# dexmal/dexbotic

Measured on AMD Instinct MI355X. Metric: episodes/sec DB-CogACT fine-tune, higher is better.
Workload: dtype bf16; 1 GPU; DB-CogACT fine-tune step (CLIP-L/14@224 x1 view, Qwen2.5-7B-class 28L decoder, DiT-B head, AdamW), 16 episodes/GPU, 32-token instruction, S=287; global_batch=16, seq_len=287, parallelism=dp1, optimizer=AdamW serial, grad_accum=1, activations=resident

## Files before the change

dexbotic_amd/_lib.py:

```python
from __future__ import annotations

import ctypes as C
import os

import torch

_HERE = os.path.dirname(os.path.abspath(__file__))
LIB_PATH = os.environ.get("DXA_LIB") or os.path.join(_HERE, "libdexbotic_amd.so")

F32, BF16 = 0, 1
ACT_NONE, ACT_GELU_ERF, ACT_GELU_TANH, ACT_QUICK_GELU, ACT_SILU, ACT_RELU, ACT_SIGMOID = 0, 1, 2, 3, 4, 5, 6
NT, NN, TN = 0, 1, 2
FILTER_BICUBIC = 3
FUSE_NONE, FUSE_SWIGLU = 0, 1

_vp, _i64, _i32, _f32, _sz = C.c_void_p, C.c_int64, C.c_int32, C.c_float, C.c_size_t
_int = C.c_int


class DxaError(RuntimeError):
    pass


class GemmDesc(C.Structure):
    _fields_ = [
        ("layout", _i32), ("in_dtype", _i32), ("out_dtype", _i32), ("act", _i32),
        ("M", _i64), ("N", _i64), ("K", _i64),
        ("A", _vp), ("lda", _i64), ("B", _vp), ("ldb", _i64), ("C", _vp), ("ldc", _i64),
        ("bias", _vp), ("residual", _vp), ("ldr", _i64), ("aux_out", _vp), ("mulgrad", _vp), ("ldg", _i64),
        ("alpha", _f32), ("accumulate", _i32), ("nb", _i32 * 3),
        ("sA", _i64 * 3), ("sB", _i64 * 3), ("sC", _i64 * 3), ("sR", _i64 * 3), ("sG", _i64 * 3),
        ("epi_f32", _i32), ("mirror", _vp), ("sumsq", _vp),
        ("A2", _vp), ("B2", _vp), ("K2", _i64),
        ("fuse", _i32), ("ld_aux", _i64),
    ]


class GemmStepInfo(C.Structure):
    _fields_ = [
        ("kernel", C.c_char_p), ("grid", _i32 * 3), ("block", _i32), ("lds", _i32),
        ("K", _i64), ("K2", _i64), ("a_off", _i64), ("b_off", _i64), ("seg2", _i32),
        ("accumulate", _i32), ("bias", _i32), ("residual", _i32),
        ("tm", _i32), ("tn", _i32), ("full", _i32), ("tail_r", _i32), ("split_s", _i32), ("group_m", _i32),
        ("vecA", _i32), ("vecB", _i32), ("vecC", _i32), ("vecR", _i32), ("vecG", _i32), ("vecBias", _i32),
        ("ksplit", _i32), ("kper", _i32), ("split_ws", _i32), ("mirror", _i32), ("sumsq", _i32),
    ]


class GemmPlanInfo(C.Structure):
    _fields_ = [("nsteps", _i32), ("mirror_pass", _i32), ("sumsq_pass", _i32), ("step", GemmStepInfo * 2)]


class Split3Op(C.Structure):
    _fields_ = [("src", _vp), ("ld", _i64), ("dst", _vp), ("rows", _i64), ("cols", _i64), ("pad", _i64), ("side", _i32), ("transposed", _i32)]


class AttnDesc(C.Structure):
    _fields_ = [
        ("dtype", _i32), ("B", _i32), ("Hq", _i32), ("Hkv", _i32), ("Sq", _i32), ("Sk", _i32), ("D", _i32),
        ("causal", _i32), ("scale", _f32),
        ("q", _vp), ("q_sb", _i64), ("q_sh", _i64), ("q_ss", _i64),
        ("k", _vp), ("k_sb", _i64), ("k_sh", _i64), ("k_ss", _i64),
        ("v", _vp), ("v_sb", _i64), ("v_sh", _i64), ("v_ss", _i64),
        ("o", _vp), ("o_sb", _i64), ("o_sh", _i64), ("o_ss", _i64),
        ("lse", _vp), ("kv_start", _vp), ("kv_end", _vp),
        ("d_o", _vp), ("do_sb", _i64), ("do_sh", _i64), ("do_ss", _i64),
        ("dq", _vp), ("dq_sb", _i64), ("dq_sh", _i64), ("dq_ss", _i64),
        ("dk", _vp), ("dk_sb", _i64), ("dk_sh", _i64), ("dk_ss", _i64),
        ("dv", _vp), ("dv_sb", _i64), ("dv_sh", _i64), ("dv_ss", _i64),
        ("force_generic", _i32),
        ("q_limit", _vp), ("key_valid", _vp), ("drop_mask", _vp),
    ]


class AdamWDesc(C.Structure):
    _fields_ = [
        ("p", _vp), ("g", _vp), ("m", _vp), ("v", _vp), ("shadow", _vp),
        ("chunk_start", _vp), ("chunk_len", _vp), ("chunk_grp", _vp), ("n_chunks", _i32),
        ("lr", _f32 * 8), ("wd", _f32 * 8),
        ("beta1", _f32), ("beta2", _f32), ("eps", _f32), ("bc1", _f32), ("bc2", _f32),
        ("clip_coef", _vp), ("g_dtype", _i32), ("chunk_state", _vp), ("chunk_mv_start", _vp),
    ]


class ImageDesc(C.Structure):
    _fields_ = [
        ("src", _vp), ("n", _i32), ("h", _i32), ("w", _i32), ("pad", _i32), ("bg", C.c_ubyte * 4),
        ("res_h", _i32), ("res_w", _i32), ("crop_top", _i32), ("crop_left", _i32), ("out_h", _i32), ("out_w", _i32),
        ("row0", _i32), ("rows", _i32), ("hb", _vp), ("hk", _vp), ("hks", _i32), ("vb", _vp), ("vk", _vp), ("vks", _i32),
        ("tmp", _vp), ("out", _vp), ("out_dtype", _i32), ("out_u8", _vp), ("rescale", C.c_double),
        ("mean", _f32 * 3), ("std", _f32 * 3),
    ]


class DecodeDesc(C.Structure):
    _fields_ = [
        ("layers", _vp), ("x_in", _vp), ("out", _vp), ("final_norm_w", _vp), ("cos_row", _vp), ("sin_row", _vp),
        ("workspace", _vp), ("workspace_bytes", _sz),
        ("n_layers", _i32), ("d", _i32), ("Hq", _i32), ("Hkv", _i32), ("D", _i32), ("F", _i32), ("slot", _i32), ("kv_lo", _i32),
        ("max_len", _i32), ("eps", _f32),
    ]


SIGNATURES = {
    "dxa_last_error": (C.c_char_p, []),
    "dxa_version": (_int, []),
    "dxa_gemm": (_int, [C.POINTER(GemmDesc), _vp]),
    "dxa_gemm_plan": (_int, [C.POINTER(GemmDesc), C.POINTER(GemmPlanInfo)]),
    "dxa_gemm_kernel_name": (C.c_char_p, [_int]),
    "dxa_split3": (_int, [_vp, _i64, _vp, _i64, _i64, _int, _vp]),
    "dxa_split3_t": (_int, [_vp, _i64, _vp, _i64, _i64, _i64, _int, _vp]),
    "dxa_split3_pair": (_int, [C.POINTER(Split3Op), C.POINTER(Split3Op), _vp]),
    "dxa_rmsnorm_fwd": (_int, [_vp, _vp, _vp, _vp, _i64, _i64, _f32, _int, _int, _vp]),
    "dxa_rmsnorm_bwd": (_int, [_vp, _vp, _vp, _vp, _vp, _vp, _vp, _i64, _i64, _int, _int, _vp]),
    "dxa_layernorm_fwd": (_int, [_vp, _vp, _vp, _vp, _vp, _vp, _i64, _i64, _f32, _int, _int, _vp]),
    "dxa_layernorm_bwd": (_int, [_vp, _vp, _vp, _vp, _vp, _vp, _vp, _vp, _i64, _i64, _int, _int, _vp]),
    "dxa_norm_bwd_blocks": (_int, [_i64]),
    "dxa_downsample_layernorm_fwd": (_int, [_vp, _vp, _vp, _vp, _vp, _vp, _i64, _i64, _i64, _f32, _int, _int, _vp]),
    "dxa_downsample_layernorm_bwd": (_int, [_vp, _vp, _vp, _vp, _vp, _vp, _vp, _i64, _i64, _i64, _int, _int, _vp]),
    "dxa_colsum": (_int, [_vp, _i64, _vp, _i64, _i64, _int, _int, _vp, _sz, _vp]),
    "dxa_rope_split": (_int, [_vp, _vp, _vp, _vp, _vp, _vp, _vp, _int, _int, _int, _int, _int, _int, _vp]),
    "dxa_rope_merge": (_int, [_vp, _vp, _vp, _vp, _vp, _vp, _vp, _int, _int, _int, _int, _int, _int, _vp]),
    "dxa_rope_split_at": (_int, [_vp, _vp, _vp, _vp, _vp, _vp, _vp, _int, _int, _int, _int, _int, _int, _int, _int, _vp]),
    "dxa_rope_merge_at": (_int, [_vp, _vp, _vp, _vp, _vp, _vp, _vp, _int, _int, _int, _int, _int, _int, _int, _int, _vp]),
    "dxa_qknorm_rope_split": (_int, [_vp, _vp, _vp, _vp, _vp, _vp, _f32, _vp, _vp, _vp, _vp, _int, _int, _int, _int, _int, _int, _vp]),
    "dxa_qknorm_rope_merge": (_int, [_vp, _vp, _vp, _vp, _vp, _vp, _vp, _vp, _vp, _vp, _vp, _vp, _int, _int, _int, _int, _int, _int, _vp]),
    "dxa_qknorm_rope_merge_blocks": (_int, [_i64, _int, _int, _int, _int]),
    "dxa_attn_fwd": (_int, [C.POINTER(AttnDesc), _vp]),
    "dxa_attn_fwd_workspace": (_sz, [C.POINTER(AttnDesc)]),
    "dxa_attn_fwd_ws": (_int, [C.POINTER(AttnDesc), _vp, _sz, _vp]),
    "dxa_attn_bwd_workspace": (_sz, [C.POINTER(AttnDesc)]),
    "dxa_attn_bwd": (_int, [C.POINTER(AttnDesc), _vp, _sz, _vp]),
    "dxa_swiglu_fwd": (_int, [_vp, _vp, _i64, _i64, _int, _vp]),
    "dxa_swiglu_bwd": (_int, [_vp, _vp, _vp, _i64, _i64, _int, _vp]),
    "dxa_axpby": (_int, [_vp, _vp, _vp, _i64, _f32, _f32, _int, _vp]),
    "dxa_mul": (_int, [_vp, _vp, _vp, _i64, _int, _vp]),
    "dxa_mul_rows": (_int, [_vp, _vp, _vp, _i64, _i64, _i64, _int, _vp]),
    "dxa_glu_fwd": (_int, [_vp, _vp, _i64, _i64, _int, _int, _vp]),
    "dxa_glu_bwd": (_int, [_vp, _vp, _vp, _i64, _i64, _int, _int, _vp]),
    "dxa_act_fwd": (_int, [_vp, _vp, _i64, _int, _int, _vp]),
    "dxa_act_bwd": (_int, [_vp, _vp, _vp, _i64, _int, _int, _vp]),
    "dxa_add": (_int, [_vp, _vp, _vp, _i64, _int, _vp]),
    "dxa_cast": (_int, [_vp, _vp, _i64, _int, _int, _vp]),
    "dxa_copy2d": (_int, [_vp, _i64, _vp, _i64, _i64, _i64, _i64, _int, _int, _vp]),
    "dxa_transpose": (_int, [_vp, _i64, _vp, _i64, _i64, _i64, _i64, _int, _vp]),
    "dxa_permute_bshd": (_int, [_vp, _vp, _int, _int, _int, _int, _int, _int, _vp]),
    "dxa_splice_fwd": (_int, [_vp, _vp, _vp, _vp, _i64, _i64, _int, _vp]),
    "dxa_splice_bwd": (_int, [_vp, _vp, _vp, _vp, _i64, _i64, _int, _vp]),
    "dxa_zero_rows": (_int, [_vp, _vp, _i64, _i64, _vp]),
    "dxa_gather_rows": (_int, [_vp, _vp, _vp, _i64, _i64, _int, _int, _vp]),
    "dxa_scatter_rows": (_int, [_vp, _vp, _vp, _i64, _i64, _i64, _int, _int, _vp]),
    "dxa_im2col": (_int, [_vp, _vp, _int, _int, _int, _int, _i64, _int, _int, _vp]),
    "dxa_vit_embed_fwd": (_int, [_vp, _vp, _vp, _vp, _int, _int, _int, _int, _int, _vp]),
    "dxa_vit_embed_bwd": (_int, [_vp, _vp, _int, _int, _int, _int, _vp]),
    "dxa_qsample": (_int, [_vp, _vp, _vp, _vp, _vp, _i64, _i64, _vp]),
    "dxa_timestep_embedding": (_int, [_vp, _vp, _vp, _i64, _int, _vp]),
    "dxa_dit_assemble_fwd": (_int, [_vp, _vp, _vp, _vp, _vp, _int, _int, _int, _vp]),
    "dxa_dit_assemble_bwd": (_int, [_vp, _vp, _vp, _int, _int, _int, _vp]),
    "dxa_token_drop": (_int, [_vp, _vp, _vp, _vp, _i64, _i64, _vp]),
    "dxa_token_drop_bwd": (_int, [_vp, _vp, _vp, _vp, _i64, _i64, _int, _vp]),
    "dxa_dropout_mask": (_int, [_vp, _i64, _f32, C.c_uint64, C.c_uint64, _int, _vp]),
    "dxa_bank_consolidate": (_int, [_vp, _vp, _int, _i64, _i64, _int, _int, _vp, _vp]),
    "dxa_add_rows": (_int, [_vp, _vp, _vp, _i64, _i64, _i64, _f32, _int, _vp]),
    "dxa_token_sum": (_int, [_vp, _vp, _i64, _i64, _i64, _f32, _int, _vp]),
    "dxa_mse_loss": (_int, [_vp, _vp, _vp, _vp, _i64, _f32, _vp]),
    "dxa_mse_loss_rows": (_int, [_vp, _vp, _vp, _vp, _vp, _i64, _i64, _f32, _vp]),
    "dxa_ddim_step": (_int, [_vp, _vp, _i64, _i64, _int, _f32, _f32, _f32, _f32, _vp]),
    "dxa_adamw": (_int, [C.POINTER(AdamWDesc), _vp]),
    "dxa_sumsq": (_int, [_vp, _i64, _int, _vp, _vp, _int, _vp]),
    "dxa_sumsq_ranges": (_int, [_vp, _int, _vp, _vp, _int, _vp, _vp, _int, _vp]),
    "dxa_sum_f32": (_int, [_vp, _i64, _vp, _int, _vp]),
    "dxa_gemm_sumsq_slots": (_i64, [_i64, _i64]),
    "dxa_cross_entropy_fwd": (_int, [_vp, _i64, _vp, _vp, _vp, _i64, _i64, _i64, _int, _vp]),
    "dxa_cross_entropy_bwd": (_int, [_vp, _i64, _vp, _vp, _vp, _f32, _vp, _i64, _i64, _i64, _i64, _int, _vp]),
    "dxa_soft_cross_entropy_fwd": (_int, [_vp, _i64, _vp, _vp, _vp, _i64, _i64, _i64, _vp, _vp, _int, _f32, _int, _vp]),
    "dxa_soft_cross_entropy_bwd": (_int, [_vp, _i64, _vp, _vp, _vp, _f32, _vp, _i64, _i64, _i64, _i64, _vp, _vp, _int, _f32,
                                          _int, _vp]),
    "dxa_argmax_rows": (_int, [_vp, _i64, _vp, _i64, _i64, _int, _vp]),
    "dxa_sample_rows": (_int, [_vp, _i64, _i64, _i64, _int, _f32, _i64, _f32, _vp, _vp, _vp, _vp, _vp, _vp]),
    "dxa_resample_ksize":(_int, [_int, _int]),
    "dxa_resample_coeffs": (_int, [_int, _int, _int, _vp, _vp]),
    "dxa_image_preprocess": (_int, [C.POINTER(ImageDesc), _vp]),
    "dxa_dit_blocks_workspace": (_sz, [_int, _int, _int]),
    "dxa_dit_blocks_fwd": (_int, [_vp, _vp, _int, _int, _int, _int, _int, _int, _f32, _vp, _sz, _vp]),
    "dxa_dit_blocks_status": (_int, [_vp, _vp]),
    "dxa_dit_sample_workspace": (_sz, [_int, _int, _int]),
    "dxa_dit_sample_fwd": (_int, [_vp] * 9 + [_int, _int, _int, _int, _f32, _vp, _int, _int, _int, _int, _int, _int, _f32, _vp, _sz, _vp]),
    "dxa_dit_bf16_pack_bytes": (_sz, [_int, _int, _int]),
    "dxa_dit_bf16_pack": (_int, [_vp, _int, _int, _int, _vp, _sz, _vp, _vp]),
    "dxa_dit_bf16_pack_per_bytes": (_sz, [_int, _int, _int]),
    "dxa_dit_bf16_pack_per": (_int, [_vp, _int, _int, _int, _vp, _sz, _vp, _vp]),
    "dxa_dit_sample_bf16_per_fwd": (_int, [_vp] * 9 + [_int, _int, _int, _int, _f32, _vp, _vp, _int, _int, _int, _int, _int, _int, _int, _f32, _vp, _sz, _vp]),
    "dxa_dit_sample_bf16_workspace": (_sz, [_int, _int, _int]),
    "dxa_dit_sample_bf16_fwd": (_int, [_vp] * 9 + [_int, _int, _int, _int, _f32, _vp, _int, _int, _int, _int, _int, _int, _f32, _vp, _sz, _vp]),
    "dxa_decode_step_workspace": (_sz, [_int, _int, _int, _int, _int]),
    "dxa_decode_step": (_int, [C.POINTER(DecodeDesc), _vp]),
    "dxa_decode_status": (_int, [_vp, _vp]),
    "dxa_clip_coef": (_int, [_vp, _f32, _vp, _vp, _vp]),
    "dxa_clip_coef_scaled": (_int, [_vp, _f32, _f32, _vp, _vp, _vp]),
    "dxa_scale": (_int, [_vp, _i64, _f32, _vp]),
    "dxa_scale_dev": (_int, [_vp, _i64, _vp, _vp]),
}


def _load() -> C.CDLL:
    if not os.path.exists(LIB_PATH):
        raise ImportError(
            f"dexbotic_amd: native library {LIB_PATH} not found. Build it with "
            "`python -m dexbotic_amd.build` (hipcc --offload-arch=gfx950); there is no CPU fallback.")
    lib = C.CDLL(LIB_PATH)
    for name, (res, args) in SIGNATURES.items():
        try:
            fn = getattr(lib, name)
        except AttributeError as e:
            raise ImportError(f"dexbotic_amd: symbol {name} missing from {LIB_PATH} (stale build?)") from e
        fn.restype = res
        fn.argtypes = args
    return lib


lib = _load()


def last_error() -> str:
    return (lib.dxa_last_error() or b"").decode()


def check(rc: int, what: str = "") -> None:
    if rc != 0:
        raise DxaError(f"{what}: status {rc}: {last_error()}")
```

dexbotic_amd/csrc/gemm.hip:

```cpp
#include "common.h"
#include "gemm_common.h"

#include <algorithm>
#include <cassert>

namespace {


template <typename T> struct EltTraits;
template <> struct EltTraits<float> { static constexpr int EPC = 4; };
template <> struct EltTraits<bf16_t> { static constexpr int EPC = 8; };

__device__ __forceinline__ int lds_off(int row, int chunk) { return row * ROWB + ((chunk ^ (row & 7)) << 4); }

template <typename T, int NR>
__device__ __forceinline__ void load_kc(uint4 (&r)[4], const T* __restrict__ base, int64_t ld, int64_t row0,
                                        int64_t rows, int64_t k0, int64_t K, int vec, int tid) {
  constexpr int EPC = EltTraits<T>::EPC;
  const int c = tid & 7;
  const int64_t k = k0 + (int64_t)c * EPC;
#pragma unroll
  for (int i = 0; i < NR / 32; ++i) {
    const int64_t row = row0 + (tid >> 3) + 32 * i;
    uint4 v = make_uint4(0, 0, 0, 0);
// ... 515 lines not shown
#pragma unroll
    for (int w = 0; w < 8; ++w) {
      const float4 v = *reinterpret_cast<const float4*>(red[w][wave][lane]);
      a4[0] += v.x; a4[1] += v.y; a4[2] += v.z; a4[3] += v.w;
    }
  }
  if (split_s > 1) {
    constexpr int SC1 = 16;
    constexpr uint32_t SLOT = MB * 64 * 16;
    const __amdgpu_buffer_rsrc_t rW = __builtin_amdgcn_make_buffer_rsrc(p.ws, 0, (int)(256u * 7u * 4u * 64u * 16u), 0x00020000);
    const uint32_t slot0 = (uint32_t)tile * (uint32_t)(split_s - 1) * SLOT + (uint32_t)(wave * 64 + lane) * 16u;
    if (split_j < split_s - 1) {
      if (worker) {
        const f32x4_t v = {a4[0], a4[1], a4[2], a4[3]};
        __builtin_amdgcn_raw_buffer_store_b128(__builtin_bit_cast(u32x4_t, v), rW, slot0 + (uint32_t)split_j * SLOT, 0, SC1);
      }
      asm volatile("s_waitcnt vmcnt(0)" ::: "memory");
      __syncthreads();
      if (tid == 0) __hip_atomic_fetch_add(p.flags + tile, 1, __ATOMIC_RELAXED, __HIP_MEMORY_SCOPE_AGENT);
      return;
    }
    if (tid == 0) {
      while (__hip_atomic_load(p.flags + tile, __ATOMIC_RELAXED, __HIP_MEMORY_SCOPE_AGENT) < split_s - 1)
        __builtin_amdgcn_s_sleep(2);
      __hip_atomic_store(p.flags + tile, 0, __ATOMIC_RELAXED, __HIP_MEMORY_SCOPE_AGENT);
    }
    __syncthreads();
    if (worker) {
      float own[4] = {a4[0], a4[1], a4[2], a4[3]};
      a4[0] = a4[1] = a4[2] = a4[3] = 0.f;
      for (int sj = 0; sj < split_s - 1; ++sj) {
        const f32x4_t v = __builtin_bit_cast(f32x4_t, __builtin_amdgcn_raw_buffer_load_b128(rW, slot0 + (uint32_t)sj * SLOT, 0, SC1));
        a4[0] += v[0]; a4[1] += v[1]; a4[2] += v[2]; a4[3] += v[3];
      }
      a4[0] += own[0]; a4[1] += own[1]; a4[2] += own[2]; a4[3] += own[3];
    }
  }
  if (!worker) return;
  const int64_t m = (int64_t)wave * 16 + l16, n = n0 + 4 * lg;
  if (m >= p.M || n >= p.N) return;
  const int n_ok = (int)min((int64_t)4, p.N - n);
  float bv[4] = {0.f, 0.f, 0.f, 0.f};
  const float* bias = reinterpret_cast<const float*>(p.bias);
  if (bias) load4<float>(bv, bias + n, p.vecBias, n_ok);
  epilogue4<float, float>(p, reinterpret_cast<float*>(p.C), reinterpret_cast<float*>(p.aux),
                          reinterpret_cast<const float*>(p.R), reinterpret_cast<const float*>(p.G), bv, m, n, n_ok, a4);
}

template <int MB, typename TO, int U = 2>
__global__ __launch_bounds__(512) void gemm_skinny_bf16_kernel(const GemmP p) {
  __shared__ float red[8][MB][64][4];
  const int tid = threadIdx.x, lane = tid & 63, wave = tid >> 6;
  const int l16 = lane & 15, lg = lane >> 4;
  const int split_s = p.split_s > 1 ? p.split_s : 1;
  const int ntile = (int)gridDim.x / split_s;
  const int tile = (int)blockIdx.x % ntile, split_j = (int)blockIdx.x / ntile;
  const int64_t n0 = (int64_t)tile * 16;
  const bf16_t* W = reinterpret_cast<const bf16_t*>(p.B) + min(n0 + l16, p.N - 1) * p.ldb + 8 * lg;
  const bf16_t* A[MB];
#pragma unroll
  for (int mb = 0; mb < MB; ++mb)
    A[mb] = reinterpret_cast<const bf16_t*>(p.A) + min((int64_t)mb * 16 + l16, p.M - 1) * p.lda + 8 * lg;
  f32x4_t acc[MB];
#pragma unroll
  for (int mb = 0; mb < MB; ++mb) acc[mb] = (f32x4_t){0.f, 0.f, 0.f, 0.f};
  const int nkb = (int)(p.K / 64);
  const int kb_lo = split_j * nkb / split_s, kb_hi = (split_j + 1) * nkb / split_s;
  for (int kb = kb_lo + wave; kb < kb_hi; kb += 8 * U) {
    u32x4n_t wv[U][2];
    uint4 av[U][MB][2];
#pragma unroll
    for (int u = 0; u < U; ++u) {
      const int k0 = (kb + 8 * u) * 64;
      if (kb + 8 * u < kb_hi) {
#pragma unroll
        for (int j = 0; j < 2; ++j) wv[u][j] = __builtin_nontemporal_load(reinterpret_cast<const u32x4n_t*>(W + k0 + 32 * j));
#pragma unroll
        for (int mb = 0; mb < MB; ++mb)
#pragma unroll
          for (int j = 0; j < 2; ++j) av[u][mb][j] = *reinterpret_cast<const uint4*>(A[mb] + k0 + 32 * j);
      } else {
#pragma unroll
        for (int j = 0; j < 2; ++j) {
          wv[u][j] = (u32x4n_t){0u, 0u, 0u, 0u};
#pragma unroll
          for (int mb = 0; mb < MB; ++mb) av[u][mb][j] = make_uint4(0, 0, 0, 0);
        }
      }
    }
#pragma unroll
    for (int u = 0; u < U; ++u)
#pragma unroll
      for (int j = 0; j < 2; ++j)
#pragma unroll
        for (int mb = 0; mb < MB; ++mb)
          acc[mb] = __builtin_amdgcn_mfma_f32_16x16x32_bf16(__builtin_bit_cast(bf16x8_t, wv[u][j]),
                                                            __builtin_bit_cast(bf16x8_t, av[u][mb][j]), acc[mb], 0, 0, 0);
  }
#pragma unroll
  for (int mb = 0; mb < MB; ++mb)
    *reinterpret_cast<float4*>(red[wave][mb][lane]) = make_float4(acc[mb][0], acc[mb][1], acc[mb][2], acc[mb][3]);
  __syncthreads();
  const bool worker = wave < MB;
  float a4[4] = {0.f, 0.f, 0.f, 0.f};
  if (worker) {
#pragma unroll
    for (int w = 0; w < 8; ++w) {
      const float4 v = *reinterpret_cast<const float4*>(red[w][wave][lane]);
      a4[0] += v.x; a4[1] += v.y; a4[2] += v.z; a4[3] += v.w;
    }
  }
  if (split_s > 1) {
    constexpr int SC1 = 16;
    constexpr uint32_t SLOT = MB * 64 * 16;
    const __amdgpu_buffer_rsrc_t rW = __builtin_amdgcn_make_buffer_rsrc(p.ws, 0, (int)(256u * 7u * 4u * 64u * 16u), 0x00020000);
    const uint32_t slot0 = (uint32_t)tile * (uint32_t)(split_s - 1) * SLOT + (uint32_t)(wave * 64 + lane) * 16u;
    if (split_j < split_s - 1) {
      if (worker) {
        const f32x4_t v = {a4[0], a4[1], a4[2], a4[3]};
        __builtin_amdgcn_raw_buffer_store_b128(__builtin_bit_cast(u32x4_t, v), rW, slot0 + (uint32_t)split_j * SLOT, 0, SC1);
      }
      asm volatile("s_waitcnt vmcnt(0)" ::: "memory");
      __syncthreads();
      if (tid == 0) __hip_atomic_fetch_add(p.flags + tile, 1, __ATOMIC_RELAXED, __HIP_MEMORY_SCOPE_AGENT);
      return;
    }
    if (tid == 0) {
      while (__hip_atomic_load(p.flags + tile, __ATOMIC_RELAXED, __HIP_MEMORY_SCOPE_AGENT) < split_s - 1)
        __builtin_amdgcn_s_sleep(2);
      __hip_atomic_store(p.flags + tile, 0, __ATOMIC_RELAXED, __HIP_MEMORY_SCOPE_AGENT);
    }
    __syncthreads();
    if (worker) {
      const float own[4] = {a4[0], a4[1], a4[2], a4[3]};
      a4[0] = a4[1] = a4[2] = a4[3] = 0.f;
      for (int sj = 0; sj < split_s - 1; ++sj) {
        const f32x4_t v = __builtin_bit_cast(f32x4_t, __builtin_amdgcn_raw_buffer_load_b128(rW, slot0 + (uint32_t)sj * SLOT, 0, SC1));
        a4[0] += v[0]; a4[1] += v[1]; a4[2] += v[2]; a4[3] += v[3];
      }
      a4[0] += own[0]; a4[1] += own[1]; a4[2] += own[2]; a4[3] += own[3];
    }
  }
  if (!worker) return;
  const int64_t m = (int64_t)wave * 16 + l16, n = n0 + 4 * lg;
  if (m >= p.M || n >= p.N) return;
  const int n_ok = (int)min((int64_t)4, p.N - n);
  float bv[4] = {0.f, 0.f, 0.f, 0.f};
  const bf16_t* bias = reinterpret_cast<const bf16_t*>(p.bias);
  if (bias) load4<bf16_t>(bv, bias + n, p.vecBias, n_ok);
  epilogue4<bf16_t, TO>(p, reinterpret_cast<TO*>(p.C), reinterpret_cast<TO*>(p.aux), reinterpret_cast<const bf16_t*>(p.R),
                        reinterpret_cast<const bf16_t*>(p.G), bv, m, n, n_ok, a4);
}


template <typename TO, int AI, typename TE>
__global__ __launch_bounds__(512) void gemm_nt_ring_kernel(const GemmP p) {
#if defined(__HIP_DEVICE_COMPILE__)
  extern __shared__ __attribute__((aligned(16))) char smem[];
  constexpr int A_ST = 256 * 64, STAGE = 2 * A_ST;
  constexpr int BMR = AI * 64;
  const int tid = threadIdx.x, lane = tid & 63;
  const int wave = __builtin_amdgcn_readfirstlane(tid >> 6);
  const int wm = wave >> 2, wn = wave & 3;
  const int l32 = lane & 31, lh = lane >> 5;

  int bid = blockIdx.x;
  int split_j = 0, split_s = 1, tail_i = 0;
  if (bid < p.full) {
    const int q = p.full >> 3, r = p.full & 7, xcd = bid & 7;
    bid = (xcd < r ? xcd * (q + 1) : r * (q + 1) + (xcd - r) * q) + (bid >> 3);
  } else {
    const int idx = bid - p.full;
    tail_i = idx % p.tail_r;
    split_j = idx / p.tail_r;
    split_s = p.split_s;
    bid = p.full + tail_i;
  }
  const int GROUP_M = p.group_m;
  const int width = GROUP_M * p.tn;
  const int group = bid / width;
  const int first_pm = group * GROUP_M;
  const int gsz = min(p.tm - first_pm, GROUP_M);
  const int pm = first_pm + (bid % width) % gsz;
  const int pn = (bid % width) / gsz;
  const int64_t m0 = (int64_t)pm * BMR, n0 = (int64_t)pn * 256;
  const bool has_a = AI == 4 || wave < 6;

  const uint32_t bytesA = (uint32_t)(((p.M - 1) * p.lda + p.K) * 2);
  const uint32_t bytesB = (uint32_t)(((p.N - 1) * p.ldb + p.K) * 2);
  const __amdgpu_buffer_rsrc_t rA = __builtin_amdgcn_make_buffer_rsrc(const_cast<char*>(p.A), 0, bytesA, 0x00020000);
  const __amdgpu_buffer_rsrc_t rB = __builtin_amdgcn_make_buffer_rsrc(const_cast<char*>(p.B), 0, bytesB, 0x00020000);
  uint32_t offA[2], offB[2];
#pragma unroll
  for (int j = 0; j < 2; ++j) {
    const int row = (wave * 2 + j) * 16 + (lane >> 2);
    const int chunk = (lane & 3) ^ ((row >> 2) & 3);
    const int64_t ga = m0 + row, gb = n0 + row;
    offA[j] = ga < p.M ? (uint32_t)((ga * p.lda) * 2 + chunk * 16) : 0x80000000u;
    offB[j] = gb < p.N ? (uint32_t)((gb * p.ldb) * 2 + chunk * 16) : 0x80000000u;
  }
  const int nk_tot = (int)(p.K / 32);
  const int k_lo = (int)((int64_t)split_j * nk_tot / split_s);
  const int nk = (int)((int64_t)(split_j + 1) * nk_tot / split_s) - k_lo;
#define DMA_A(slab, j) __builtin_amdgcn_raw_ptr_buffer_load_lds(rA, (lds_void_t*)(smem + ((slab) & 3) * STAGE + (wave * 2 + (j)) * 1024), 16, offA[j], (k_lo + (slab)) * 64, 0, 0)
#define DMA_B(slab, j) __builtin_amdgcn_raw_ptr_buffer_load_lds(rB, (lds_void_t*)(smem + ((slab) & 3) * STAGE + A_ST + (wave * 2 + (j)) * 1024), 16, offB[j], (k_lo + (slab)) * 64, 0, 0)
#define DMA_SLAB(slab) do { if (has_a) { DMA_A(slab, 0); DMA_A(slab, 1); } DMA_B(slab, 0); DMA_B(slab, 1); } while (0)
#define WAIT_PREV_SLAB() do { if (has_a) asm volatile("s_waitcnt vmcnt(4)" ::: "memory"); else asm volatile("s_waitcnt vmcnt(2)" ::: "memory"); } while (0)

  f32x16_t acc[AI][2];
#pragma unroll
  for (int i = 0; i < AI; ++i)
#pragma unroll
    for (int j = 0; j < 2; ++j)
#pragma unroll
      for (int r = 0; r < 16; ++r) acc[i][j][r] = 0.f;

  DMA_SLAB(0);
  if (nk > 1) DMA_SLAB(1);
  if (nk > 2) {
    DMA_SLAB(2);
    WAIT_PREV_SLAB();
  } else {
    asm volatile("s_waitcnt vmcnt(0)" ::: "memory");
  }
  __builtin_amdgcn_s_barrier();
  __builtin_amdgcn_sched_barrier(0);

  u32x4_t a0[AI], b0[2], a1[AI], b1[2];
  const uint32_t lds0 = (uint32_t)(uintptr_t)(__attribute__((address_space(3))) char*)smem;
  const int sw = (l32 >> 2) & 3;
  const uint32_t abase0 = lds0 + (wm * (BMR / 2) + l32) * 64 + (((0 + lh) ^ sw) << 4);
  const uint32_t abase1 = lds0 + (wm * (BMR / 2) + l32) * 64 + (((2 + lh) ^ sw) << 4);
  const uint32_t bbase0 = lds0 + A_ST + (wn * 64 + l32) * 64 + (((0 + lh) ^ sw) << 4);
  const uint32_t bbase1 = lds0 + A_ST + (wn * 64 + l32) * 64 + (((2 + lh) ^ sw) << 4);
#define DS_READ(dst, addr, imm) asm volatile("ds_read_b128 %0, %1 offset:%2" : "=v"(dst) : "v"(addr), "n"(imm) : "memory")
#define RD_SET(A_, B_, abase, bbase, soff)                                                      \
  do {                                                                                          \
    const uint32_t ax_ = (abase) + (soff), bx_ = (bbase) + (soff);                              \
    DS_READ(A_[0], ax_, 0); DS_READ(A_[1], ax_, 2048); DS_READ(A_[2], ax_, 4096);          \
    if constexpr (AI > 3) DS_READ(A_[3], ax_, 6144);                                            \
    DS_READ(B_[0], bx_, 0); DS_READ(B_[1], bx_, 2048);                                          \
  } while (0)
#define MFMA1(A_, B_, i, j) acc[i][j] = __builtin_amdgcn_mfma_f32_32x32x16_bf16(__builtin_bit_cast(bf16x8_t, B_[j]), __builtin_bit_cast(bf16x8_t, A_[i]), acc[i][j], 0, 0, 0)
#define SB() __builtin_amdgcn_sched_barrier(0)

  RD_SET(a0, b0, abase0, bbase0, 0u);
  for (int t = 0; t < nk; ++t) {
    const uint32_t soff = (uint32_t)((t & 3) * STAGE), soff_n = (uint32_t)(((t + 1) & 3) * STAGE);
    const bool dma = t + 3 < nk;
    asm volatile("s_waitcnt lgkmcnt(0)" ::: "memory");
    SB();
    MFMA1(a0, b0, 0, 0); MFMA1(a0, b0, 0, 1);
    SB();
    RD_SET(a1, b1, abase1, bbase1, soff);
    SB();
    MFMA1(a0, b0, 1, 0); MFMA1(a0, b0, 1, 1);
    SB();
    if (dma && has_a) { DMA_A(t + 3, 0); DMA_A(t + 3, 1); }
    SB();
    MFMA1(a0, b0, 2, 0); MFMA1(a0, b0, 2, 1);
    SB();
    if (dma) { DMA_B(t + 3, 0); DMA_B(t + 3, 1); }
    SB();
    if constexpr (AI > 3) { MFMA1(a0, b0, 3, 0); MFMA1(a0, b0, 3, 1); }
    SB();
    asm volatile("s_waitcnt lgkmcnt(0)" ::: "memory");
    SB();
    MFMA1(a1, b1, 0, 0); MFMA1(a1, b1, 0, 1);
    SB();
    if (t + 1 < nk) RD_SET(a0, b0, abase0, bbase0, soff_n);
    SB();
    MFMA1(a1, b1, 1, 0); MFMA1(a1, b1, 1, 1);
    MFMA1(a1, b1, 2, 0); MFMA1(a1, b1, 2, 1);
    if constexpr (AI > 3) { MFMA1(a1, b1, 3, 0); MFMA1(a1, b1, 3, 1); }
    SB();
    if (dma) WAIT_PREV_SLAB();
    else asm volatile("s_waitcnt vmcnt(0)" ::: "memory");
    __builtin_amdgcn_s_barrier();
    SB();
  }
#undef DMA_A
#undef DMA_B
#undef DMA_SLAB
#undef WAIT_PREV_SLAB
#undef DS_READ
#undef RD_SET
#undef MFMA1
#undef SB

  tile_finish<TO, AI, TE>(p, acc, smem, tid, lane, wave, wm, wn, l32, lh, m0, n0, split_j, split_s, tail_i);
#endif
}


template <typename TO, typename TE, bool LEAN, bool A_KS, bool B_KS, int FUSE = 0>
__global__ __launch_bounds__(512) void gemm_pp_kernel(const GemmP p) {
#if defined(__HIP_DEVICE_COMPILE__)
  extern __shared__ __attribute__((aligned(16))) char smem[];
  constexpr int REG = 256 * 128;
  constexpr int BUF = 2 * REG;
  const int tid = threadIdx.x, lane = tid & 63;
  const int wave = __builtin_amdgcn_readfirstlane(tid >> 6);
  const int wm = wave >> 2, wn = wave & 3;
  const int l32 = lane & 31, lh = lane >> 5;

  int bid = blockIdx.x;
  int split_j = 0, split_s = 1, tail_i = 0;
  if (bid < p.full) {
    const int q = p.full >> 3, r = p.full & 7, xcd = bid & 7;
    bid = (xcd < r ? xcd * (q + 1) : r * (q + 1) + (xcd - r) * q) + (bid >> 3);
  } else {
    const int idx = bid - p.full;
    tail_i = idx % p.tail_r;
    split_j = idx / p.tail_r;
    split_s = p.split_s;
    bid = p.full + tail_i;
  }
  int m0i, n0i;
  sk_tile_origin(p, bid, m0i, n0i);
  const int64_t m0 = m0i, n0 = n0i;

  const uint32_t bytesA = (uint32_t)((A_KS ? (p.K - 1) * p.lda + p.M : (p.M - 1) * p.lda + p.K) * 2);
  const uint32_t bytesB = (uint32_t)((B_KS ? (p.K - 1) * p.ldb + p.N : (p.N - 1) * p.ldb + p.K) * 2);
  const __amdgpu_buffer_rsrc_t rA = __builtin_amdgcn_make_buffer_rsrc(const_cast<char*>(p.A), 0, bytesA, 0x00020000);
  const __amdgpu_buffer_rsrc_t rB = __builtin_amdgcn_make_buffer_rsrc(const_cast<char*>(p.B), 0, bytesB, 0x00020000);
#define PP_A_ROW0(h, j) ((((wave * 2 + (j)) & 7) * 8) + (((wave * 2 + (j)) >> 3) * 128) + 64 * (h))
#define PP_B_ROW0(h, j) ((((wave * 2 + (j)) >> 2) * 64) + (((wave * 2 + (j)) & 3) * 8) + 32 * (h))
  uint32_t voA[2][2], voB[2][2];
  {
    const int lrow = lane >> 3, lslot = lane & 7;
    const uint32_t lda2 = (uint32_t)p.lda * 2u, ldb2 = (uint32_t)p.ldb * 2u;
#pragma unroll
    for (int h = 0; h < 2; ++h)
#pragma unroll
      for (int j = 0; j < 2; ++j) {
        const int krow = (wave * 2 + j) * 4 + (lane >> 4);
        const int sig = (lane & 15) ^ ((krow & 3) << 2) ^ (((krow >> 3) & 1) << 1);
        if constexpr (A_KS) {
          const int ga = m0i + (sig >> 3) * 128 + 64 * h + 8 * (sig & 7);
          voA[h][j] = ga < (int)p.M ? (uint32_t)krow * lda2 + (uint32_t)ga * 2u : 0x80000000u;
        } else {
          const int ra = PP_A_ROW0(h, j) + lrow, ga = m0i + ra;
          voA[h][j] = ga < (int)p.M ? (uint32_t)ga * lda2 + (uint32_t)((lslot ^ ((ra >> 1) & 7)) << 4) : 0x80000000u;
        }
        if constexpr (B_KS) {
          const int gb = n0i + (sig >> 2) * 64 + 32 * h + 8 * (sig & 3);
          voB[h][j] = gb < (int)p.N ? (uint32_t)krow * ldb2 + (uint32_t)gb * 2u : 0x80000000u;
        } else if constexpr (FUSE == 1) {
          const int rb = PP_B_ROW0(h, j) + lrow, half_n = (int)(p.N >> 1);
          const int lc = (n0i >> 1) + (rb >> 6) * 32 + (rb & 31), gb = ((rb >> 5) & 1) * half_n + lc;
          voB[h][j] = lc < half_n ? (uint32_t)gb * ldb2 + (uint32_t)((lslot ^ ((rb >> 1) & 7)) << 4) : 0x80000000u;
        } else {
          const int rb = PP_B_ROW0(h, j) + lrow, gb = n0i + rb;
          voB[h][j] = gb < (int)p.N ? (uint32_t)gb * ldb2 + (uint32_t)((lslot ^ ((rb >> 1) & 7)) << 4) : 0x80000000u;
        }
      }
  }
  const int nk1 = (int)((p.K + 63) >> 6);
  const int nk_tot = nk1 + ((A_KS && B_KS) ? (int)((p.K2 + 63) >> 6) : 0);
  const bool seg2 = (A_KS && B_KS) && p.K2 > 0;
  const __amdgpu_buffer_rsrc_t rA2 = __builtin_amdgcn_make_buffer_rsrc(
      const_cast<char*>(seg2 ? p.A2 : p.A), 0, seg2 ? (uint32_t)(((p.K2 - 1) * p.lda + p.M) * 2) : 0u, 0x00020000);
  const __amdgpu_buffer_rsrc_t rB2 = __builtin_amdgcn_make_buffer_rsrc(
      const_cast<char*>(seg2 ? p.B2 : p.B), 0, seg2 ? (uint32_t)(((p.K2 - 1) * p.ldb + p.N) * 2) : 0u, 0x00020000);
  const int k_lo = split_j * nk_tot / split_s;
  const int nk = (split_j + 1) * nk_tot / split_s - k_lo;
  const uint32_t ktileA = A_KS ? 64u * (uint32_t)p.lda * 2u : 0u, ktileB = B_KS ? 64u * (uint32_t)p.ldb * 2u : 0u;
#define PP_DMA(rsrc, vo, ldsoff, buf, soff)                                                                             \
  __builtin_amdgcn_raw_ptr_buffer_load_lds(rsrc, (lds_void_t*)(smem + (buf) * BUF + (ldsoff)), 16, vo, soff, 0, 0)
#define PP_DMA_A1(h, j, buf, tile)                                                                          \
  do {                                                                                                      \
    if constexpr (A_KS && B_KS) {                                                                           \
      const int kt_ = k_lo + (tile);                                                                        \
      if (kt_ < nk1) PP_DMA(rA, voA[h][j] + (uint32_t)kt_ * ktileA, (h) * 16384 + (wave * 2 + (j)) * 1024, buf, 0);          \
      else PP_DMA(rA2, voA[h][j] + (uint32_t)(kt_ - nk1) * ktileA, (h) * 16384 + (wave * 2 + (j)) * 1024, buf, 0);           \
    } else if constexpr (A_KS) {                                                                            \
      const uint32_t kb_ = (uint32_t)(k_lo + (tile)) * ktileA;                                              \
      PP_DMA(rA, voA[h][j] + kb_, (h) * 16384 + (wave * 2 + (j)) * 1024, buf, 0);                           \
    } else {                                                                                                \
      PP_DMA(rA, voA[h][j], PP_A_ROW0(h, j) * 128, buf, (k_lo + (tile)) * 128);                             \
    }                                                                                                       \
  } while (0)
#define PP_DMA_B1(h, j, buf, tile)                                                                          \
  do {                                                                                                      \
    if constexpr (A_KS && B_KS) {                                                                           \
      const int kt_ = k_lo + (tile);                                                                        \
      if (kt_ < nk1) PP_DMA(rB, voB[h][j] + (uint32_t)kt_ * ktileB, REG + (h) * 16384 + (wave * 2 + (j)) * 1024, buf, 0);    \
      else PP_DMA(rB2, voB[h][j] + (uint32_t)(kt_ - nk1) * ktileB, REG + (h) * 16384 + (wave * 2 + (j)) * 1024, buf, 0);     \
    } else if constexpr (B_KS) {                                                                            \
      const uint32_t kb_ = (uint32_t)(k_lo + (tile)) * ktileB;                                              \
      PP_DMA(rB, voB[h][j] + kb_, REG + (h) * 16384 + (wave * 2 + (j)) * 1024, buf, 0);                     \
    } else {                                                                                                \
      PP_DMA(rB, voB[h][j], REG + PP_B_ROW0(h, j) * 128, buf, (k_lo + (tile)) * 128);                       \
    }                                                                                                       \
  } while (0)
#define PP_DMA_A(h, buf, tile) do { PP_DMA_A1(h, 0, buf, tile); PP_DMA_A1(h, 1, buf, tile); } while (0)
#define PP_DMA_B(h, buf, tile) do { PP_DMA_B1(h, 0, buf, tile); PP_DMA_B1(h, 1, buf, tile); } while (0)

  f32x4_t acc[8][4];
#pragma unroll
  for (int i = 0; i < 8; ++i)
#pragma unroll
    for (int j = 0; j < 4; ++j) acc[i][j] = (f32x4_t){0.f, 0.f, 0.f, 0.f};

  const uint32_t lds0 = (uint32_t)(uintptr_t)(__attribute__((address_space(3))) char*)smem;
  const int i16 = lane & 15, g = lane >> 4, sw = (i16 >> 1) & 7, tq = (i16 >> 2) & 3;
  const uint32_t ks_lane = (uint32_t)((8 * g + (i16 >> 2)) * 256 + (g & 1) * 32 + (i16 & 3) * 8);
  const uint32_t ya = A_KS ? lds0 + ks_lane + (uint32_t)(((wm * 2) ^ tq) << 6)
                           : (lds0 + (wm * 128 + i16) * 128) | (uint32_t)((g ^ sw) << 4);
  const uint32_t yb = B_KS ? lds0 + REG + ks_lane + (uint32_t)((wn ^ tq) << 6)
                           : (lds0 + REG + (wn * 64 + i16) * 128) | (uint32_t)((g ^ sw) << 4);
  u32x4_t af[4][2], bq[2][2][2];
  typedef uint32_t u32x2_t __attribute__((ext_vector_type(2)));
#define PP_READ(dst, addr, imm) asm volatile("ds_read_b128 %0, %1 offset:%2" : "=v"(dst) : "v"(addr), "n"(imm) : "memory")
#define PP_READ_TR(dst, addr, imm) asm volatile("ds_read_b64_tr_b16 %0, %1 offset:%2" : "=v"(dst) : "v"(addr), "n"(imm) : "memory")
#define PP_FRAG_TR(dst, addr, imm)                                                       \
  do {                                                                                   \
    u32x2_t lo_ = {0u, 0u}, hi_ = {0u, 0u};                                              \
    PP_READ_TR(lo_, addr, imm); PP_READ_TR(hi_, addr, (imm) + 1024);                     \
    dst = (u32x4_t){lo_[0], lo_[1], hi_[0], hi_[1]};                                     \
  } while (0)
#define PP_RDF_A(cur, h, b, ks)                                                                             \
  do {                                                                                                      \
    if constexpr (A_KS) PP_FRAG_TR(af[b][ks], ya ^ (uint32_t)((cur) * BUF + 32 * (b)), (h) * 16384 + (ks) * 8192); \
    else PP_READ(af[b][ks], ya ^ (uint32_t)((cur) * BUF + 64 * (ks)), (4 * (h) + (b)) * 2048);            \
  } while (0)
#define PP_RDF_B(cur, j, b, ks)                                                                             \
  do {                                                                                                      \
    if constexpr (B_KS) PP_FRAG_TR(bq[j][b][ks], yb ^ (uint32_t)((cur) * BUF + 32 * (b)), (j) * 16384 + (ks) * 8192); \
    else PP_READ(bq[j][b][ks], yb ^ (uint32_t)((cur) * BUF + 64 * (ks)), (2 * (j) + (b)) * 2048);         \
  } while (0)
#define PP_MFMA(h, j, b, jb, ks)                                                                                            \
  acc[4 * (h) + (b)][2 * (j) + (jb)] = __builtin_amdgcn_mfma_f32_16x16x32_bf16(                                           \
      __builtin_bit_cast(bf16x8_t, bq[j][jb][ks]), __builtin_bit_cast(bf16x8_t, af[b][ks]), acc[4 * (h) + (b)][2 * (j) + (jb)], 0, 0, 0)
#define PP_SB() __builtin_amdgcn_sched_barrier(0)
#define PP_BAR() do { PP_SB(); __builtin_amdgcn_s_barrier(); PP_SB(); } while (0)
#define PP_MFMA2(h, j, b, ks, R) do { PP_MFMA(h, j, b, 0, ks); PP_MFMA(h, j, b, 1, ks); PP_SB(); R(ks, b); PP_SB(); } while (0)
#define PP_COMPUTE_R(h, j, R)                                                                     \
  do {                                                                                            \
    asm volatile("s_waitcnt lgkmcnt(0)" ::: "memory");                                            \
    PP_SB();                                                                                      \
    PP_MFMA2(h, j, 0, 0, R); PP_MFMA2(h, j, 1, 0, R); PP_MFMA2(h, j, 2, 0, R); PP_MFMA2(h, j, 3, 0, R); \
    PP_MFMA2(h, j, 0, 1, R); PP_MFMA2(h, j, 1, 1, R); PP_MFMA2(h, j, 2, 1, R); PP_MFMA2(h, j, 3, 1, R); \
  } while (0)
#define PP_R_NONE(ks, b) do { } while (0)
#define PP_VMCNT(n) asm volatile("s_waitcnt vmcnt(" #n ")" ::: "memory")
#if defined(DXA_PP_STAMPS)
  uint64_t ts_[8];
  uint32_t iv_[8] = {0u, 0u, 0u, 0u, 0u, 0u, 0u, 0u}, ts_last_ = 0u;
#define PP_STAMP(i) asm volatile("s_memtime %0" : "=s"(ts_[i]))
#define PP_STAMPS_FOLD()                                                                                    \
  do {                                                                                                      \
    asm volatile("s_waitcnt lgkmcnt(0)" ::: "memory");                                                      \
    PP_SB();                                                                                                \
    if (ts_last_ != 0u) iv_[7] += (uint32_t)ts_[0] - ts_last_;                                              \
    _Pragma("unroll") for (int i_ = 0; i_ < 7; ++i_) iv_[i_] += (uint32_t)ts_[i_ + 1] - (uint32_t)ts_[i_];  \
    ts_last_ = (uint32_t)ts_[7];                                                                            \
    PP_SB();                                                                                                \
  } while (0)
#else
#define PP_STAMP(i) do { } while (0)
#define PP_STAMPS_FOLD() do { } while (0)
#endif
#define PP_R_B1(ks, b) do { if constexpr (((b) & 1) != 0) PP_RDF_B(cur_, 1, (b) >> 1, ks); } while (0)
#define PP_R_A1(ks, b) PP_RDF_A(cur_, 1, b, ks)
#define PP_R_NEXT(ks, b)                                                                                    \
  do {                                                                                                      \
    if (more1) {                                                                                            \
      PP_RDF_A(cur_ ^ 1, 0, b, ks);                                                                         \
      if constexpr ((ks) == 1 && (b) < 2) PP_RDF_B(cur_ ^ 1, 0, (b) & 1, 0);                                \
      if constexpr ((ks) == 1 && (b) == 3) { PP_RDF_B(cur_ ^ 1, 0, 0, 1); PP_RDF_B(cur_ ^ 1, 0, 1, 1); }    \
    }                                                                                                       \
  } while (0)
#define PP_TILE(cur, t)                                                                                     \
  do {                                                                                                      \
    constexpr int cur_ = (cur);                                                                             \
    const bool more1 = (t) + 1 < nk, more2 = (t) + 2 < nk;                                                  \
                                                                                               \
    if (more1) { PP_DMA_A(1, cur_ ^ 1, (t) + 1); PP_SB(); PP_VMCNT(8); } else { PP_VMCNT(0); }              \
    PP_BAR(); PP_STAMP(0); PP_COMPUTE_R(0, 0, PP_R_B1); PP_BAR(); PP_STAMP(1);                              \
                                                                                               \
    if (more2) { PP_DMA_A(0, cur_, (t) + 2); PP_SB(); }                                                     \
    PP_BAR(); PP_STAMP(2); PP_COMPUTE_R(0, 1, PP_R_A1); PP_BAR(); PP_STAMP(3);                              \
                                                                                               \
    if (more2) { PP_DMA_B(0, cur_, (t) + 2); PP_SB(); PP_VMCNT(8); } else if (more1) { PP_VMCNT(4); }       \
    PP_BAR(); PP_STAMP(4); PP_COMPUTE_R(1, 1, PP_R_NONE); PP_BAR(); PP_STAMP(5);                                         \
                                                                                               \
    if (more2) { PP_DMA_B(1, cur_, (t) + 2); PP_SB(); PP_VMCNT(8); } else if (more1) { PP_VMCNT(2); }       \
    PP_BAR(); PP_STAMP(6); PP_COMPUTE_R(1, 0, PP_R_NEXT); PP_BAR(); PP_STAMP(7);                            \
    PP_STAMPS_FOLD();                                                                                       \
  } while (0)

  PP_DMA_A(0, 0, 0); PP_DMA_B(0, 0, 0); PP_DMA_B(1, 0, 0); PP_DMA_A(1, 0, 0);
  if (nk > 1) { PP_DMA_A(0, 1, 1); PP_DMA_B(0, 1, 1); PP_DMA_B(1, 1, 1); }
  PP_SB();
  if (nk > 1) { PP_VMCNT(8); } else { PP_VMCNT(2); }
  PP_BAR();
  PP_RDF_A(0, 0, 0, 0); PP_RDF_A(0, 0, 1, 0); PP_RDF_A(0, 0, 2, 0); PP_RDF_A(0, 0, 3, 0);
  PP_RDF_A(0, 0, 0, 1); PP_RDF_A(0, 0, 1, 1); PP_RDF_A(0, 0, 2, 1); PP_RDF_A(0, 0, 3, 1);
  PP_RDF_B(0, 0, 0, 0); PP_RDF_B(0, 0, 1, 0); PP_RDF_B(0, 0, 0, 1); PP_RDF_B(0, 0, 1, 1);
  PP_SB();
  if (wm == 1) PP_BAR();
  for (int t = 0; t < nk; t += 2) {
    PP_TILE(0, t);
    if (t + 1 < nk) PP_TILE(1, t + 1);
  }
  if (wm == 0) PP_BAR();
#if defined(DXA_PP_STAMPS)
  const uint32_t iv0_ = iv_[0], iv1_ = iv_[1], iv2_ = iv_[2], iv3_ = iv_[3], iv4_ = iv_[4], iv5_ = iv_[5], iv6_ = iv_[6], iv7_ = iv_[7];
#endif
#undef PP_A_ROW0
#undef PP_B_ROW0
#undef PP_DMA
#undef PP_DMA_A
#undef PP_DMA_B
#undef PP_READ
#undef PP_READ_TR
#undef PP_FRAG_TR
#undef PP_RDF_A
#undef PP_RDF_B
#undef PP_MFMA
#undef PP_MFMA2
#undef PP_SB
#undef PP_BAR
#undef PP_R_NONE
#undef PP_VMCNT
#undef PP_TILE
#undef PP_DMA_A1
#undef PP_DMA_B1
#undef PP_STAMP
#undef PP_STAMPS_FOLD
#undef PP_COMPUTE_R
#undef PP_R_B1
#undef PP_R_A1
#undef PP_R_NEXT

  if constexpr (LEAN) {
    if (!tile_split_exchange<4, 16>(p, acc, tid, split_j, split_s, tail_i)) return;
    __builtin_amdgcn_sched_barrier(0);
    if constexpr (FUSE == 1) sk_epilogue_swiglu<4, 16>(p, acc, smem + wave * 4096, lane, wm, wn, m0i, n0i);
    else sk_epilogue<TO, TE, 4, 16>(p, acc, smem + wave * 4096, lane, wm, wn, m0i, n0i, reinterpret_cast<float*>(smem + 8 * 4096), bid);
#if defined(DXA_PP_STAMPS)
    __syncthreads();
    if (m0i == 0 && n0i == 0 && lane == 0) {
      uint32_t* o_ = reinterpret_cast<uint32_t*>(p.C) + wave * 16;
      o_[0] = iv0_; o_[1] = iv1_; o_[2] = iv2_; o_[3] = iv3_; o_[4] = iv4_; o_[5] = iv5_; o_[6] = iv6_; o_[7] = iv7_;
      o_[8] = (uint32_t)nk;
    }
#endif
  } else {
    tile_finish<TO, 4, TE, false, 16>(p, acc, smem, tid, lane, wave, wm, wn, l32, lh, m0, n0, split_j, split_s, tail_i);
  }
#endif
}

#if defined(DXA_PP3_STAMPS)
__device__ unsigned long long g_pp3_stamps[4];
#define P3_STAMP(i) do { if (blockIdx.x == DXA_PP3_STAMPS && threadIdx.x == 0) { unsigned long long t_; asm volatile("s_memtime %0\n\ts_waitcnt lgkmcnt(0)" : "=s"(t_) :: "memory"); g_pp3_stamps[i] = t_; } } while (0)
#else
#define P3_STAMP(i) do { } while (0)
#endif
template <typename TO, typename TE, bool LEAN, int FUSE = 0>
__global__ __launch_bounds__(512) void gemm_pp3_kernel(const GemmP p) {
#if defined(__HIP_DEVICE_COMPILE__)
  extern __shared__ __attribute__((aligned(16))) char smem[];
  P3_STAMP(0);
  constexpr int AREG = 192 * 128, BREG = 256 * 128, BUFSZ = AREG + BREG;
  const int tid = threadIdx.x, lane = tid & 63;
  const int wave = __builtin_amdgcn_readfirstlane(tid >> 6);
  const int wm = wave >> 2, wn = wave & 3;
  const int l32 = lane & 31, lh = lane >> 5;
  int bid = blockIdx.x;
  int split_j = 0, split_s = 1, tail_i = 0;
  if (bid < p.full) {
    const int q = p.full >> 3, r = p.full & 7, xcd = bid & 7;
    bid = (xcd < r ? xcd * (q + 1) : r * (q + 1) + (xcd - r) * q) + (bid >> 3);
  } else {
    const int idx = bid - p.full;
    tail_i = idx % p.tail_r;
    split_j = idx / p.tail_r;
    split_s = p.split_s;
    bid = p.full + tail_i;
  }
  const int width = p.group_m * p.tn;
  const int group = bid / width;
  const int first_pm = group * p.group_m;
  const int gsz = min(p.tm - first_pm, p.group_m);
  const int pm = first_pm + (bid % width) % gsz;
  const int pn = (bid % width) / gsz;
  const int64_t m0 = (int64_t)pm * 192, n0 = (int64_t)pn * 256;

  const uint32_t bytesA = (uint32_t)(((p.M - 1) * p.lda + p.K) * 2);
  const uint32_t bytesB = (uint32_t)(((p.N - 1) * p.ldb + p.K) * 2);
  const __amdgpu_buffer_rsrc_t rA = __builtin_amdgcn_make_buffer_rsrc(const_cast<char*>(p.A), 0, bytesA, 0x00020000);
  const __amdgpu_buffer_rsrc_t rB = __builtin_amdgcn_make_buffer_rsrc(const_cast<char*>(p.B), 0, bytesB, 0x00020000);
#define P3_A_ROW0(g) ((wave >> 2) * 96 + 32 * (g) + (wave & 3) * 8)
#define P3_B_ROW0(h, j) ((((wave * 2 + (j)) >> 2) * 64) + (((wave * 2 + (j)) & 3) * 8) + 32 * (h))
  uint32_t voA[3], voB[2][2];
  {
    const int lrow = lane >> 3, lslot = lane & 7;
    const uint32_t lda2 = (uint32_t)p.lda * 2u, ldb2 = (uint32_t)p.ldb * 2u;
#pragma unroll
    for (int g = 0; g < 3; ++g) {
      const int ra = P3_A_ROW0(g) + lrow;
      const int64_t ga = m0 + ra;
      voA[g] = ga < p.M ? (uint32_t)ga * lda2 + (uint32_t)((lslot ^ ((ra >> 1) & 7)) << 4) : 0x80000000u;
    }
#pragma unroll
    for (int h = 0; h < 2; ++h)
#pragma unroll
      for (int j = 0; j < 2; ++j) {
        const int rb = P3_B_ROW0(h, j) + lrow;
        if constexpr (FUSE == 1) {
          const int half_n = (int)(p.N >> 1);
          const int lc = (int)(n0 >> 1) + (rb >> 6) * 32 + (rb & 31), gb = ((rb >> 5) & 1) * half_n + lc;
          voB[h][j] = lc < half_n ? (uint32_t)gb * ldb2 + (uint32_t)((lslot ^ ((rb >> 1) & 7)) << 4) : 0x80000000u;
        } else {
          const int64_t gb = n0 + rb;
          voB[h][j] = gb < p.N ? (uint32_t)gb * ldb2 + (uint32_t)((lslot ^ ((rb >> 1) & 7)) << 4) : 0x80000000u;
        }
      }
  }
  const int nk_tot = (int)(p.K / 64);
  const int k_lo = split_j * nk_tot / split_s;
  const int nk = (split_j + 1) * nk_tot / split_s - k_lo;
#define P3_DMA(rsrc, vo, ldsoff, buf, tile) \
  __builtin_amdgcn_raw_ptr_buffer_load_lds(rsrc, (lds_void_t*)(smem + (buf) * BUFSZ + (ldsoff)), 16, vo, (k_lo + (tile)) * 128, 0, 0)
#define P3_DMA_A(g, buf, tile) P3_DMA(rA, voA[g], P3_A_ROW0(g) * 128, buf, tile)
#define P3_DMA_B(h, buf, tile) do { P3_DMA(rB, voB[h][0], AREG + P3_B_ROW0(h, 0) * 128, buf, tile); P3_DMA(rB, voB[h][1], AREG + P3_B_ROW0(h, 1) * 128, buf, tile); } while (0)

  f32x16_t acc[3][2];
#pragma unroll
  for (int i = 0; i < 3; ++i)
#pragma unroll
    for (int j = 0; j < 2; ++j)
#pragma unroll
      for (int r = 0; r < 16; ++r) acc[i][j][r] = 0.f;

  const uint32_t lds0 = (uint32_t)(uintptr_t)(__attribute__((address_space(3))) char*)smem;
  const int sw = (l32 >> 1) & 7;
  const uint32_t ya0 = (lds0 + (wm * 96 + l32) * 128) | (uint32_t)((lh ^ sw) << 4), ya1 = ya0 + BUFSZ;
  const uint32_t yb0 = (lds0 + AREG + (wn * 64 + l32) * 128) | (uint32_t)((lh ^ sw) << 4), yb1 = yb0 + BUFSZ;
  u32x4_t af[2][4], bq[2][2][4];
#define P3_READ(dst, addr, imm) asm volatile("ds_read_b128 %0, %1 offset:%2" : "=v"(dst) : "v"(addr), "n"(imm) : "memory")
#define P3_RD_A(buf, g, set, ks) P3_READ(af[set][ks], ((buf) ? ya1 : ya0) ^ (uint32_t)(32 * (ks)), (g) * 4096)
#define P3_RD_B(buf, h, bset, ks) P3_READ(bq[bset][h][ks], ((buf) ? yb1 : yb0) ^ (uint32_t)(32 * (ks)), (h) * 4096)
#define P3_MFMA(g, set, bset, j, ks) acc[g][j] = __builtin_amdgcn_mfma_f32_32x32x16_bf16(__builtin_bit_cast(bf16x8_t, bq[bset][j][ks]), __builtin_bit_cast(bf16x8_t, af[set][ks]), acc[g][j], 0, 0, 0)
#define P3_SB() __builtin_amdgcn_sched_barrier(0)
#define P3_BAR() do { P3_SB(); __builtin_amdgcn_s_barrier(); P3_SB(); } while (0)
#define P3_COMPUTE(g, set, bset, R)                                                                 \
  do {                                                                                              \
    asm volatile("s_waitcnt lgkmcnt(0)" ::: "memory");                                              \
    P3_SB();                                                                                        \
    P3_MFMA(g, set, bset, 0, 0); P3_MFMA(g, set, bset, 1, 0); P3_SB(); R(0); P3_SB();               \
    P3_MFMA(g, set, bset, 0, 1); P3_MFMA(g, set, bset, 1, 1); P3_SB(); R(1); P3_SB();               \
    P3_MFMA(g, set, bset, 0, 2); P3_MFMA(g, set, bset, 1, 2); P3_SB(); R(2); P3_SB();               \
    P3_MFMA(g, set, bset, 0, 3); P3_MFMA(g, set, bset, 1, 3); P3_SB(); R(3); P3_SB();               \
  } while (0)
#define P3_VMCNT(n) asm volatile("s_waitcnt vmcnt(" #n ")" ::: "memory")
#define P3_TILE(cur, t)                                                                                                  \
  do {                                                                                                                   \
    constexpr int cur_ = (cur), s0_ = (cur), s1_ = (cur) ^ 1;            \
    const bool more1 = (t) + 1 < nk, more2 = (t) + 2 < nk;                                                               \
                                                                                                            \
    if (more1) P3_DMA_A(2, cur_ ^ 1, (t) + 1);                                                                           \
    if (more2) { P3_DMA_B(0, cur_, (t) + 2); P3_SB(); P3_VMCNT(7); } else if (more1) { P3_SB(); P3_VMCNT(5); } else { P3_VMCNT(0); } \
    P3_BAR();                                                                                                            \
    P3_COMPUTE(0, s0_, cur_, P3_R_A1);                                                                                   \
    P3_BAR();                                                                                                            \
                                                                                                            \
    if (more2) { P3_DMA_A(0, cur_, (t) + 2); P3_DMA_B(1, cur_, (t) + 2); P3_SB(); P3_VMCNT(7); } else if (more1) { P3_VMCNT(2); } \
    P3_BAR();                                                                                                            \
    P3_COMPUTE(1, s1_, cur_, P3_R_A2B0);                                                                                 \
    P3_BAR();                                                                                                            \
                                                                                                            \
    if (more2) { P3_DMA_A(1, cur_, (t) + 2); P3_SB(); P3_VMCNT(7); } else if (more1) { P3_VMCNT(1); }                    \
    P3_BAR();                                                                                                            \
    P3_COMPUTE(2, s0_, cur_, P3_R_A0B1);                                                                                 \
    P3_BAR();                                                                                                            \
  } while (0)
#define P3_R_A1(ks) P3_RD_A(cur_, 1, s1_, ks)
#define P3_R_A2B0(ks) do { P3_RD_A(cur_, 2, s0_, ks); if (more1) P3_RD_B(cur_ ^ 1, 0, cur_ ^ 1, ks); } while (0)
#define P3_R_A0B1(ks) do { if (more1) { P3_RD_A(cur_ ^ 1, 0, s1_, ks); P3_RD_B(cur_ ^ 1, 1, cur_ ^ 1, ks); } } while (0)

  P3_DMA_B(0, 0, 0); P3_DMA_A(0, 0, 0); P3_DMA_B(1, 0, 0); P3_DMA_A(1, 0, 0); P3_DMA_A(2, 0, 0);
  if (nk > 1) { P3_DMA_B(0, 1, 1); P3_DMA_A(0, 1, 1); P3_DMA_B(1, 1, 1); P3_DMA_A(1, 1, 1); }
  P3_SB();
  if (nk > 1) { P3_VMCNT(7); } else { P3_VMCNT(1); }
  P3_BAR();
  P3_STAMP(1);
#pragma unroll
  for (int ks = 0; ks < 4; ++ks) { P3_RD_A(0, 0, 0, ks); P3_RD_B(0, 0, 0, ks); P3_RD_B(0, 1, 0, ks); }
  P3_SB();
  if (wm == 1) P3_BAR();
  for (int t = 0; t < nk; t += 2) {
    P3_TILE(0, t);
    if (t + 1 < nk) P3_TILE(1, t + 1);
  }
  if (wm == 0) P3_BAR();
  P3_STAMP(2);
#undef P3_A_ROW0
#undef P3_B_ROW0
#undef P3_DMA
#undef P3_DMA_A
#undef P3_DMA_B
#undef P3_READ
#undef P3_RD_A
#undef P3_RD_B
#undef P3_MFMA
#undef P3_SB
#undef P3_BAR
#undef P3_COMPUTE
#undef P3_VMCNT
#undef P3_TILE
#undef P3_R_A1
#undef P3_R_A2B0
#undef P3_R_A0B1
  if constexpr (LEAN) {
    if (!tile_split_exchange<3>(p, acc, tid, split_j, split_s, tail_i)) return;
    __builtin_amdgcn_sched_barrier(0);
    if constexpr (FUSE == 1) sk_epilogue_swiglu<3>(p, acc, smem + wave * 4096, lane, wm, wn, (int)m0, (int)n0);
    else sk_epilogue<TO, TE, 3>(p, acc, smem + wave * 4096, lane, wm, wn, (int)m0, (int)n0, reinterpret_cast<float*>(smem + 8 * 4096), bid);
  } else {
    tile_finish<TO, 3, TE>(p, acc, smem, tid, lane, wave, wm, wn, l32, lh, m0, n0, split_j, split_s, tail_i);
  }
  asm volatile("s_waitcnt vmcnt(0)" ::: "memory");
  P3_STAMP(3);
#endif
}
#undef P3_STAMP

template <typename T>
__global__ __launch_bounds__(256) void sumsq_rows_k(const T* __restrict__ C, int64_t ldc, int64_t M, int64_t N,
                                                    float* __restrict__ out) {
  __shared__ float red[4];
  float s = 0.f;
  for (int64_t r = blockIdx.x; r < M; r += gridDim.x) {
    const T* row = C + r * ldc;
    for (int64_t c = threadIdx.x; c < N; c += 256) { const float v = ldf<T>(row + c); s += v * v; }
  }
#pragma unroll
  for (int o = 32; o > 0; o >>= 1) s += __shfl_xor(s, o, 64);
  if ((threadIdx.x & 63) == 0) red[threadIdx.x >> 6] = s;
  __syncthreads();
  if (threadIdx.x == 0) out[blockIdx.x] = (red[0] + red[1]) + (red[2] + red[3]);
}


constexpr int NUM_CU = 256;
static_assert(NUM_CU == NUM_CU_D, "split-K scratch sizing");
constexpr size_t SPLIT_WS_BYTES = (size_t)NUM_CU * 256 * 256 * 4;
int get_split_ws(hipStream_t st, char** ws) {
  static StreamBlock blocks(SPLIT_WS_BYTES + NUM_CU * sizeof(int));
  char* base = nullptr;
  if (int rc = blocks.get(st, &base)) return rc;
  DXA_CHECK_ARG(base != nullptr, "dxa_gemm: first split-K product on a stream allocates its scratch and cannot happen under stream "
                "capture: run the request once eagerly on this stream first");
  *ws = base;
  return DXA_OK;
}

enum GemmArgs { ARGS_P, ARGS_GEMV1, ARGS_GEMV2 };
struct GemmKernel {
  const char* name;
  const void* fn;
  int block, lds;
  int (*raise)(int);
  GemmArgs args;
};
template <auto kernel>
GemmKernel row(const char* name, int block, int lds = 0, GemmArgs args = ARGS_P) {
  return {name, reinterpret_cast<const void*>(kernel), block, lds, lds > 65536 ? &dxa_raise_lds<kernel> : nullptr, args};
}
constexpr int GEN_LDS2 = 4 * (32 * 2) * ROWB, GEN_LDS4 = 4 * (32 * 4) * ROWB;
constexpr int T128_LDS = 4 * 32768;
constexpr int RING_LDS = 139264;
#define KROW_TY3(X, ...) {X(bf16_t, bf16_t, "bf16,bf16", __VA_ARGS__), X(float, bf16_t, "f32,bf16", __VA_ARGS__), X(float, float, "f32,f32", __VA_ARGS__)}
#define KROW_GENERIC(TI, TO, n, A_KS, B_KS, l) {row<gemm_kernel<TI, TO, A_KS, B_KS, 2>>("generic<" n "," l ",64>", 256, GEN_LDS2), \
                                           row<gemm_kernel<TI, TO, A_KS, B_KS, 4>>("generic<" n "," l ",128>", 256, GEN_LDS4)}
#define KROW_GENERIC3(TI, TO, n) {KROW_GENERIC(TI, TO, n, false, false, "nt"), KROW_GENERIC(TI, TO, n, false, true, "nn"), KROW_GENERIC(TI, TO, n, true, true, "tn")}
#define KROW_GEMV1(M) row<gemv_nn_stage1_k<M>>("gemv_nn_stage1<" #M ">", 256, 0, ARGS_GEMV1)
#define KROW_SKINNY_F32(MB) row<gemm_skinny_f32_kernel<MB>>("skinny_f32<" #MB ">", 512)
#define KROW_SKINNY_BF16(MB, U) {row<gemm_skinny_bf16_kernel<MB, bf16_t, U>>("skinny_bf16<" #MB ",bf16>", 512), row<gemm_skinny_bf16_kernel<MB, float, U>>("skinny_bf16<" #MB ",f32>", 512)}
#define KROW_RING(TO, TE, n, AI, rows) row<gemm_nt_ring_kernel<TO, AI, TE>>("ring<" n "," rows ">", 512, RING_LDS)
#define KROW_PP(TO, TE, n, LEAN, A_KS, B_KS, FUSE, l) row<gemm_pp_kernel<TO, TE, LEAN, A_KS, B_KS, FUSE>>("pp<" n "," l ">", 512, RING_LDS)
#define KROW_PP3(TO, TE, n, LEAN, FUSE, l) row<gemm_pp3_kernel<TO, TE, LEAN, FUSE>>("pp3<" n "," l ">", 512, RING_LDS)
const struct GemmKernels {
  GemmKernel generic[3][3][2];
  GemmKernel t128[2];
  GemmKernel gemv1[4], gemv2[2];
  GemmKernel skinny_f32[4];
  GemmKernel skinny_bf16[4][2];
  GemmKernel ring[2][3];
  GemmKernel pp_nt[2][3];
  GemmKernel pp_nn[3];
  GemmKernel pp_tn[2];
  GemmKernel pp_swiglu;
  GemmKernel pp3[2][3], pp3_swiglu;
} KERNELS = {
    {KROW_GENERIC3(bf16_t, bf16_t, "bf16,bf16"), KROW_GENERIC3(bf16_t, float, "bf16,f32"), KROW_GENERIC3(float, float, "f32,f32")},
    {row<gemm_nt_t128_kernel<bf16_t, 4, 4>>("t128<bf16>", 512, T128_LDS), row<gemm_nt_t128_kernel<float, 4, 4>>("t128<f32>", 512, T128_LDS)},
    {KROW_GEMV1(1), KROW_GEMV1(2), KROW_GEMV1(4), KROW_GEMV1(8)},
    {row<gemv_nn_stage2_k<bf16_t>>("gemv_nn_stage2<bf16>", 256, 0, ARGS_GEMV2), row<gemv_nn_stage2_k<float>>("gemv_nn_stage2<f32>", 256, 0, ARGS_GEMV2)},
    {KROW_SKINNY_F32(1), KROW_SKINNY_F32(2), KROW_SKINNY_F32(3), KROW_SKINNY_F32(4)},
    {KROW_SKINNY_BF16(1, 4), KROW_SKINNY_BF16(2, 2), KROW_SKINNY_BF16(3, 2), KROW_SKINNY_BF16(4, 2)},
    {KROW_TY3(KROW_RING, 4, "256"), KROW_TY3(KROW_RING, 3, "192")},
    {KROW_TY3(KROW_PP, true, false, false, 0, "lean,nt"), KROW_TY3(KROW_PP, false, false, false, 0, "full,nt")},
    {KROW_PP(bf16_t, bf16_t, "bf16,bf16", true, false, true, 0, "lean,nn"), KROW_PP(bf16_t, bf16_t, "bf16,bf16", false, false, true, 0, "full,nn"),
     KROW_PP(float, bf16_t, "f32,bf16", true, false, true, 0, "lean,nn")},
    {KROW_PP(bf16_t, bf16_t, "bf16,bf16", true, true, true, 0, "lean,tn"), KROW_PP(float, bf16_t, "f32,bf16", true, true, true, 0, "lean,tn")},
    KROW_PP(bf16_t, bf16_t, "bf16,bf16", true, false, false, 1, "swiglu,nt"),
    {KROW_TY3(KROW_PP3, true, 0, "lean"), KROW_TY3(KROW_PP3, false, 0, "full")},
    KROW_PP3(bf16_t, bf16_t, "bf16,bf16", true, 1, "swiglu"),
};
constexpr int NUM_KERNELS = sizeof(GemmKernels) / sizeof(GemmKernel);

struct GemmPlan {
  dxa_gemm_plan_info info;
  const GemmKernel* kernel[2];
};
void plan_add(GemmPlan* plan, dxa_gemm_step_info s, const GemmKernel& k, int64_t gx, int64_t gy = 1, int64_t gz = 1) {
  assert(plan->info.nsteps < 2);
  s.kernel = k.name;
  s.grid[0] = (int32_t)gx; s.grid[1] = (int32_t)gy; s.grid[2] = (int32_t)gz;
  s.block = k.block; s.lds = k.lds;
  plan->kernel[plan->info.nsteps] = &k;
  plan->info.step[plan->info.nsteps++] = s;
}

inline bool aligned_to(const void* p, size_t a) { return (reinterpret_cast<uintptr_t>(p) % a) == 0; }
inline bool strides_mult(const int64_t s[3], int64_t m) { return s[0] % m == 0 && s[1] % m == 0 && s[2] % m == 0; }

int skinny_split(int64_t tiles, int64_t K) {
  if (tiles > NUM_CU / 2) return 1;
  return (int)std::max<int64_t>(1, std::min<int64_t>(std::min<int64_t>(8, (K / 64) / 8), dxa_cdiv(256, tiles)));
}

int plan_product(const dxa_gemm_desc* d, int64_t nbatch, GemmPlan* plan, bool* seg_fallback) {
  const size_t es = d->in_dtype == DXA_BF16 ? 2 : 4, os = d->out_dtype == DXA_BF16 ? 2 : 4;
  const int64_t epc = 16 / es;
  dxa_gemm_step_info s;
  memset(&s, 0, sizeof(s));
  s.K = d->K;
  s.accumulate = d->accumulate; s.bias = d->bias != nullptr; s.residual = d->residual != nullptr;
  if (d->fuse != DXA_FUSE_NONE) {
    DXA_CHECK_ARG(d->fuse == DXA_FUSE_SWIGLU, "dxa_gemm: unknown fuse mode %d", d->fuse);
    const int64_t F_ = d->N / 2;
    DXA_CHECK_ARG(d->layout == DXA_NT && d->in_dtype == DXA_BF16 && d->out_dtype == DXA_BF16 && nbatch == 1 && d->N % 2 == 0 &&
                  F_ % 8 == 0 && d->K % 64 == 0 && d->K >= 64 && d->M >= 129 && F_ >= 128 && !d->bias && !d->residual && !d->mulgrad &&
                  d->act == DXA_ACT_NONE && !d->accumulate && !d->mirror && !d->sumsq && !d->epi_f32 && d->K2 == 0,
                  "dxa_gemm: DXA_FUSE_SWIGLU is a plain bf16 NT product of the MFMA fast path (M >= 129, K %% 64 == 0, F %% 8 == 0)");
    DXA_CHECK_ARG(aligned_to(d->A, 16) && aligned_to(d->B, 16) && aligned_to(d->C, 8) && d->lda % 8 == 0 && d->ldb % 8 == 0 &&
                  d->ldc % 4 == 0 && d->ldc >= F_ && (!d->aux_out || (aligned_to(d->aux_out, 8) && d->ld_aux % 4 == 0 && d->ld_aux >= d->N)) &&
                  ((d->M - 1) * d->ld_aux + d->N) * 2 < (1ll << 31) && ((d->M - 1) * d->lda + d->K) * 2 < (1ll << 31) &&
                  ((d->N - 1) * d->ldb + d->K) * 2 < (1ll << 31),
                  "dxa_gemm: DXA_FUSE_SWIGLU needs 16-byte aligned operand rows, 8-byte aligned output rows and operands < 2 GiB");
  }
  DXA_CHECK_ARG(!d->mirror || (d->out_dtype == DXA_F32 && nbatch == 1), "dxa_gemm: mirror needs an fp32, unbatched output");
  DXA_CHECK_ARG(!d->sumsq || nbatch == 1, "dxa_gemm: sumsq needs an unbatched output");
  s.tm = dxa_cdiv(d->M, BM);
  s.tn = dxa_cdiv(d->N, BN);
  const bool a_ks = d->layout == DXA_TN, b_ks = d->layout != DXA_NT;
  s.vecA = a_ks ? (aligned_to(d->A, 4 * es) && d->lda % 4 == 0 && strides_mult(d->sA, 4))
                : (aligned_to(d->A, 16) && d->lda % epc == 0 && strides_mult(d->sA, epc));
  s.vecB = b_ks ? (aligned_to(d->B, 4 * es) && d->ldb % 4 == 0 && strides_mult(d->sB, 4))
                : (aligned_to(d->B, 16) && d->ldb % epc == 0 && strides_mult(d->sB, epc));
  s.vecC = aligned_to(d->C, 4 * os) && d->ldc % 4 == 0 && strides_mult(d->sC, 4) &&
           (!d->aux_out || aligned_to(d->aux_out, 4 * os));
  const size_t ees = d->epi_f32 ? 4 : es;
  DXA_CHECK_ARG(!d->epi_f32 || (d->in_dtype == DXA_BF16 && d->out_dtype == DXA_F32), "dxa_gemm: epi_f32 needs bf16 in, fp32 out");
  s.vecR = d->residual && aligned_to(d->residual, 4 * ees) && d->ldr % 4 == 0 && strides_mult(d->sR, 4);
  s.vecG = d->mulgrad && aligned_to(d->mulgrad, 4 * ees) && d->ldg % 4 == 0 && strides_mult(d->sG, 4);
  s.vecBias = d->bias && aligned_to(d->bias, 4 * ees);

  const int64_t bytesA = (a_ks ? (d->K - 1) * d->lda + d->M : (d->M - 1) * d->lda + d->K) * 2;
  const int64_t bytesB = (b_ks ? (d->K - 1) * d->ldb + d->N : (d->N - 1) * d->ldb + d->K) * 2;
  const bool ks_layout = d->layout != DXA_NT;
  const int64_t cpl = 16 / (int64_t)os;
  const bool bf = d->out_dtype == DXA_BF16;
  const bool lean_ok = d->N % cpl == 0 && d->ldc % cpl == 0 && aligned_to(d->C, 16) &&
                       ((d->M - 1) * d->ldc + d->N) * (int64_t)os < (1ll << 31) && !d->aux_out && !d->mulgrad &&
                       d->act == DXA_ACT_NONE && (!d->bias || aligned_to(d->bias, cpl * ees)) &&
                       (!d->residual || (aligned_to(d->residual, cpl * ees) && d->ldr % cpl == 0 &&
                                         ((d->M - 1) * d->ldr + d->N) * (int64_t)ees < (1ll << 31)));
  const bool ks_ok = (d->layout == DXA_NN ? (bf || lean_ok) : lean_ok) && !d->epi_f32 && ks_layout && aligned_to(d->A, 16) && aligned_to(d->B, 16) && d->lda % 8 == 0 && d->ldb % 8 == 0 &&
                     (d->layout == DXA_TN || d->K % 64 == 0) && d->K >= 64;
  const int64_t t128_tiles = (int64_t)dxa_cdiv(d->M, 128) * dxa_cdiv(d->N, 128);
  if (d->fuse == DXA_FUSE_NONE && d->layout == DXA_NT && d->in_dtype == DXA_BF16 && nbatch == 1 && !d->epi_f32 &&
      d->M >= 64 && d->M <= 1024 && d->N >= 64 && d->K >= 64 && d->K % 64 == 0 && s.vecA && s.vecB &&
      bytesA < (1ll << 31) && bytesB < (1ll << 31) && t128_tiles >= 32 && t128_tiles <= NUM_CU && d->K <= 4096) {
    s.tm = dxa_cdiv(d->M, 128); s.tn = dxa_cdiv(d->N, 128);
    int t_split = 1;
    if (t128_tiles <= NUM_CU / 4 || (t128_tiles <= NUM_CU / 2 && d->K >= 2048))
      t_split = (int)std::min<int64_t>(std::min<int64_t>(4, NUM_CU / t128_tiles), (d->K / 64) / 8);
    s.split_s = std::max(t_split, 1);
    s.split_ws = t_split >= 2;
    plan_add(plan, s, KERNELS.t128[!bf], (int64_t)s.tm * s.tn * s.split_s);
    return DXA_OK;
  }
  if (d->K2 > 0) {
    DXA_CHECK_ARG(d->layout == DXA_TN && d->A2 && d->B2 && nbatch == 1, "dxa_gemm: A2 / B2 / K2 need an unbatched TN product");
    const int64_t bytesA2 = ((d->K2 - 1) * d->lda + d->M) * 2, bytesB2 = ((d->K2 - 1) * d->ldb + d->N) * 2;
    const bool seg_fast = d->in_dtype == DXA_BF16 && ks_ok && d->M >= 64 && d->N >= 64 &&
                          (int64_t)d->M * d->N >= 128 * 128 && bytesA < (1ll << 31) && bytesB < (1ll << 31) &&
                          bytesA2 < (1ll << 31) && bytesB2 < (1ll << 31) && aligned_to(d->A2, 16) && aligned_to(d->B2, 16);
    if (!seg_fast) { *seg_fallback = true; return DXA_OK; }
    s.K2 = d->K2;
  }
  if (d->in_dtype == DXA_BF16 && nbatch == 1 &&
      ((d->layout == DXA_NT && d->K >= 32 && d->K % 32 == 0 && s.vecA && s.vecB) || ks_ok) &&
      d->M >= 64 && d->N >= 64 && (int64_t)d->M * d->N >= 128 * 128 && bytesA < (1ll << 31) && bytesB < (1ll << 31)) {
    const int64_t pad256 = (int64_t)dxa_cdiv(d->M, 256) * 256, pad192 = (int64_t)dxa_cdiv(d->M, 192) * 192;
    const int ai = ks_layout ? 4 : (pad192 * 27 < pad256 * 25 ? 3 : 4);
    s.tm = dxa_cdiv(d->M, ai * 64);
    s.tn = dxa_cdiv(d->N, 256);
    const int nt = s.tm * s.tn, nk_tot = (int)((d->K + s.K2 + 31) / 32);
    s.full = nt; s.tail_r = 0; s.split_s = 1; s.group_m = 4;
    const int tail = nt % NUM_CU;
    if (tail > 0) {
      const int split = nk_tot >= 64 ? std::min(std::min(NUM_CU / tail, 8), nk_tot / 32) : 1;
      if (split >= 2) { s.full = nt - tail; s.tail_r = tail; s.split_s = split; s.split_ws = 1; }
    }
    const bool pp = ks_layout || (ai == 4 && d->K % 64 == 0);
    const bool lean = pp && lean_ok;
    s.mirror = lean && d->mirror;
    s.sumsq = lean && d->sumsq;
    const int ty = d->epi_f32 ? 2 : !bf;
    const GemmKernel* k;
    if (d->layout == DXA_NN) k = &KERNELS.pp_nn[bf ? !lean : 2];
    else if (d->layout == DXA_TN) k = &KERNELS.pp_tn[!bf];
    else if (d->fuse == DXA_FUSE_SWIGLU) k = ai == 4 ? &KERNELS.pp_swiglu : &KERNELS.pp3_swiglu;
    else if (pp) k = &KERNELS.pp_nt[!lean][ty];
    else if (ai == 3 && d->K % 64 == 0) k = &KERNELS.pp3[!lean_ok][ty];
    else k = &KERNELS.ring[ai == 3][ty];
    plan_add(plan, s, *k, s.full + s.tail_r * s.split_s);
    return DXA_OK;
  }
  DXA_CHECK_ARG(d->fuse == DXA_FUSE_NONE, "dxa_gemm: fuse is only implemented on the bf16 NT MFMA fast path (K %% 32 == 0, M, N >= 64, 16-byte aligned rows, no batching)");
  DXA_CHECK_ARG(!d->epi_f32, "dxa_gemm: epi_f32 is only implemented on the bf16 NT fast path (K %% 32 == 0, M, N >= 64, "
                              "16-byte aligned rows, no batching)");
  if (d->layout == DXA_NN && d->in_dtype == DXA_BF16 && nbatch == 1 && d->M <= GV_MAXM && d->K >= 64 &&
      d->N >= 64 && d->N % 8 == 0 && d->ldb % 8 == 0 && aligned_to(d->B, 16) && !d->bias && !d->residual && !d->aux_out &&
      !d->mulgrad && d->act == DXA_ACT_NONE && !d->accumulate && !d->epi_f32) {
    const int nbn = dxa_cdiv(d->N, 2048);
    int ksplit = (int)std::min<int64_t>(std::min<int64_t>(64, d->K / 32), dxa_cdiv(512, nbn));
    if (ksplit < 1) ksplit = 1;
    int kper = dxa_cdiv(d->K, ksplit);
    if (kper > 512) { kper = 512; ksplit = dxa_cdiv(d->K, kper); }
    if ((size_t)ksplit * d->M * d->N * sizeof(float) <= SPLIT_WS_BYTES) {
      s.ksplit = ksplit; s.kper = kper; s.split_ws = 1;
      plan_add(plan, s, KERNELS.gemv1[d->M <= 1 ? 0 : d->M <= 2 ? 1 : d->M <= 4 ? 2 : 3], nbn, ksplit);
      plan_add(plan, s, KERNELS.gemv2[!bf], dxa_cdiv(d->M * d->N, 256));
      return DXA_OK;
    }
  }
  if (d->layout == DXA_NT && nbatch == 1 && d->M <= 64 && d->K >= 64 && d->K % 64 == 0 && s.vecA && s.vecB) {
    const int64_t sk_tiles = dxa_cdiv(d->N, 16);
    const int mb = dxa_cdiv(d->M, 16);
    s.split_s = skinny_split(sk_tiles, d->K);
    s.split_ws = s.split_s >= 2;
    plan_add(plan, s, d->in_dtype == DXA_BF16 ? KERNELS.skinny_bf16[mb - 1][!bf] : KERNELS.skinny_f32[mb - 1], sk_tiles * s.split_s);
    return DXA_OK;
  }
  const bool small = (int64_t)s.tm * s.tn * nbatch < 192;
  if (small) { s.tm = dxa_cdiv(d->M, 64); s.tn = dxa_cdiv(d->N, 64); }
  plan_add(plan, s, KERNELS.generic[d->in_dtype == DXA_F32 ? 2 : !bf][d->layout][!small], (int64_t)s.tm * s.tn, 1, nbatch);
  return DXA_OK;
}

int gemm_plan(const dxa_gemm_desc* d, GemmPlan* plan) {
  memset(plan, 0, sizeof(*plan));
  DXA_CHECK_ARG(d != nullptr, "dxa_gemm: null desc");
  DXA_CHECK_ARG(d->M >= 0 && d->N >= 0 && d->K >= 0, "dxa_gemm: negative dims");
  DXA_CHECK_ARG(d->layout >= DXA_NT && d->layout <= DXA_TN, "dxa_gemm: bad layout %d", d->layout);
  DXA_CHECK_ARG(d->in_dtype == DXA_F32 || d->in_dtype == DXA_BF16, "dxa_gemm: bad in_dtype %d", d->in_dtype);
  DXA_CHECK_ARG(d->out_dtype == d->in_dtype || d->out_dtype == DXA_F32,
                "dxa_gemm: out_dtype must equal in_dtype or be fp32");
  DXA_CHECK_ARG(d->nb[0] >= 1 && d->nb[1] >= 1 && d->nb[2] >= 1, "dxa_gemm: batch extents must be >= 1");
  if (d->M == 0 || d->N == 0) return DXA_OK;
  DXA_CHECK_ARG(d->A && d->B && d->C, "dxa_gemm: null operand");
  const int64_t nbatch = (int64_t)d->nb[0] * d->nb[1] * d->nb[2];
  DXA_CHECK_ARG(nbatch <= 65535, "dxa_gemm: too many batches (%lld)", (long long)nbatch);

  dxa_gemm_desc a = *d, b = *d;
  int64_t a_off = 0, b_off = 0;
  bool two = false, seg2 = false;
  const int64_t es = d->in_dtype == DXA_BF16 ? 2 : 4;
  if (d->in_dtype == DXA_BF16 && nbatch == 1 && d->layout != DXA_TN && d->K % 64 != 0 && d->K >= 1024 &&
      d->M >= 256 && d->N >= 256 && d->act == DXA_ACT_NONE && !d->aux_out && !d->mulgrad && !d->sumsq && !d->mirror && !d->epi_f32) {
    a.K = d->K - d->K % 64; b.K = d->K - a.K;
    b.accumulate = 1; b.bias = nullptr; b.residual = nullptr;
    a_off = a.K * es;
    b_off = (d->layout == DXA_NT ? a.K : a.K * d->ldb) * es;
    b.A = (const char*)d->A + a_off; b.B = (const char*)d->B + b_off;
    two = true;
  }
  if (int rc = plan_product(&a, nbatch, plan, &seg2)) return rc;
  if (seg2) {
    assert(!two && d->layout == DXA_TN);
    a.A2 = a.B2 = nullptr; a.K2 = 0; a.mirror = nullptr; a.sumsq = nullptr;
    b.A = d->A2; b.B = d->B2; b.K = d->K2; b.A2 = b.B2 = nullptr; b.K2 = 0;
    b.accumulate = 1; b.bias = nullptr; b.residual = nullptr;
    two = true;
    if (int rc = plan_product(&a, nbatch, plan, &seg2)) return rc;
  }
  const int n0 = plan->info.nsteps;
  if (two)
    if (int rc = plan_product(&b, nbatch, plan, &seg2)) return rc;
  for (int i = n0; i < plan->info.nsteps; ++i) {
    dxa_gemm_step_info& s = plan->info.step[i];
    s.seg2 = seg2; s.a_off = a_off; s.b_off = b_off;
  }
  const dxa_gemm_step_info& last = plan->info.step[plan->info.nsteps - 1];
  plan->info.mirror_pass = d->mirror && !last.mirror;
  plan->info.sumsq_pass = d->sumsq && !last.sumsq;
  return DXA_OK;
}

int gemm_run_step(const dxa_gemm_desc* d, const dxa_gemm_step_info& s, const GemmKernel& k, hipStream_t st, char** ws) {
  GemmP p;
  memset(&p, 0, sizeof(p));
  p.M = d->M; p.N = d->N; p.K = s.K;
  p.A = (const char*)(s.seg2 ? d->A2 : d->A) + s.a_off; p.lda = d->lda;
  p.B = (const char*)(s.seg2 ? d->B2 : d->B) + s.b_off; p.ldb = d->ldb;
  p.C = (char*)d->C; p.ldc = d->ldc;
  p.bias = s.bias ? (const char*)d->bias : nullptr;
  p.R = s.residual ? (const char*)d->residual : nullptr; p.ldr = d->ldr;
  p.aux = (char*)d->aux_out;
  p.G = (const char*)d->mulgrad; p.ldg = d->ldg;
  p.alpha = d->alpha; p.act = d->act; p.accumulate = s.accumulate;
  p.fuse = d->fuse; p.ldaux = d->ld_aux;
  p.nb1 = d->nb[1]; p.nb2 = d->nb[2];
  for (int i = 0; i < 3; ++i) {
    p.sA[i] = d->sA[i]; p.sB[i] = d->sB[i]; p.sC[i] = d->sC[i]; p.sR[i] = d->sR[i]; p.sG[i] = d->sG[i];
  }
  p.tm = s.tm; p.tn = s.tn;
  p.vecA = s.vecA; p.vecB = s.vecB; p.vecC = s.vecC; p.vecR = s.vecR; p.vecG = s.vecG; p.vecBias = s.vecBias;
  p.full = s.full; p.tail_r = s.tail_r; p.split_s = s.split_s; p.group_m = s.group_m;
  if (s.mirror) p.mirror = (char*)d->mirror;
  if (s.sumsq) p.sumsq = d->sumsq;
  if (s.K2 > 0) { p.A2 = (const char*)d->A2; p.B2 = (const char*)d->B2; p.K2 = s.K2; }
  if (s.split_ws) {
    if (*ws == nullptr)
      if (int rc = get_split_ws(st, ws)) return rc;
    p.ws = (float*)*ws; p.flags = (int*)(*ws + SPLIT_WS_BYTES);
  }
  if (int rc = k.raise ? k.raise(k.lds) : DXA_OK) return rc;
  int M = (int)d->M, ksplit = s.ksplit, kper = s.kper;
  void* args_p[] = {&p};
  void* args_gemv1[] = {&p.A, &p.lda, &p.B, &p.ldb, &p.ws, &M, &p.N, &p.K, &kper};
  void* args_gemv2[] = {&p.ws, &p.C, &p.ldc, &M, &p.N, &ksplit, &p.alpha};
  void** args = k.args == ARGS_P ? args_p : k.args == ARGS_GEMV1 ? args_gemv1 : args_gemv2;
  (void)hipLaunchKernel(k.fn, dim3(s.grid[0], s.grid[1], s.grid[2]), dim3(k.block), args, k.lds, st);
  DXA_CHECK_LAUNCH();
  return DXA_OK;
}

}

extern "C" int64_t dxa_gemm_sumsq_slots(int64_t M, int64_t N) {
  if (M <= 0 || N <= 0) return 0;
  return ((M + 255) / 256) * ((N + 255) / 256);
}
extern "C" const char* dxa_gemm_kernel_name(int i) {
  return i >= 0 && i < NUM_KERNELS ? reinterpret_cast<const GemmKernel*>(&KERNELS)[i].name : nullptr;
}
extern "C" int dxa_gemm_plan(const dxa_gemm_desc* d, dxa_gemm_plan_info* out) {
  DXA_CHECK_ARG(out != nullptr, "dxa_gemm_plan: null output");
  GemmPlan plan;
  const int rc = gemm_plan(d, &plan);
  *out = plan.info;
  return rc;
}
extern "C" int dxa_gemm(const dxa_gemm_desc* d, dxa_stream_t stream) {
  GemmPlan plan;
  if (int rc = gemm_plan(d, &plan)) return rc;
  char* ws = nullptr;
  for (int i = 0; i < plan.info.nsteps; ++i) {
    if (int rc = gemm_run_step(d, plan.info.step[i], *plan.kernel[i], (hipStream_t)stream, &ws)) return rc;
  }
  if (plan.info.mirror_pass) {
    if (int rc = dxa_copy2d(d->C, d->ldc, d->mirror, d->ldc, d->M, d->N, d->N, DXA_F32, DXA_BF16, stream)) return rc;
  }
  if (plan.info.sumsq_pass) {
    const dim3 sgrid((unsigned)dxa_gemm_sumsq_slots(d->M, d->N));
    if (d->out_dtype == DXA_F32)
      hipLaunchKernelGGL(sumsq_rows_k<float>, sgrid, dim3(256), 0, (hipStream_t)stream, (const float*)d->C, d->ldc, d->M, d->N, d->sumsq);
    else
      hipLaunchKernelGGL(sumsq_rows_k<bf16_t>, sgrid, dim3(256), 0, (hipStream_t)stream, (const bf16_t*)d->C, d->ldc, d->M, d->N, d->sumsq);
    DXA_CHECK_LAUNCH();
  }
  return DXA_OK;
}

namespace {
struct S3Op { const float* src; int64_t ld; bf16_t* dst; int64_t rows, cols, pad; int side, transposed; unsigned nblocks, tiles_x; };
__global__ __launch_bounds__(256) void split3_pair_k(const S3Op a, const S3Op b) {
  __shared__ float tile[32][33];
  const bool first = blockIdx.x < a.nblocks;
  const S3Op& o = first ? a : b;
  const unsigned bid = first ? blockIdx.x : blockIdx.x - a.nblocks;
  if (!o.transposed) {
    const int64_t c4 = o.cols >> 2;
    for (int64_t i = (int64_t)bid * 256 + threadIdx.x; i < o.rows * c4; i += (int64_t)o.nblocks * 256) {
      const int64_t r = i / c4, c = (i - r * c4) * 4;
      float x[4];
      Vec<float, 4>::ld(x, o.src + r * o.ld + c);
      float hi[4], lo[4];
#pragma unroll
      for (int e = 0; e < 4; ++e) {
        hi[e] = bf2f(f2bf(x[e]));
        lo[e] = x[e] - hi[e];
      }
      bf16_t* d = o.dst + r * 3 * o.cols + c;
      Vec<bf16_t, 4>::st(d, hi);
      Vec<bf16_t, 4>::st(d + o.cols, o.side == 0 ? hi : lo);
      Vec<bf16_t, 4>::st(d + 2 * o.cols, o.side == 0 ? lo : hi);
    }
    return;
  }
  const int tx = threadIdx.x & 31, ty = threadIdx.x >> 5;
  const int64_t R = o.rows, C_ = o.cols, Rp = o.pad;
  const int64_t r0 = (int64_t)(bid / o.tiles_x) * 32, c0 = (int64_t)(bid % o.tiles_x) * 32;
#pragma unroll
  for (int i = 0; i < 4; ++i) {
    const int64_t r = r0 + ty + 8 * i, c = c0 + tx;
    tile[ty + 8 * i][tx] = (r < R && c < C_) ? o.src[r * o.ld + c] : 0.f;
  }
  __syncthreads();
#pragma unroll
  for (int i = 0; i < 4; ++i) {
    const int64_t c = c0 + ty + 8 * i, r = r0 + tx;
    if (c < C_ && r < Rp) {
      const float x = tile[tx][ty + 8 * i];
      const bf16_t hb = f2bf(x);
      const bf16_t lb = f2bf(x - bf2f(hb));
      bf16_t* d = o.dst + c * 3 * Rp + r;
      d[0] = hb;
      d[Rp] = o.side == 0 ? hb : lb;
      d[2 * Rp] = o.side == 0 ? lb : hb;
    }
  }
}
int s3_fill(const dxa_split3_op* u, S3Op* o) {
  DXA_CHECK_ARG(u && u->rows >= 0 && u->cols >= 0 && (u->side == 0 || u->side == 1) && u->ld >= u->cols, "dxa_split3_pair: bad operand");
  o->src = u->src; o->ld = u->ld; o->dst = (bf16_t*)u->dst; o->rows = u->rows; o->cols = u->cols; o->pad = u->pad; o->side = u->side;
  o->transposed = u->transposed != 0; o->nblocks = 0; o->tiles_x = 1;
  if ((o->transposed ? std::max(u->rows, u->pad) : u->rows) == 0 || u->cols == 0) return DXA_OK;
  DXA_CHECK_ARG(u->src && u->dst, "dxa_split3_pair: null buffer");
  if (o->transposed) {
    DXA_CHECK_ARG(u->pad >= u->rows, "dxa_split3_pair: pad < rows");
    o->tiles_x = (unsigned)((u->cols + 31) / 32);
    const int64_t nb = (int64_t)o->tiles_x * ((u->pad + 31) / 32);
    DXA_CHECK_ARG(nb < (1ll << 30), "dxa_split3_pair: operand too large");
    o->nblocks = (unsigned)nb;
  } else {
    DXA_CHECK_ARG(u->cols % 4 == 0 && u->ld % 4 == 0 && (reinterpret_cast<uintptr_t>(u->src) % 16) == 0 &&
                      (reinterpret_cast<uintptr_t>(u->dst) % 8) == 0,
                  "dxa_split3_pair: cols and ld must be multiples of 4 and the buffers 16-byte aligned");
    o->nblocks = (unsigned)dxa_grid1d(u->rows * (u->cols / 4), 256);
  }
  return DXA_OK;
}
}
extern "C" int dxa_split3_pair(const dxa_split3_op* a, const dxa_split3_op* b, dxa_stream_t stream) {
  S3Op oa, ob;
  if (int rc = s3_fill(a, &oa)) return rc;
  if (int rc = s3_fill(b, &ob)) return rc;
  if (oa.nblocks + ob.nblocks == 0) return DXA_OK;
  hipLaunchKernelGGL(split3_pair_k, dim3(oa.nblocks + ob.nblocks), dim3(256), 0, (hipStream_t)stream, oa, ob);
  DXA_CHECK_LAUNCH();
  return DXA_OK;
}
extern "C" int dxa_split3(const float* src, int64_t ld, void* dst, int64_t rows, int64_t cols, int side, dxa_stream_t stream) {
  DXA_CHECK_ARG(rows >= 0 && cols >= 0 && (side == 0 || side == 1), "dxa_split3: bad arguments");
  if (rows == 0 || cols == 0) return DXA_OK;
  DXA_CHECK_ARG(src && dst, "dxa_split3: null buffer");
  DXA_CHECK_ARG(cols % 4 == 0 && ld % 4 == 0 && (reinterpret_cast<uintptr_t>(src) % 16) == 0 &&
                    (reinterpret_cast<uintptr_t>(dst) % 8) == 0,
                "dxa_split3: cols and ld must be multiples of 4 and the buffers 16-byte aligned");
  const dxa_split3_op a = {src, ld, dst, rows, cols, 0, side, 0}, none = {};
  return dxa_split3_pair(&a, &none, stream);
}
extern "C" int dxa_split3_t(const float* src, int64_t ld, void* dst, int64_t R, int64_t C, int64_t Rp, int side,
                            dxa_stream_t stream) {
  DXA_CHECK_ARG(R >= 0 && C >= 0 && Rp >= R && ld >= C && (side == 0 || side == 1), "dxa_split3_t: bad arguments");
  if (Rp == 0 || C == 0) return DXA_OK;
  DXA_CHECK_ARG(src && dst, "dxa_split3_t: null buffer");
  const dxa_split3_op a = {src, ld, dst, R, C, Rp, side, 1}, none = {};
  return dxa_split3_pair(&a, &none, stream);
}

#if defined(DXA_PP3_STAMPS)
extern "C" int dxa_gemm_debug_pp3_stamps(unsigned long long* out) {
  DXA_CHECK_HIP(hipDeviceSynchronize());
  DXA_CHECK_HIP(hipMemcpyFromSymbol(out, HIP_SYMBOL(g_pp3_stamps), sizeof(unsigned long long) * 4));
  return DXA_OK;
}
#endif
```

dexbotic_amd/csrc/gemm_common.h:

```cpp
#pragma once
#include "common.h"

namespace dxa_gemm_detail {
typedef float f32x16_t __attribute__((ext_vector_type(16)));
struct GemmP {
  int64_t M, N, K;
  const char* A; int64_t lda;
  const char* B; int64_t ldb;
  char* C; int64_t ldc;
  const char* bias;
  const char* R; int64_t ldr;
  char* aux;
  const char* G; int64_t ldg;
  float alpha;
  int act, accumulate;
  int nb1, nb2;
  int64_t sA[3], sB[3], sC[3], sR[3], sG[3];
  int tm, tn;
  int vecA, vecB, vecC, vecR, vecG, vecBias;
  int full, tail_r, split_s;
  int group_m;
  char* mirror;
  float* sumsq;
  float* ws;
  int* flags;
  const char* A2; const char* B2; int64_t K2;
  int fuse; int64_t ldaux;
};
}

namespace {
using dxa_gemm_detail::GemmP;
using dxa_gemm_detail::f32x16_t;
typedef uint32_t u32x4n_t __attribute__((ext_vector_type(4)));
typedef uint32_t u32x4_t __attribute__((ext_vector_type(4)));
typedef __attribute__((address_space(3))) void lds_void_t;
constexpr int BM = 128, BN = 128;
constexpr int ROWB = 128;
constexpr int TILE_BYTES = BM * ROWB;

template <typename T> __device__ __forceinline__ void load4(float (&o)[4], const T* p, bool vec, int n_ok);
template <> __device__ __forceinline__ void load4<float>(float (&o)[4], const float* p, bool vec, int n_ok) {
  if (vec && n_ok == 4) {
    const float4 v = *reinterpret_cast<const float4*>(p);
    o[0] = v.x; o[1] = v.y; o[2] = v.z; o[3] = v.w;
  } else {
#pragma unroll
    for (int i = 0; i < 4; ++i) o[i] = i < n_ok ? p[i] : 0.f;
  }
}
template <> __device__ __forceinline__ void load4<bf16_t>(float (&o)[4], const bf16_t* p, bool vec, int n_ok) {
  if (vec && n_ok == 4) {
    const uint2 v = *reinterpret_cast<const uint2*>(p);
    o[0] = __uint_as_float(v.x << 16); o[1] = __uint_as_float(v.x & 0xffff0000u);
    o[2] = __uint_as_float(v.y << 16); o[3] = __uint_as_float(v.y & 0xffff0000u);
  } else {
#pragma unroll
    for (int i = 0; i < 4; ++i) o[i] = i < n_ok ? bf2f(p[i]) : 0.f;
  }
}
template <typename T> __device__ __forceinline__ void store4(T* p, const float (&v)[4], bool vec, int n_ok);
template <> __device__ __forceinline__ void store4<float>(float* p, const float (&v)[4], bool vec, int n_ok) {
  if (vec && n_ok == 4) {
    *reinterpret_cast<float4*>(p) = make_float4(v[0], v[1], v[2], v[3]);
  } else {
#pragma unroll
    for (int i = 0; i < 4; ++i) if (i < n_ok) p[i] = v[i];
  }
}
template <> __device__ __forceinline__ void store4<bf16_t>(bf16_t* p, const float (&v)[4], bool vec, int n_ok) {
  if (vec && n_ok == 4) {
    uint2 o;
    o.x = pack_bf16x2(v[0], v[1]);
    o.y = pack_bf16x2(v[2], v[3]);
    *reinterpret_cast<uint2*>(p) = o;
  } else {
#pragma unroll
    for (int i = 0; i < 4; ++i) if (i < n_ok) p[i] = f2bf(v[i]);
  }
}

template <typename TI, typename TO>
__device__ __forceinline__ void epilogue4(const GemmP& p, TO* C, TO* AUX, const TI* R, const TI* G,
                                          const float (&bv)[4], int64_t m, int64_t n, int n_ok, const float (&a)[4]) {
  float v[4];
#pragma unroll
  for (int r = 0; r < 4; ++r) v[r] = a[r] * p.alpha + bv[r];
  if (AUX) store4<TO>(AUX + m * p.ldc + n, v, p.vecC, n_ok);
  if (G) {
    float g[4];
    load4<TI>(g, G + m * p.ldg + n, p.vecG, n_ok);
#pragma unroll
    for (int r = 0; r < 4; ++r) v[r] *= act_grad(p.act, g[r]);
  } else if (p.act != DXA_ACT_NONE) {
#pragma unroll
    for (int r = 0; r < 4; ++r) v[r] = act_fwd(p.act, v[r]);
  }
  if (R) {
    float rr[4];
    load4<TI>(rr, R + m * p.ldr + n, p.vecR, n_ok);
#pragma unroll
    for (int r = 0; r < 4; ++r) v[r] += rr[r];
  }
  TO* cp = C + m * p.ldc + n;
  if (p.accumulate) {
    float c0[4];
    load4<TO>(c0, cp, p.vecC, n_ok);
#pragma unroll
    for (int r = 0; r < 4; ++r) v[r] += c0[r];
  }
  store4<TO>(cp, v, p.vecC, n_ok);
}

constexpr int NUM_CU_D = 256;

template <int AI, int MF> struct AccL;
template <int AI> struct AccL<AI, 32> { typedef f32x16_t T[AI][2]; };
template <int AI> struct AccL<AI, 16> {
  typedef f32x4_t T[2 * AI][4];
  static __device__ __forceinline__ f32x4_t unit(const T& a, int u) { return a[u >> 2][u & 3]; }
  static __device__ __forceinline__ void add(T& a, int u, const f32x4_t& v) { a[u >> 2][u & 3] += v; }
  static __device__ __forceinline__ void stage16(const T& a, int s, char* slab, int lane) {
    const int r16 = lane & 15, g = lane >> 4;
#pragma unroll
    for (int j = 0; j < 4; ++j) {
      const f32x4_t x = a[s][j];
      *reinterpret_cast<float4*>(slab + r16 * 256 + (((j * 4 + g) ^ r16) << 4)) = make_float4(x[0], x[1], x[2], x[3]);
    }
  }
  template <int RP>
  static __device__ __forceinline__ void stage64(const T& a, int s, char* slab, int lane) {
    const int r16 = lane & 15, g = lane >> 4;
#pragma unroll
    for (int ii = 0; ii < 4; ++ii)
#pragma unroll
      for (int j = 0; j < 4; ++j) {
        const int i = 4 * s + ii;
        if (i >= 2 * AI) continue;
        const f32x4_t x = a[i][j];
        *reinterpret_cast<float4*>(slab + (ii * 16 + r16) * RP + (j * 16 + 4 * g) * 4) = make_float4(x[0], x[1], x[2], x[3]);
      }
  }
};

template <int AI, int MF = 32>
__device__ __forceinline__ bool tile_split_exchange(const GemmP& p, typename AccL<AI, MF>::T& acc, int tid, int split_j, int split_s,
                                                    int tail_i) {
#if defined(__HIP_DEVICE_COMPILE__)
  typedef AccL<AI, MF> L;
  if (split_s > 1) {
    constexpr int SC1 = 16;
    constexpr uint32_t SLOT = 256 * 256 * 4;
    const __amdgpu_buffer_rsrc_t rW = __builtin_amdgcn_make_buffer_rsrc(p.ws, 0, (int)(NUM_CU_D * SLOT), 0x00020000);
    const uint32_t slot0 = (uint32_t)tail_i * (uint32_t)(split_s - 1) * SLOT + (uint32_t)tid * 16u;
    if (split_j < split_s - 1) {
      const uint32_t dst = slot0 + (uint32_t)split_j * SLOT;
      if constexpr (MF == 32) {
#pragma unroll
        for (int i = 0; i < AI; ++i)
#pragma unroll
          for (int j = 0; j < 2; ++j)
#pragma unroll
            for (int q = 0; q < 4; ++q) {
              const f32x4_t v = {acc[i][j][4 * q], acc[i][j][4 * q + 1], acc[i][j][4 * q + 2], acc[i][j][4 * q + 3]};
              __builtin_amdgcn_raw_buffer_store_b128(__builtin_bit_cast(u32x4_t, v), rW, dst + ((i * 2 + j) * 4 + q) * 8192, 0, SC1);
            }
      } else {
#pragma unroll
        for (int u = 0; u < 8 * AI; ++u)
          __builtin_amdgcn_raw_buffer_store_b128(__builtin_bit_cast(u32x4_t, L::unit(acc, u)), rW, dst + u * 8192, 0, SC1);
      }
      asm volatile("s_waitcnt vmcnt(0)" ::: "memory");
      __syncthreads();
      if (tid == 0) __hip_atomic_fetch_add(p.flags + tail_i, 1, __ATOMIC_RELAXED, __HIP_MEMORY_SCOPE_AGENT);
      return false;
    }
    if (tid == 0) {
      while (__hip_atomic_load(p.flags + tail_i, __ATOMIC_RELAXED, __HIP_MEMORY_SCOPE_AGENT) < split_s - 1)
        __builtin_amdgcn_s_sleep(4);
      __hip_atomic_store(p.flags + tail_i, 0, __ATOMIC_RELAXED, __HIP_MEMORY_SCOPE_AGENT);
    }
    __syncthreads();
    for (int sj = 0; sj < split_s - 1; ++sj) {
      const uint32_t src = slot0 + (uint32_t)sj * SLOT;
      if constexpr (MF == 32) {
#pragma unroll
        for (int i = 0; i < AI; ++i) {
#pragma unroll
          for (int j = 0; j < 2; ++j)
#pragma unroll
            for (int q = 0; q < 4; ++q) {
              const f32x4_t v = __builtin_bit_cast(f32x4_t, __builtin_amdgcn_raw_buffer_load_b128(rW, src + ((i * 2 + j) * 4 + q) * 8192, 0, SC1));
#pragma unroll
              for (int c = 0; c < 4; ++c) acc[i][j][4 * q + c] += v[c];
            }
          if (AI == 4 && i == 1) __builtin_amdgcn_sched_barrier(0);
        }
      } else {
#pragma unroll
        for (int u = 0; u < 8 * AI; ++u) {
          L::add(acc, u, __builtin_bit_cast(f32x4_t, __builtin_amdgcn_raw_buffer_load_b128(rW, src + u * 8192, 0, SC1)));
          if (AI == 4 && u == 15) __builtin_amdgcn_sched_barrier(0);
        }
      }
    }
  }

#endif
  return true;
}

template <typename TO, int AI, typename TE, bool SMALL = false, int MF = 32>
__device__ __forceinline__ void tile_finish(const GemmP& p, typename AccL<AI, MF>::T& acc, char* smem, int tid, int lane, int wave,
                                            int wm, int wn, int l32, int lh, int64_t m0, int64_t n0, int split_j,
                                            int split_s, int tail_i) {
#if defined(__HIP_DEVICE_COMPILE__)
  typedef AccL<AI, MF> L;
  constexpr int BMR = AI * 64;
  if (!tile_split_exchange<AI, MF>(p, acc, tid, split_j, split_s, tail_i)) return;

  TO* C = reinterpret_cast<TO*>(p.C);
  TO* AUX = p.aux ? reinterpret_cast<TO*>(p.aux) : nullptr;
  const TE* R = reinterpret_cast<const TE*>(p.R);
  const TE* G = reinterpret_cast<const TE*>(p.G);
  const TE* bias = reinterpret_cast<const TE*>(p.bias);
  const int cr = lane >> 4, cc = (lane & 15) * 4;
  const int64_t n = n0 + wn * 64 + cc;
  const int n_ok = (int)max((int64_t)0, min((int64_t)4, p.N - n));
  float bv[4] = {0.f, 0.f, 0.f, 0.f};
  if (bias && n_ok > 0) load4<TE>(bv, bias + n, p.vecBias, n_ok);
  if constexpr (!SMALL) {
    constexpr int ROWP = 64 * 4 + 16;
    char* slab = smem + wave * (64 * ROWP);
#pragma unroll
    for (int pass = 0; pass < 2; ++pass) {
      if constexpr (MF == 32) {
#pragma unroll
        for (int ii = 0; ii < 2; ++ii)
#pragma unroll
          for (int j = 0; j < 2; ++j)
#pragma unroll
            for (int q = 0; q < 4; ++q) {
              const int i = 2 * pass + ii;
              if (i >= AI) continue;
              float4 v = make_float4(acc[i][j][4 * q], acc[i][j][4 * q + 1], acc[i][j][4 * q + 2], acc[i][j][4 * q + 3]);
              *reinterpret_cast<float4*>(slab + (ii * 32 + l32) * ROWP + (j * 32 + 8 * q + 4 * lh) * 4) = v;
            }
      } else {
        L::template stage64<ROWP>(acc, pass, slab, lane);
      }
      __builtin_amdgcn_fence(__ATOMIC_RELEASE, "wavefront");
      __builtin_amdgcn_wave_barrier();
#pragma unroll 4
      for (int it = 0; it < (AI == 3 && pass == 1 ? 8 : 16); ++it) {
        const int row = cr + 4 * it;
        const int64_t m = m0 + wm * (BMR / 2) + pass * 64 + row;
        const float4 v = *reinterpret_cast<const float4*>(slab + row * ROWP + cc * 4);
        if (m < p.M && n_ok > 0) {
          const float a4[4] = {v.x, v.y, v.z, v.w};
          epilogue4<TE, TO>(p, C, AUX, R, G, bv, m, n, n_ok, a4);
        }
      }
      __builtin_amdgcn_fence(__ATOMIC_RELEASE, "wavefront");
      __builtin_amdgcn_wave_barrier();
    }
  } else {
    char* slab = smem + 131072 + wave * 4096;
    [[maybe_unused]] const int r16 = l32 & 15;
#pragma unroll
    for (int i = 0; i < AI; ++i)
#pragma unroll
      for (int hh = 0; hh < 2; ++hh) {
        if constexpr (MF == 32) {
          if ((l32 >> 4) == hh) {
#pragma unroll
            for (int j = 0; j < 2; ++j)
#pragma unroll
              for (int q = 0; q < 4; ++q) {
                float4 v = make_float4(acc[i][j][4 * q], acc[i][j][4 * q + 1], acc[i][j][4 * q + 2], acc[i][j][4 * q + 3]);
                *reinterpret_cast<float4*>(slab + r16 * 256 + (((j * 8 + 2 * q + lh) ^ r16) << 4)) = v;
              }
          }
        } else {
          L::stage16(acc, 2 * i + hh, slab, lane);
        }
        __builtin_amdgcn_fence(__ATOMIC_RELEASE, "wavefront");
        __builtin_amdgcn_wave_barrier();
#pragma unroll
        for (int it = 0; it < 4; ++it) {
          const int row = cr + 4 * it;
          const int64_t m = m0 + wm * (BMR / 2) + i * 32 + hh * 16 + row;
          const float4 v = *reinterpret_cast<const float4*>(slab + row * 256 + (((lane & 15) ^ row) << 4));
          if (m < p.M && n_ok > 0) {
            const float a4[4] = {v.x, v.y, v.z, v.w};
            epilogue4<TE, TO>(p, C, AUX, R, G, bv, m, n, n_ok, a4);
          }
        }
        __builtin_amdgcn_fence(__ATOMIC_RELEASE, "wavefront");
        __builtin_amdgcn_wave_barrier();
        __builtin_amdgcn_sched_barrier(0);
      }
  }
#endif
}

__device__ __forceinline__ void sk_tile_origin(const GemmP& p, int t, int& m0, int& n0) {
  const int width = p.group_m * p.tn;
  const int group = t / width;
  const int first_pm = group * p.group_m;
  const int gsz = min(p.tm - first_pm, p.group_m);
  const int rem = t - group * width;
  const int pn = rem / gsz;
  m0 = (first_pm + rem - pn * gsz) * 256;
  n0 = pn * 256;
}
template <typename T> struct SkIO;
template <> struct SkIO<float> {
  template <int CPL>
  static __device__ __forceinline__ void ld(float (&o)[CPL], __amdgpu_buffer_rsrc_t r, uint32_t off) {
    static_assert(CPL == 4, "fp32 operands come 4 columns per lane");
    const f32x4_t v = __builtin_bit_cast(f32x4_t, __builtin_amdgcn_raw_buffer_load_b128(r, off, 0, 0));
#pragma unroll
    for (int e = 0; e < 4; ++e) o[e] = v[e];
  }
  template <int CPL>
  static __device__ __forceinline__ void st(const float (&v)[CPL], __amdgpu_buffer_rsrc_t r, uint32_t off) {
    static_assert(CPL == 4, "fp32 outputs go 4 columns per lane");
    const f32x4_t o = {v[0], v[1], v[2], v[3]};
    __builtin_amdgcn_raw_buffer_store_b128(__builtin_bit_cast(u32x4_t, o), r, off, 0, 0);
  }
};
template <> struct SkIO<bf16_t> {
  template <int CPL>
  static __device__ __forceinline__ void ld(float (&o)[CPL], __amdgpu_buffer_rsrc_t r, uint32_t off) {
    if constexpr (CPL == 8) {
      const u32x4_t v = __builtin_amdgcn_raw_buffer_load_b128(r, off, 0, 0);
#pragma unroll
      for (int e = 0; e < 4; ++e) { o[2 * e] = __uint_as_float(v[e] << 16); o[2 * e + 1] = __uint_as_float(v[e] & 0xffff0000u); }
    } else {
      typedef uint32_t u32x2_t __attribute__((ext_vector_type(2)));
      const u32x2_t v = __builtin_amdgcn_raw_buffer_load_b64(r, off, 0, 0);
#pragma unroll
      for (int e = 0; e < 2; ++e) { o[2 * e] = __uint_as_float(v[e] << 16); o[2 * e + 1] = __uint_as_float(v[e] & 0xffff0000u); }
    }
  }
  template <int CPL>
  static __device__ __forceinline__ void st(const float (&v)[CPL], __amdgpu_buffer_rsrc_t r, uint32_t off) {
    static_assert(CPL == 8, "bf16 outputs go 8 columns per lane");
    u32x4_t o;
#pragma unroll
    for (int e = 0; e < 4; ++e) o[e] = pack_bf16x2(v[2 * e], v[2 * e + 1]);
    __builtin_amdgcn_raw_buffer_store_b128(o, r, off, 0, 0);
  }
};

template <typename TO, typename TE, int AI = 4, int MF = 32>
__device__ __forceinline__ float sk_epilogue_rows(const GemmP& p, typename AccL<AI, MF>::T& acc, char* slab, int lane, int wm, int wn,
                                                  int m0, int n0) {
  float ssq = 0.f;
#if defined(__HIP_DEVICE_COMPILE__)
  constexpr int CPL = 16 / (int)sizeof(TO);
  constexpr int LPR = 64 / CPL;
  constexpr int RPI = 64 / LPR;
  [[maybe_unused]] const int l32 = lane & 31, lh = lane >> 5, r16 = l32 & 15;
  const int lr = lane / LPR, lc = (lane % LPR) * CPL;
  const int n = n0 + wn * 64 + lc;
  const int rowb = m0 + wm * (32 * AI) + lr;
  const bool col_ok = n < (int)p.N;
  const uint32_t Mi = (uint32_t)p.M;
  const uint32_t esO = sizeof(TO), esE = sizeof(TE);
  const __amdgpu_buffer_rsrc_t rC = __builtin_amdgcn_make_buffer_rsrc(p.C, 0, (int)(((p.M - 1) * p.ldc + p.N) * esO), 0x00020000);
  const __amdgpu_buffer_rsrc_t rR = __builtin_amdgcn_make_buffer_rsrc(const_cast<char*>(p.R ? p.R : p.A), 0, p.R ? (int)(((p.M - 1) * p.ldr + p.N) * esE) : 0, 0x00020000);
  const uint32_t ldcB = (uint32_t)p.ldc * esO, ldrB = (uint32_t)p.ldr * esE;
  const uint32_t offC0 = (uint32_t)rowb * ldcB + (uint32_t)n * esO;
  const uint32_t offR0 = (uint32_t)rowb * ldrB + (uint32_t)n * esE;
  float bv[CPL];
#pragma unroll
  for (int e = 0; e < CPL; ++e) bv[e] = 0.f;
  if (p.bias && col_ok) {
    const __amdgpu_buffer_rsrc_t rBias = __builtin_amdgcn_make_buffer_rsrc(const_cast<char*>(p.bias), 0, (int)(p.N * esE), 0x00020000);
    SkIO<TE>::template ld<CPL>(bv, rBias, (uint32_t)n * esE);
  }
  const bool has_R = p.R != nullptr, accum = p.accumulate != 0, has_mirror = p.mirror != nullptr;
  const __amdgpu_buffer_rsrc_t rM = __builtin_amdgcn_make_buffer_rsrc(p.mirror ? p.mirror : (char*)p.C, 0,
                                                                      p.mirror ? (int)(((p.M - 1) * p.ldc + p.N) * 2) : 0, 0x00020000);
  const float alpha = p.alpha;
  const bool want_ssq = p.sumsq != nullptr;
#pragma unroll
  for (int i = 0; i < AI; ++i)
#pragma unroll
    for (int hh = 0; hh < 2; ++hh) {
      if constexpr (MF == 32) {
        if ((l32 >> 4) == hh) {
#pragma unroll
          for (int j = 0; j < 2; ++j)
#pragma unroll
            for (int q = 0; q < 4; ++q) {
              float4 v = make_float4(acc[i][j][4 * q], acc[i][j][4 * q + 1], acc[i][j][4 * q + 2], acc[i][j][4 * q + 3]);
              *reinterpret_cast<float4*>(slab + r16 * 256 + (((j * 8 + 2 * q + lh) ^ r16) << 4)) = v;
            }
        }
      } else {
        AccL<AI, MF>::stage16(acc, 2 * i + hh, slab, lane);
      }
      __builtin_amdgcn_fence(__ATOMIC_RELEASE, "wavefront");
      __builtin_amdgcn_wave_barrier();
#pragma unroll
      for (int it = 0; it < 16 / RPI; ++it) {
        const int row = lr + RPI * it;
        const uint32_t rr = (uint32_t)(32 * i + 16 * hh + RPI * it);
        const bool ok = col_ok && (uint32_t)rowb + rr < Mi;
        float v[CPL];
#pragma unroll
        for (int u = 0; u < CPL / 4; ++u) {
          const float4 t = *reinterpret_cast<const float4*>(slab + row * 256 + (((lc / 4 + u) ^ row) << 4));
          v[4 * u] = t.x; v[4 * u + 1] = t.y; v[4 * u + 2] = t.z; v[4 * u + 3] = t.w;
        }
        const uint32_t oc = ok ? offC0 + rr * ldcB : 0x80000000u;
#pragma unroll
        for (int e = 0; e < CPL; ++e) v[e] = v[e] * alpha + bv[e];
        if (has_R) {
          float r[CPL];
          SkIO<TE>::template ld<CPL>(r, rR, ok ? offR0 + rr * ldrB : 0x80000000u);
#pragma unroll
          for (int e = 0; e < CPL; ++e) v[e] += r[e];
        }
        if (accum) {
          float c0[CPL];
          SkIO<TO>::template ld<CPL>(c0, rC, oc);
#pragma unroll
          for (int e = 0; e < CPL; ++e) v[e] += c0[e];
        }
        SkIO<TO>::template st<CPL>(v, rC, oc);
        if constexpr (sizeof(TO) == 2) {
          if (want_ssq && ok) {
#pragma unroll
            for (int e = 0; e < CPL; ++e) { const float t = rnd<bf16_t>(v[e]); ssq += t * t; }
          }
        }
        if constexpr (sizeof(TO) == 4) {
          if (ok) {
#pragma unroll
            for (int e = 0; e < CPL; ++e) ssq += v[e] * v[e];
          }
          if (has_mirror) {
            typedef uint32_t u32x2_t_ __attribute__((ext_vector_type(2)));
            const u32x2_t_ o2 = {pack_bf16x2(v[0], v[1]), pack_bf16x2(v[2], v[3])};
            __builtin_amdgcn_raw_buffer_store_b64(o2, rM, ok ? (offC0 + rr * ldcB) >> 1 : 0x80000000u, 0, 0);
          }
        }
      }
      __builtin_amdgcn_fence(__ATOMIC_RELEASE, "wavefront");
      __builtin_amdgcn_wave_barrier();
      __builtin_amdgcn_sched_barrier(0);
    }
#endif
  return ssq;
}
template <int AI = 4, int MF = 32>
__device__ __forceinline__ void sk_epilogue_swiglu(const GemmP& p, typename AccL<AI, MF>::T& acc, char* slab, int lane, int wm, int wn,
                                                   int m0, int n0) {
#if defined(__HIP_DEVICE_COMPILE__)
  [[maybe_unused]] const int l32 = lane & 31, lh = lane >> 5, r16 = l32 & 15;
  const int lr = lane >> 3, lq = lane & 7;
  const int F = (int)(p.N >> 1);
  const int nout = (n0 >> 1) + wn * 32 + lq * 4;
  const int rowb = m0 + wm * (32 * AI) + lr;
  const bool col_ok = nout < F;
  const uint32_t Mi = (uint32_t)p.M;
  const __amdgpu_buffer_rsrc_t rC = __builtin_amdgcn_make_buffer_rsrc(p.C, 0, (int)(((p.M - 1) * p.ldc + F) * 2), 0x00020000);
  const __amdgpu_buffer_rsrc_t rX = __builtin_amdgcn_make_buffer_rsrc(p.aux ? p.aux : p.C, 0,
                                                                      p.aux ? (int)(((p.M - 1) * p.ldaux + p.N) * 2) : 0, 0x00020000);
  const uint32_t ldcB = (uint32_t)p.ldc * 2u, ldxB = (uint32_t)p.ldaux * 2u;
  const uint32_t offC0 = (uint32_t)rowb * ldcB + (uint32_t)nout * 2u;
  const uint32_t offG0 = (uint32_t)rowb * ldxB + (uint32_t)nout * 2u, offU0 = offG0 + (uint32_t)F * 2u;
  const bool has_aux = p.aux != nullptr;
  const float alpha = p.alpha;
  typedef uint32_t u32x2_t_ __attribute__((ext_vector_type(2)));
#pragma unroll
  for (int i = 0; i < AI; ++i)
#pragma unroll
    for (int hh = 0; hh < 2; ++hh) {
      if constexpr (MF == 32) {
        if ((l32 >> 4) == hh) {
#pragma unroll
          for (int j = 0; j < 2; ++j)
#pragma unroll
            for (int q = 0; q < 4; ++q) {
              float4 v = make_float4(acc[i][j][4 * q], acc[i][j][4 * q + 1], acc[i][j][4 * q + 2], acc[i][j][4 * q + 3]);
              *reinterpret_cast<float4*>(slab + r16 * 256 + (((j * 8 + 2 * q + lh) ^ r16) << 4)) = v;
            }
        }
      } else {
        AccL<AI, MF>::stage16(acc, 2 * i + hh, slab, lane);
      }
      __builtin_amdgcn_fence(__ATOMIC_RELEASE, "wavefront");
      __builtin_amdgcn_wave_barrier();
#pragma unroll
      for (int it = 0; it < 2; ++it) {
        const int row = lr + 8 * it;
        const uint32_t rr = (uint32_t)(32 * i + 16 * hh + 8 * it);
        const bool ok = col_ok && (uint32_t)rowb + rr < Mi;
        const float4 g4 = *reinterpret_cast<const float4*>(slab + row * 256 + ((lq ^ row) << 4));
        const float4 u4 = *reinterpret_cast<const float4*>(slab + row * 256 + (((8 + lq) ^ row) << 4));
        const float g[4] = {rnd<bf16_t>(g4.x * alpha + 0.f), rnd<bf16_t>(g4.y * alpha + 0.f), rnd<bf16_t>(g4.z * alpha + 0.f), rnd<bf16_t>(g4.w * alpha + 0.f)};
        const float u[4] = {rnd<bf16_t>(u4.x * alpha + 0.f), rnd<bf16_t>(u4.y * alpha + 0.f), rnd<bf16_t>(u4.z * alpha + 0.f), rnd<bf16_t>(u4.w * alpha + 0.f)};
        float o[4];
#pragma unroll
        for (int e = 0; e < 4; ++e) {
          o[e] = rnd<bf16_t>(g[e] * fast_sigmoidf(g[e])) * u[e];
        }
        const u32x2_t_ ov = {pack_bf16x2(o[0], o[1]), pack_bf16x2(o[2], o[3])};
        __builtin_amdgcn_raw_buffer_store_b64(ov, rC, ok ? offC0 + rr * ldcB : 0x80000000u, 0, 0);
        if (has_aux) {
          const u32x2_t_ gv = {pack_bf16x2(g[0], g[1]), pack_bf16x2(g[2], g[3])};
          const u32x2_t_ uv = {pack_bf16x2(u[0], u[1]), pack_bf16x2(u[2], u[3])};
          __builtin_amdgcn_raw_buffer_store_b64(gv, rX, ok ? offG0 + rr * ldxB : 0x80000000u, 0, 0);
          __builtin_amdgcn_raw_buffer_store_b64(uv, rX, ok ? offU0 + rr * ldxB : 0x80000000u, 0, 0);
        }
      }
      __builtin_amdgcn_fence(__ATOMIC_RELEASE, "wavefront");
      __builtin_amdgcn_wave_barrier();
      __builtin_amdgcn_sched_barrier(0);
    }
#endif
}
template <typename TO, typename TE, int AI = 4, int MF = 32>
__device__ __forceinline__ void sk_epilogue(const GemmP& p, typename AccL<AI, MF>::T& acc, char* slab, int lane, int wm, int wn,
                                            int m0, int n0, float* red, int tile) {
#if defined(__HIP_DEVICE_COMPILE__)
  float ssq = sk_epilogue_rows<TO, TE, AI, MF>(p, acc, slab, lane, wm, wn, m0, n0);
  {
    if (p.sumsq != nullptr) {
#pragma unroll
      for (int o = 32; o > 0; o >>= 1) ssq += __shfl_xor(ssq, o, 64);
      if (lane == 0) red[wm * 4 + wn] = ssq;
      __syncthreads();
      if (threadIdx.x == 0) {
        float t = 0.f;
#pragma unroll
        for (int w8 = 0; w8 < 8; ++w8) t += red[w8];
        p.sumsq[tile] = t;
      }
    }
  }
#endif
}
}
```

dexbotic_amd/kernels.py:

```python
from __future__ import annotations

import contextlib
import ctypes as C
from typing import Optional, Sequence, Tuple

import torch

from . import _lib as L
from ._lib import lib

F32, BF16 = L.F32, L.BF16


def dt(t: torch.Tensor) -> int:
    if t.dtype == torch.float32:
        return F32
    if t.dtype == torch.bfloat16:
        return BF16
    raise L.DxaError(f"unsupported dtype {t.dtype} (fp32 / bf16 only)")


def torch_dtype(code: int) -> torch.dtype:
    return torch.bfloat16 if code == BF16 else torch.float32


_raw_stream = getattr(torch._C, "_cuda_getCurrentRawStream", None)
_cur_device = getattr(torch._C, "_cuda_getDevice", None)


def _stream() -> int:
    if _raw_stream is not None and _cur_device is not None:
        return _raw_stream(_cur_device())
    return torch.cuda.current_stream().cuda_stream


def _ptr(t: Optional[torch.Tensor]) -> Optional[int]:
    if t is None:
        return None
    if not t.is_cuda:
        raise L.DxaError("dexbotic_amd kernels need device tensors (no CPU fallback exists)")
    return t.data_ptr()


def _row_major(t: torch.Tensor, name: str) -> int:
    if t.dim() != 2 or (t.shape[1] > 1 and t.stride(1) != 1):
        raise L.DxaError(f"{name}: expected a 2-D tensor with contiguous rows, got shape {tuple(t.shape)} "
                         f"strides {t.stride()}")
    return t.stride(0) if t.shape[0] > 1 else max(t.shape[1], t.stride(0))


F32_GEMM_MODE = "exact"


@contextlib.contextmanager
def f32_gemm_mode(mode: str):
    global F32_GEMM_MODE
    if mode not in ("exact", "bf16x3"):
        raise L.DxaError(f"unknown fp32 GEMM mode {mode!r}")
    prev, F32_GEMM_MODE = F32_GEMM_MODE, mode
    try:
        yield
    finally:
        F32_GEMM_MODE = prev


def split3(x: torch.Tensor, rows: int, cols: int, ld: int, side: int) -> torch.Tensor:
    out = torch.empty((rows, 3 * cols), device=x.device, dtype=torch.bfloat16)
    L.check(lib.dxa_split3(_ptr(x), ld, _ptr(out), rows, cols, side, _stream()), "dxa_split3")
    return out


def split3_t(x: torch.Tensor, pad_to: int, side: int) -> torch.Tensor:
    R, C_ = x.shape
    Rp = (R + pad_to - 1) // pad_to * pad_to
    out = torch.empty((C_, 3 * Rp), device=x.device, dtype=torch.bfloat16)
    L.check(lib.dxa_split3_t(_ptr(x), _row_major(x, "x"), _ptr(out), R, C_, Rp, side, _stream()), "dxa_split3_t")
    return out


def split3_pair(a: torch.Tensor, a_t: bool, b: torch.Tensor, b_t: bool, pad_to: int = 1, a_dims=None, b_dims=None
                ) -> Tuple[torch.Tensor, torch.Tensor]:
    ops, outs = [], []
    for x, t, side, dims in ((a, a_t, 0, a_dims), (b, b_t, 1, b_dims)):
        R, C_, ld = dims if dims is not None else (x.shape[0], x.shape[1], _row_major(x, "x"))
        o = L.Split3Op()
        o.src, o.ld, o.rows, o.cols, o.side, o.transposed = _ptr(x), ld, R, C_, side, int(t)
        if t:
            Rp = (R + pad_to - 1) // pad_to * pad_to
            out = torch.empty((C_, 3 * Rp), device=x.device, dtype=torch.bfloat16)
            o.pad = Rp
        else:
            out = torch.empty((R, 3 * C_), device=x.device, dtype=torch.bfloat16)
            o.pad = 0
        o.dst = _ptr(out)
        ops.append(o)
        outs.append(out)
    L.check(lib.dxa_split3_pair(C.byref(ops[0]), C.byref(ops[1]), _stream()), "dxa_split3_pair")
    return outs[0], outs[1]


def _x3_t_ok(M: int, N: int, Kc: int, out: torch.Tensor) -> bool:
    return (F32_GEMM_MODE == "bf16x3" and out.dtype == torch.float32 and M >= 128 and N >= 128 and Kc >= 64 and Kc % 32 == 0
            and 6 * max(M, N) * Kc < (1 << 31))


def mm_tn_f32(a: torch.Tensor, b: torch.Tensor, *, out: torch.Tensor, **kw) -> torch.Tensor:
    Kc, M = a.shape
    N = b.shape[1]
    if a.dtype == torch.float32 and b.dtype == torch.float32 and _x3_t_ok(M, N, (Kc + 31) // 32 * 32, out):
        a3, b3 = split3_pair(a, True, b, True, pad_to=32)
        Kp = a3.shape[1] // 3
        kw = _ld_kwargs(kw, out)
        return gemm(L.NT, a3, b3, M, N, 3 * Kp, 3 * Kp, 3 * Kp, out, _row_major(out, "out"), epi_f32=True, **kw)
    return mm_nt(transpose(a, 4), transpose(b, 4), out=out, **kw)


def mm_nn_f32(a: torch.Tensor, b: torch.Tensor, **kw) -> torch.Tensor:
    M, Kc = a.shape
    N = b.shape[1]
    out = kw.get("out")
    if (a.dtype == torch.float32 and b.dtype == torch.float32 and Kc % 32 == 0 and a.is_contiguous() and a.data_ptr() % 16 == 0
            and Kc % 4 == 0 and (out is None or out.dtype == torch.float32)):
        if out is None:
            out = kw["out"] = torch.empty((M, N), device=a.device, dtype=torch.float32)
        if _x3_t_ok(M, N, Kc, out):
            a3, b3 = split3_pair(a, False, b, True)
            kw2 = _ld_kwargs({k: v for k, v in kw.items() if k != "out"}, out)
            return gemm(L.NT, a3, b3, M, N, 3 * Kc, 3 * Kc, 3 * Kc, out, _row_major(out, "out"), epi_f32=True, **kw2)
    return mm_nt(a, transpose(b, 1), **kw)


def _x3_eligible(layout, a, b, out, M, N, K, lda, ldb, nb) -> bool:
    return (F32_GEMM_MODE == "bf16x3" and layout == L.NT and a.dtype == torch.float32 and b.dtype == torch.float32
            and out.dtype == torch.float32 and tuple(nb) == (1, 1, 1) and M >= 128 and N >= 128 and K >= 64 and K % 32 == 0
            and lda % 4 == 0 and ldb % 4 == 0 and a.data_ptr() % 16 == 0 and b.data_ptr() % 16 == 0
            and 6 * max(M, N) * K < (1 << 31))


_NB1 = (1, 1, 1)


def gemm(layout: int, a: torch.Tensor, b: torch.Tensor, M: int, N: int, K: int, lda: int, ldb: int,
         out: torch.Tensor, ldc: int, *, bias: Optional[torch.Tensor] = None,
         residual: Optional[torch.Tensor] = None, ldr: int = 0, act: int = L.ACT_NONE,
         aux_out: Optional[torch.Tensor] = None, mulgrad: Optional[torch.Tensor] = None, ldg: int = 0,
         alpha: float = 1.0, accumulate: bool = False, nb: Sequence[int] = _NB1,
         sA: Sequence[int] = (0, 0, 0), sB: Sequence[int] = (0, 0, 0), sC: Sequence[int] = (0, 0, 0),
         sR: Sequence[int] = (0, 0, 0), sG: Sequence[int] = (0, 0, 0), epi_f32: bool = False,
         mirror: Optional[torch.Tensor] = None, sumsq: Optional[torch.Tensor] = None,
         a2: Optional[torch.Tensor] = None, b2: Optional[torch.Tensor] = None) -> torch.Tensor:
    if not epi_f32 and a2 is None and _x3_eligible(layout, a, b, out, M, N, K, lda, ldb, nb):
        a3, b3 = split3_pair(a, False, b, False, a_dims=(M, K, lda), b_dims=(N, K, ldb))
        return gemm(L.NT, a3, b3, M, N, 3 * K, 3 * K, 3 * K, out, ldc, bias=bias, residual=residual, ldr=ldr, act=act,
                    aux_out=aux_out, mulgrad=mulgrad, ldg=ldg, alpha=alpha, accumulate=accumulate, epi_f32=True,
                    mirror=mirror, sumsq=sumsq)
    d = L.GemmDesc()
    d.layout, d.in_dtype, d.out_dtype, d.act = layout, dt(a), dt(out), act
    d.epi_f32 = int(epi_f32)
    if dt(b) != d.in_dtype:
        raise L.DxaError("gemm: A and B dtypes differ")
    for t, n in ((bias, "bias"), (residual, "residual"), (mulgrad, "mulgrad")):
        if t is not None and dt(t) != (F32 if epi_f32 else d.in_dtype):
            raise L.DxaError(f"gemm: {n} dtype must equal the input dtype")
    if aux_out is not None and dt(aux_out) != d.out_dtype:
        raise L.DxaError("gemm: aux_out dtype must equal the output dtype")
    d.M, d.N, d.K = M, N, K
    d.A, d.lda, d.B, d.ldb, d.C, d.ldc = _ptr(a), lda, _ptr(b), ldb, _ptr(out), ldc
    d.bias, d.residual, d.ldr = _ptr(bias), _ptr(residual), ldr
    d.aux_out, d.mulgrad, d.ldg = _ptr(aux_out), _ptr(mulgrad), ldg
    d.alpha, d.accumulate = alpha, int(accumulate)
    if mirror is not None:
        if mirror.dtype != torch.bfloat16 or out.dtype != torch.float32 or tuple(nb) != (1, 1, 1) or \
                _row_major(mirror, "mirror") != ldc:
            raise L.DxaError("gemm: mirror must be a bf16 [M, N] view with the output's leading dimension (fp32 output)")
        d.mirror = _ptr(mirror)
    if sumsq is not None:
        if sumsq.dtype != torch.float32 or tuple(nb) != (1, 1, 1) or not sumsq.is_contiguous() \
                or sumsq.numel() != gemm_sumsq_slots(M, N):
            raise L.DxaError("gemm: sumsq must be gemm_sumsq_slots(M, N) contiguous floats (unbatched output)")
        d.sumsq = _ptr(sumsq)
    if nb is _NB1 or tuple(nb) == (1, 1, 1):
        d.nb[0] = d.nb[1] = d.nb[2] = 1
    else:
        for i in range(3):
            d.nb[i], d.sA[i], d.sB[i], d.sC[i], d.sR[i], d.sG[i] = nb[i], sA[i], sB[i], sC[i], sR[i], sG[i]
    K_all = K
    if a2 is not None:
        if layout != L.TN or b2 is None or a2.shape[1] != M or b2.shape[1] != N or a2.shape[0] != b2.shape[0] \
                or dt(a2) != d.in_dtype or dt(b2) != d.in_dtype or _row_major(a2, "a2") != lda or _row_major(b2, "b2") != ldb:
            raise L.DxaError("gemm: a2 / b2 are a second [K2, M] / [K2, N] pair of a TN product (same dtypes and leading dimensions)")
        d.A2, d.B2, d.K2 = _ptr(a2), _ptr(b2), a2.shape[0]
        K_all = K + a2.shape[0]
    prof = GEMM_PROFILE
    if prof is not None and prof.wants(layout, d.in_dtype, d.out_dtype):
        e0, e1 = torch.cuda.Event(enable_timing=True), torch.cuda.Event(enable_timing=True)
        e0.record()
        L.check(lib.dxa_gemm(C.byref(d), _stream()), "dxa_gemm")
        e1.record()
        batches = nb[0] * nb[1] * nb[2]
        esz = {L.BF16: 2, L.F32: 4}
        prof.add((layout, d.in_dtype, d.out_dtype), e0, e1, 2.0 * M * N * K_all * batches,
                 float((M * K_all + N * K_all) * esz.get(d.in_dtype, 2) + M * N * esz.get(d.out_dtype, 2)) * batches)
        return out
    L.check(lib.dxa_gemm(C.byref(d), _stream()), "dxa_gemm")
    return out


class GemmProfile:

    def __init__(self, *keys, stride: int = 1):
        if len(keys) == 3 and all(isinstance(k, int) for k in keys):
            keys = (tuple(keys),)
        self.keys = set(tuple(k) for k in keys)
        self.events = []
        self.stride = max(1, int(stride))
        self.seen = {k: 0 for k in self.keys}

    def wants(self, layout, in_dtype, out_dtype) -> bool:
        key = (layout, in_dtype, out_dtype)
        if key not in self.keys:
            return False
        n = self.seen[key]
        self.seen[key] = n + 1
        return n % self.stride == 0

    def add(self, key, e0, e1, flops: float, nbytes: float = 0.0) -> None:
        self.events.append((key, e0, e1, flops, nbytes))

    def summary(self, key=None):
        ev = [e for e in self.events if key is None or e[0] == tuple(key)]
        ms = sum(a.elapsed_time(b) for _, a, b, _, _ in ev)
        return len(ev), ms, sum(e[3] for e in ev), sum(e[4] for e in ev)

    def launches(self, key=None) -> int:
        return self.seen[tuple(key)] if key is not None else sum(self.seen.values())


GEMM_PROFILE: Optional[GemmProfile] = None


def _out2d(M: int, N: int, like: torch.Tensor, out: Optional[torch.Tensor], out_dtype: Optional[torch.dtype]):
    if out is None:
        out = torch.empty((M, N), device=like.device, dtype=out_dtype or like.dtype)
    return out


def mm_nt(a: torch.Tensor, b: torch.Tensor, *, out=None, out_dtype=None, **kw) -> torch.Tensor:
    M, K = a.shape
    N = b.shape[0]
    assert b.shape[1] == K, (a.shape, b.shape)
    out = _out2d(M, N, a, out, out_dtype)
    kw = _ld_kwargs(kw, out)
    return gemm(L.NT, a, b, M, N, K, _row_major(a, "a"), _row_major(b, "b"), out, _row_major(out, "out"), **kw)


def mm_nn(a: torch.Tensor, b: torch.Tensor, *, out=None, out_dtype=None, **kw) -> torch.Tensor:
    M, K = a.shape
    N = b.shape[1]
    assert b.shape[0] == K, (a.shape, b.shape)
    out = _out2d(M, N, a, out, out_dtype)
    kw = _ld_kwargs(kw, out)
    return gemm(L.NN, a, b, M, N, K, _row_major(a, "a"), _row_major(b, "b"), out, _row_major(out, "out"), **kw)


def mm_tn(a: torch.Tensor, b: torch.Tensor, *, out=None, out_dtype=None, **kw) -> torch.Tensor:
    K, M = a.shape
    N = b.shape[1]
    assert b.shape[0] == K, (a.shape, b.shape)
    out = _out2d(M, N, a, out, out_dtype)
    kw = _ld_kwargs(kw, out)
    return gemm(L.TN, a, b, M, N, K, _row_major(a, "a"), _row_major(b, "b"), out, _row_major(out, "out"), **kw)


def swiglu_gemm_supported(x: torch.Tensor, w: torch.Tensor, keep_pre: bool = False) -> bool:
    if keep_pre:
        return False
    M, K_ = x.shape
    F_ = w.shape[0] // 2
    return (x.dtype == torch.bfloat16 and w.dtype == torch.bfloat16 and x.is_cuda and
            M >= 129 and K_ % 64 == 0 and K_ >= 64 and F_ % 8 == 0 and F_ >= 128 and w.shape[0] % 2 == 0 and
            x.is_contiguous() and w.is_contiguous() and x.data_ptr() % 16 == 0 and w.data_ptr() % 16 == 0 and
            M * 2 * F_ * 2 < (1 << 31) and w.numel() * 2 < (1 << 31))


def mm_nt_swiglu(x: torch.Tensor, w: torch.Tensor, keep_pre: bool = True):
    M, K_ = x.shape
    N = w.shape[0]
    F_ = N // 2
    out = torch.empty((M, F_), device=x.device, dtype=x.dtype)
    pre = torch.empty((M, N), device=x.device, dtype=x.dtype) if keep_pre else None
    d = L.GemmDesc()
    d.layout, d.in_dtype, d.out_dtype, d.act = L.NT, L.BF16, L.BF16, L.ACT_NONE
    d.M, d.N, d.K = M, N, K_
    d.A, d.lda, d.B, d.ldb, d.C, d.ldc = _ptr(x), K_, _ptr(w), K_, _ptr(out), F_
    d.aux_out, d.ld_aux = _ptr(pre), N
    d.alpha, d.fuse = 1.0, L.FUSE_SWIGLU
    for i in range(3):
        d.nb[i] = 1
    prof = GEMM_PROFILE
    if prof is not None and prof.wants(L.NT, L.BF16, L.BF16):
        e0, e1 = torch.cuda.Event(enable_timing=True), torch.cuda.Event(enable_timing=True)
        e0.record()
        L.check(lib.dxa_gemm(C.byref(d), _stream()), "dxa_gemm (swiglu)")
        e1.record()
        prof.add((L.NT, L.BF16, L.BF16), e0, e1, 2.0 * M * N * K_, float((M * K_ + N * K_) * 2 + M * (N + F_) * 2))
        return out, pre
    L.check(lib.dxa_gemm(C.byref(d), _stream()), "dxa_gemm (swiglu)")
    return out, pre


def _ld_kwargs(kw: dict, out: torch.Tensor) -> dict:
    kw = dict(kw)
    if kw.get("residual") is not None:
        kw["ldr"] = _row_major(kw["residual"], "residual")
    if kw.get("mulgrad") is not None:
        kw["ldg"] = _row_major(kw["mulgrad"], "mulgrad")
    if kw.get("aux_out") is not None and _row_major(kw["aux_out"], "aux_out") != _row_major(out, "out"):
        raise L.DxaError("gemm: aux_out must share the output leading dimension")
    return kw


_MASK_STATE = {"seed": None, "offset": 0}


def dropout_mask(shape, p: float, dtype: torch.dtype, device, seed: Optional[int] = None) -> torch.Tensor:
    n = 1
    for v in shape:
        n *= int(v)
    out = torch.empty(tuple(int(v) for v in shape), device=device, dtype=dtype)
    if _MASK_STATE["seed"] is None or seed is not None:
        _MASK_STATE["seed"] = int(torch.initial_seed() if seed is None else seed) & 0xFFFFFFFFFFFFFFFF
    _MASK_STATE["offset"] += 1
    L.check(lib.dxa_dropout_mask(_ptr(out), n, float(p), _MASK_STATE["seed"], _MASK_STATE["offset"], dt(out), _stream()),
            "dxa_dropout_mask")
    return out


def bank_consolidate(feat: torch.Tensor, ts: torch.Tensor, length: int, sims: torch.Tensor, fifo: bool = False) -> None:
    assert feat.is_contiguous() and ts.is_contiguous() and ts.dtype == torch.float32 and sims.dtype == torch.float32
    assert feat.dim() == 3 and length <= feat.shape[0] and sims.numel() >= length - 1
    L.check(lib.dxa_bank_consolidate(_ptr(feat), _ptr(ts), int(length), feat.shape[1], feat.shape[2], dt(feat), int(fifo),
                                     _ptr(sims), _stream()), "dxa_bank_consolidate")


def add_rows(x: Optional[torch.Tensor], g: torch.Tensor, Nn: int, alpha: float = 1.0) -> torch.Tensor:
    R, C_ = g.shape
    assert g.is_contiguous() and (x is None or (x.is_contiguous() and x.shape == (R, Nn, C_) and x.dtype == g.dtype))
    out = torch.empty((R, Nn, C_), device=g.device, dtype=g.dtype)
    L.check(lib.dxa_add_rows(_ptr(x), _ptr(g), _ptr(out), R, Nn, C_, float(alpha), dt(g), _stream()), "dxa_add_rows")
    return out


def token_sum(x: torch.Tensor, scale: float = 1.0) -> torch.Tensor:
    R, Nn, C_ = x.shape
    assert x.is_contiguous()
    out = torch.empty((R, C_), device=x.device, dtype=x.dtype)
    L.check(lib.dxa_token_sum(_ptr(x), _ptr(out), R, Nn, C_, float(scale), dt(x), _stream()), "dxa_token_sum")
    return out


def rmsnorm_fwd(x: torch.Tensor, w: Optional[torch.Tensor], eps: float) -> Tuple[torch.Tensor, torch.Tensor]:
    x2 = x.reshape(-1, x.shape[-1])
    assert x2.is_contiguous()
    y = torch.empty_like(x2)
    rstd = torch.empty(x2.shape[0], device=x.device, dtype=torch.float32)
    L.check(lib.dxa_rmsnorm_fwd(_ptr(x2), _ptr(w), _ptr(y), _ptr(rstd), x2.shape[0], x2.shape[1], eps, dt(x2),
                                dt(w) if w is not None else dt(x2), _stream()), "dxa_rmsnorm_fwd")
    return y.view(x.shape), rstd


def norm_bwd_blocks(rows: int) -> int:
    return int(lib.dxa_norm_bwd_blocks(rows))


def _residual2d(residual, x2):
    if residual is None:
        return None
    r2 = residual.reshape(-1, x2.shape[-1])
    assert r2.is_contiguous() and r2.shape == x2.shape and r2.dtype == x2.dtype
    return r2


def rmsnorm_bwd(dy, x, w, rstd, dw_out: Optional[torch.Tensor] = None, accumulate: bool = False,
                want_dw: bool = True, residual: Optional[torch.Tensor] = None) -> Tuple[torch.Tensor, Optional[torch.Tensor]]:
    x2 = x.reshape(-1, x.shape[-1])
    dy2 = dy.reshape(-1, x.shape[-1])
    assert x2.is_contiguous() and dy2.is_contiguous()
    rows, cols = x2.shape
    dx = torch.empty_like(x2)
    part = None
    if w is not None and want_dw:
        part = torch.empty((norm_bwd_blocks(rows), cols), device=x.device, dtype=torch.float32)
    if w is not None and part is None:
        part = torch.empty((norm_bwd_blocks(rows), cols), device=x.device, dtype=torch.float32)
        want_dw = False
    L.check(lib.dxa_rmsnorm_bwd(_ptr(dy2), _ptr(x2), _ptr(w), _ptr(rstd), _ptr(dx), _ptr(_residual2d(residual, x2)), _ptr(part),
                                rows, cols, dt(x2),
                                dt(w) if w is not None else dt(x2), _stream()), "dxa_rmsnorm_bwd")
    dw = colsum(part, out=dw_out, accumulate=accumulate) if (part is not None and want_dw) else None
    return dx.view(x.shape), dw


def layernorm_fwd(x, w, b, eps):
    x2 = x.reshape(-1, x.shape[-1])
    assert x2.is_contiguous()
    y = torch.empty_like(x2)
    mean = torch.empty(x2.shape[0], device=x.device, dtype=torch.float32)
    rstd = torch.empty_like(mean)
    L.check(lib.dxa_layernorm_fwd(_ptr(x2), _ptr(w), _ptr(b), _ptr(y), _ptr(mean), _ptr(rstd), x2.shape[0],
                                  x2.shape[1], eps, dt(x2), dt(w) if w is not None else dt(x2), _stream()),
            "dxa_layernorm_fwd")
    return y.view(x.shape), mean, rstd


def layernorm_bwd(dy, x, w, mean, rstd, dw_out=None, db_out=None, accumulate: bool = False, want_dw: bool = True,
                  residual: Optional[torch.Tensor] = None, return_part: bool = False):
    x2 = x.reshape(-1, x.shape[-1])
    dy2 = dy.reshape(-1, x.shape[-1])
    assert x2.is_contiguous() and dy2.is_contiguous()
    rows, cols = x2.shape
    dx = torch.empty_like(x2)
    part = None
    if w is not None:
        part = torch.empty((norm_bwd_blocks(rows), 2 * cols), device=x.device, dtype=torch.float32)
    L.check(lib.dxa_layernorm_bwd(_ptr(dy2), _ptr(x2), _ptr(w), _ptr(mean), _ptr(rstd), _ptr(dx),
                                  _ptr(_residual2d(residual, x2)), _ptr(part), rows, cols, dt(x2), dt(w) if w is not None else dt(x2), _stream()), "dxa_layernorm_bwd")
    if return_part:
        return dx.view(x.shape), part
    if part is None or not want_dw:
        return dx.view(x.shape), None, None
    if dw_out is not None:
        if db_out is not None and db_out.data_ptr() == dw_out.data_ptr() + 4 * cols:
            both = torch.as_strided(dw_out, (2 * cols,), (1,))
            colsum(part, out=both, accumulate=accumulate)
        else:
            colsum(part[:, :cols], out=dw_out, accumulate=accumulate)
            colsum(part[:, cols:], out=db_out, accumulate=accumulate)
        return dx.view(x.shape), dw_out, db_out
    s = colsum(part)
    return dx.view(x.shape), s[:cols], s[cols:]


def downsample_grid(n_tokens: int) -> Tuple[int, int]:
    G = int(round(n_tokens ** 0.5))
    if G * G != n_tokens or G < 1:
        raise L.DxaError(f"downsample: {n_tokens} tokens per image are not a square grid")
    return G, (G + 1) // 2


def downsample_layernorm_fwd(x, w, b, eps):
    assert x.dim() == 3 and x.is_contiguous()
    N, T, C_ = x.shape
    G, h = downsample_grid(T)
    y = torch.empty((N, h * h, 4 * C_), device=x.device, dtype=x.dtype)
    mean = torch.empty(N * h * h, device=x.device, dtype=torch.float32)
    rstd = torch.empty_like(mean)
    L.check(lib.dxa_downsample_layernorm_fwd(_ptr(x), _ptr(w), _ptr(b), _ptr(y), _ptr(mean), _ptr(rstd), N, G, C_, eps, dt(x),
                                             dt(w) if w is not None else dt(x), _stream()), "dxa_downsample_layernorm_fwd")
    return y, mean, rstd


def downsample_layernorm_bwd(dy, x, w, mean, rstd, out: Optional[torch.Tensor] = None):
    assert x.dim() == 3 and x.is_contiguous()
    N, T, C_ = x.shape
    G, h = downsample_grid(T)
    dy2 = dy.reshape(N * h * h, 4 * C_)
    assert dy2.is_contiguous() and dy2.dtype == x.dtype
    dx = torch.empty_like(x) if out is None else out
    assert dx.shape == x.shape and dx.dtype == x.dtype and dx.is_contiguous()
    part = None
    if w is not None:
        part = torch.empty((norm_bwd_blocks(N * h * h), 8 * C_), device=x.device, dtype=torch.float32)
    L.check(lib.dxa_downsample_layernorm_bwd(_ptr(dy2), _ptr(x), _ptr(w), _ptr(mean), _ptr(rstd), _ptr(dx), _ptr(part), N, G, C_,
                                             dt(x), dt(w) if w is not None else dt(x), _stream()), "dxa_downsample_layernorm_bwd")
    return dx, part


def colsum(x: torch.Tensor, out: Optional[torch.Tensor] = None, accumulate: bool = False) -> torch.Tensor:
    ld = _row_major(x, "x")
    rows, cols = x.shape
    if out is None:
        out = torch.empty(cols, device=x.device, dtype=torch.float32)
        accumulate = False
    nsplit = max(1, min(64, (rows + 31) // 32))
    scratch = torch.empty(nsplit * cols, device=x.device, dtype=torch.float32)
    L.check(lib.dxa_colsum(_ptr(x), ld, _ptr(out), rows, cols, dt(x), int(accumulate), _ptr(scratch),
                           scratch.numel() * 4, _stream()), "dxa_colsum")
    return out


def rope_split(qkv: torch.Tensor, cos_t, sin_t, pos, B, S, Hq, Hkv, D, k_out=None, v_out=None):
    assert qkv.is_contiguous() and qkv.shape == (B * S, (Hq + 2 * Hkv) * D)
    q = torch.empty((B, Hq, S, D), device=qkv.device, dtype=qkv.dtype)
    k = torch.empty((B, Hkv, S, D), device=qkv.device, dtype=qkv.dtype) if k_out is None else k_out
    v = torch.empty((B, Hkv, S, D), device=qkv.device, dtype=qkv.dtype) if v_out is None else v_out
    assert k.is_contiguous() and v.is_contiguous() and k.shape == (B, Hkv, S, D) == v.shape and k.dtype == qkv.dtype == v.dtype
    L.check(lib.dxa_rope_split(_ptr(qkv), _ptr(q), _ptr(k), _ptr(v), _ptr(cos_t), _ptr(sin_t), _ptr(pos), B, S, Hq,
                               Hkv, D, dt(qkv), _stream()), "dxa_rope_split")
    return q, k, v


def rope_split_into(qkv: torch.Tensor, q: torch.Tensor, k: torch.Tensor, v: torch.Tensor, s0: int, cos_t, sin_t, pos, B, S, Hq, Hkv, D) -> None:
    S_cap = q.shape[2]
    assert qkv.is_contiguous() and qkv.shape == (B * S, (Hq + 2 * Hkv) * D)
    assert q.is_contiguous() and k.is_contiguous() and v.is_contiguous() and q.shape == (B, Hq, S_cap, D) and \
        k.shape == (B, Hkv, S_cap, D) == v.shape and q.dtype == k.dtype == v.dtype == qkv.dtype
    L.check(lib.dxa_rope_split_at(_ptr(qkv), _ptr(q), _ptr(k), _ptr(v), _ptr(cos_t), _ptr(sin_t), _ptr(pos), B, S, Hq, Hkv, D,
                                  S_cap, s0, dt(qkv), _stream()), "dxa_rope_split_at")


def rope_merge_from(dq, dk, dv, s0: int, cos_t, sin_t, pos, B, S, Hq, Hkv, D):
    S_cap = dq.shape[2]
    assert dq.is_contiguous() and dk.is_contiguous() and dv.is_contiguous() and dq.shape == (B, Hq, S_cap, D)
    dqkv = torch.empty((B * S, (Hq + 2 * Hkv) * D), device=dq.device, dtype=dq.dtype)
    L.check(lib.dxa_rope_merge_at(_ptr(dq), _ptr(dk), _ptr(dv), _ptr(dqkv), _ptr(cos_t), _ptr(sin_t), _ptr(pos), B, S, Hq, Hkv, D,
                                  S_cap, s0, dt(dq), _stream()), "dxa_rope_merge_at")
    return dqkv


def rope_merge(dq, dk, dv, cos_t, sin_t, pos, B, S, Hq, Hkv, D):
    assert dq.is_contiguous() and dk.is_contiguous() and dv.is_contiguous()
    dqkv = torch.empty((B * S, (Hq + 2 * Hkv) * D), device=dq.device, dtype=dq.dtype)
    L.check(lib.dxa_rope_merge(_ptr(dq), _ptr(dk), _ptr(dv), _ptr(dqkv), _ptr(cos_t), _ptr(sin_t), _ptr(pos), B, S,
                               Hq, Hkv, D, dt(dq), _stream()), "dxa_rope_merge")
    return dqkv


QKNORM_HEAD_DIMS = (32, 64, 128, 256)


def qknorm_rope_split(qkv: torch.Tensor, q_norm_w: torch.Tensor, k_norm_w: torch.Tensor, eps: float, cos_t, sin_t, pos, B, S, Hq, Hkv,
                      D, want_rstd: bool = True):
    assert qkv.is_contiguous() and qkv.shape == (B * S, (Hq + 2 * Hkv) * D)
    assert q_norm_w.dtype == qkv.dtype == k_norm_w.dtype and q_norm_w.numel() == D == k_norm_w.numel()
    q = torch.empty((B, Hq, S, D), device=qkv.device, dtype=qkv.dtype)
    k = torch.empty((B, Hkv, S, D), device=qkv.device, dtype=qkv.dtype)
    v = torch.empty((B, Hkv, S, D), device=qkv.device, dtype=qkv.dtype)
    rstd = torch.empty((B * S, Hq + Hkv), device=qkv.device, dtype=torch.float32) if want_rstd else None
    L.check(lib.dxa_qknorm_rope_split(_ptr(qkv), _ptr(q), _ptr(k), _ptr(v), _ptr(q_norm_w), _ptr(k_norm_w), float(eps), _ptr(rstd),
                                      _ptr(cos_t), _ptr(sin_t), _ptr(pos), B, S, Hq, Hkv, D, dt(qkv), _stream()),
            "dxa_qknorm_rope_split")
    return q, k, v, rstd


def qknorm_rope_merge(dq, dk, dv, qkv: torch.Tensor, rstd: torch.Tensor, q_norm_w, k_norm_w, cos_t, sin_t, pos, B, S, Hq, Hkv, D,
                      want_dw: bool = True):
    assert dq.is_contiguous() and dk.is_contiguous() and dv.is_contiguous() and qkv.is_contiguous() and rstd.is_contiguous()
    assert qkv.shape == (B * S, (Hq + 2 * Hkv) * D) and dq.shape == (B, Hq, S, D) and dk.shape == (B, Hkv, S, D) == dv.shape
    assert dq.dtype == dk.dtype == dv.dtype == qkv.dtype == q_norm_w.dtype == k_norm_w.dtype
    assert rstd.shape == (B * S, Hq + Hkv) and rstd.dtype == torch.float32
    dqkv = torch.empty_like(qkv)
    part = None
    if want_dw:
        nblk = int(lib.dxa_qknorm_rope_merge_blocks(B * S, Hq, Hkv, D, dt(qkv)))
        if nblk < 0:
            L.check(nblk, "dxa_qknorm_rope_merge_blocks")
        part = torch.empty((nblk, 2 * D), device=qkv.device, dtype=torch.float32)
    L.check(lib.dxa_qknorm_rope_merge(_ptr(dq), _ptr(dk), _ptr(dv), _ptr(qkv), _ptr(rstd), _ptr(q_norm_w), _ptr(k_norm_w), _ptr(dqkv),
                                      _ptr(part), _ptr(cos_t), _ptr(sin_t), _ptr(pos), B, S, Hq, Hkv, D, dt(qkv), _stream()),
            "dxa_qknorm_rope_merge")
    return dqkv, part


def _bhsd_strides(t: torch.Tensor) -> Tuple[int, int, int]:
    assert t.dim() == 4 and (t.shape[3] == 1 or t.stride(3) == 1), (t.shape, t.stride())
    return t.stride(0), t.stride(1), t.stride(2)


def _attn_desc(q, k, v, o, lse, causal, scale, kv_start, kv_end, q_limit=None, key_valid=None, drop_mask=None) -> L.AttnDesc:
    d = L.AttnDesc()
    B, Hq, Sq, D = q.shape
    _, Hkv, Sk, _ = k.shape
    d.dtype, d.B, d.Hq, d.Hkv, d.Sq, d.Sk, d.D = dt(q), B, Hq, Hkv, Sq, Sk, D
    d.causal, d.scale = int(causal), scale
    d.q, (d.q_sb, d.q_sh, d.q_ss) = _ptr(q), _bhsd_strides(q)
    d.k, (d.k_sb, d.k_sh, d.k_ss) = _ptr(k), _bhsd_strides(k)
    d.v, (d.v_sb, d.v_sh, d.v_ss) = _ptr(v), _bhsd_strides(v)
    d.o, (d.o_sb, d.o_sh, d.o_ss) = _ptr(o), _bhsd_strides(o)
    d.lse, d.kv_start, d.kv_end = _ptr(lse), _ptr(kv_start), _ptr(kv_end)
    if q_limit is not None:
        assert q_limit.dtype == torch.int32 and q_limit.is_contiguous() and q_limit.shape == (B, Sq)
    if key_valid is not None:
        assert key_valid.dtype == torch.uint8 and key_valid.is_contiguous() and key_valid.shape == (B, Sk)
    d.q_limit, d.key_valid = _ptr(q_limit), _ptr(key_valid)
    if drop_mask is not None:
        assert drop_mask.dtype == q.dtype and drop_mask.is_contiguous() and drop_mask.shape == (B, Hq, Sq, Sk)
        d.drop_mask = _ptr(drop_mask)
    return d


def attn_fwd(q, k, v, o, *, causal: bool, scale: float, kv_start=None, kv_end=None, force_generic=False,
             q_limit=None, key_valid=None, drop_mask=None):
    B, Hq, Sq, _ = q.shape
    lse = torch.empty((B, Hq, Sq), device=q.device, dtype=torch.float32)
    d = _attn_desc(q, k, v, o, lse, causal, scale, kv_start, kv_end, q_limit, key_valid, drop_mask)
    d.force_generic = int(force_generic)
    nbytes = int(lib.dxa_attn_fwd_workspace(C.byref(d)))
    if nbytes:
        ws = torch.empty(nbytes, device=q.device, dtype=torch.uint8)
# ... 614 lines not shown
```

include/dexbotic_amd.h:

```cpp
#ifndef DEXBOTIC_AMD_H_
#define DEXBOTIC_AMD_H_

#include <stddef.h>
#include <stdint.h>

#ifdef __cplusplus
extern "C" {
#endif

typedef void* dxa_stream_t;

enum dxa_status { DXA_OK = 0, DXA_ERR_BAD_ARG = -1, DXA_ERR_UNSUPPORTED = -2, DXA_ERR_HIP = -3 };
enum dxa_dtype { DXA_F32 = 0, DXA_BF16 = 1 };
enum dxa_act {
  DXA_ACT_NONE = 0,
  DXA_ACT_GELU_ERF = 1,
  DXA_ACT_GELU_TANH = 2,
  DXA_ACT_QUICK_GELU = 3,
  DXA_ACT_SILU = 4,
  DXA_ACT_RELU = 5,
  DXA_ACT_SIGMOID = 6
};
enum dxa_layout {
  DXA_NT = 0,
  DXA_NN = 1,
  DXA_TN = 2
};

const char* dxa_last_error(void);
int dxa_version(void);

enum dxa_fuse { DXA_FUSE_NONE = 0, DXA_FUSE_SWIGLU = 1 };
typedef struct dxa_gemm_desc {
  int32_t layout;
  int32_t in_dtype;
  int32_t out_dtype;
  int32_t act;
  int64_t M, N, K;
  const void* A;
  int64_t lda;
  const void* B;
  int64_t ldb;
  void* C;
  int64_t ldc;
  const void* bias;
  const void* residual;
  int64_t ldr;
  void* aux_out;
  const void* mulgrad;
  int64_t ldg;
  float alpha;
  int32_t accumulate;
  int32_t nb[3];
  int64_t sA[3], sB[3], sC[3], sR[3], sG[3];
  int32_t epi_f32;
  void* mirror;
  float* sumsq;
  const void* A2;
  const void* B2;
  int64_t K2;
  int32_t fuse;
  int64_t ld_aux;
} dxa_gemm_desc;
int dxa_gemm(const dxa_gemm_desc* d, dxa_stream_t stream);
int64_t dxa_gemm_sumsq_slots(int64_t M, int64_t N);
typedef struct dxa_gemm_step_info {
  const char* kernel;
  int32_t grid[3], block, lds;
  int64_t K, K2;
  int64_t a_off, b_off;
  int32_t seg2;
  int32_t accumulate, bias, residual;
  int32_t tm, tn, full, tail_r, split_s, group_m;
  int32_t vecA, vecB, vecC, vecR, vecG, vecBias;
  int32_t ksplit, kper;
  int32_t split_ws;
  int32_t mirror, sumsq;
} dxa_gemm_step_info;
typedef struct dxa_gemm_plan_info {
  int32_t nsteps;
  int32_t mirror_pass, sumsq_pass;
  dxa_gemm_step_info step[2];
} dxa_gemm_plan_info;
int dxa_gemm_plan(const dxa_gemm_desc* d, dxa_gemm_plan_info* out);
const char* dxa_gemm_kernel_name(int i);

int dxa_split3(const float* src, int64_t ld, void* dst, int64_t rows, int64_t cols, int side, dxa_stream_t stream);
int dxa_split3_t(const float* src, int64_t ld, void* dst, int64_t R, int64_t C, int64_t Rp, int side, dxa_stream_t stream);
typedef struct dxa_split3_op {
  const float* src;
  int64_t ld;
  void* dst;
  int64_t rows, cols, pad;
  int32_t side;
  int32_t transposed;
} dxa_split3_op;
int dxa_split3_pair(const dxa_split3_op* a, const dxa_split3_op* b, dxa_stream_t stream);

int dxa_rmsnorm_fwd(const void* x, const void* w, void* y, float* rstd, int64_t rows, int64_t cols,
                    float eps, int dtype, int w_dtype, dxa_stream_t stream);
int dxa_rmsnorm_bwd(const void* dy, const void* x, const void* w, const float* rstd, void* dx,
                    const void* residual, float* partial_dw, int64_t rows, int64_t cols, int dtype, int w_dtype,
                    dxa_stream_t stream);
int dxa_layernorm_fwd(const void* x, const void* w, const void* b, void* y, float* mean, float* rstd,
                      int64_t rows, int64_t cols, float eps, int dtype, int w_dtype, dxa_stream_t stream);
int dxa_layernorm_bwd(const void* dy, const void* x, const void* w, const float* mean, const float* rstd,
                      void* dx, const void* residual, float* partial_dwdb, int64_t rows, int64_t cols, int dtype,
                      int w_dtype, dxa_stream_t stream);
int dxa_norm_bwd_blocks(int64_t rows);
int dxa_downsample_layernorm_fwd(const void* x, const void* w, const void* b, void* y, float* mean, float* rstd,
                                 int64_t N, int64_t G, int64_t C, float eps, int dtype, int w_dtype, dxa_stream_t stream);
int dxa_downsample_layernorm_bwd(const void* dy, const void* x, const void* w, const float* mean, const float* rstd,
                                 void* dx, float* partial_dwdb, int64_t N, int64_t G, int64_t C, int dtype, int w_dtype,
                                 dxa_stream_t stream);
int dxa_colsum(const void* x, int64_t ld, float* out, int64_t rows, int64_t cols, int dtype,
               int accumulate, float* scratch, size_t scratch_bytes, dxa_stream_t stream);

int dxa_rope_split(const void* qkv, void* q, void* k, void* v, const float* cos_t, const float* sin_t,
                   const int32_t* pos, int B, int S, int Hq, int Hkv, int D, int dtype,
                   dxa_stream_t stream);
int dxa_rope_merge(const void* dq, const void* dk, const void* dv, void* dqkv, const float* cos_t,
                   const float* sin_t, const int32_t* pos, int B, int S, int Hq, int Hkv, int D,
                   int dtype, dxa_stream_t stream);
int dxa_rope_split_at(const void* qkv, void* q, void* k, void* v, const float* cos_t, const float* sin_t, const int32_t* pos, int B,
                      int S, int Hq, int Hkv, int D, int S_cap, int s0, int dtype, dxa_stream_t stream);
int dxa_rope_merge_at(const void* dq, const void* dk, const void* dv, void* dqkv, const float* cos_t, const float* sin_t,
                      const int32_t* pos, int B, int S, int Hq, int Hkv, int D, int S_cap, int s0, int dtype, dxa_stream_t stream);
int dxa_qknorm_rope_split(const void* qkv, void* q, void* k, void* v, const void* q_norm_w, const void* k_norm_w, float eps,
                          float* rstd, const float* cos_t, const float* sin_t, const int32_t* pos, int B, int S, int Hq, int Hkv,
                          int D, int dtype, dxa_stream_t stream);
int dxa_qknorm_rope_merge(const void* dq, const void* dk, const void* dv, const void* qkv, const float* rstd,
                          const void* q_norm_w, const void* k_norm_w, void* dqkv, float* partial_dw, const float* cos_t,
                          const float* sin_t, const int32_t* pos, int B, int S, int Hq, int Hkv, int D, int dtype,
                          dxa_stream_t stream);
int dxa_qknorm_rope_merge_blocks(int64_t tokens, int Hq, int Hkv, int D, int dtype);

typedef struct dxa_attn_desc {
  int32_t dtype;
  int32_t B, Hq, Hkv, Sq, Sk, D;
  int32_t causal;
  float scale;
  const void* q; int64_t q_sb, q_sh, q_ss;
  const void* k; int64_t k_sb, k_sh, k_ss;
  const void* v; int64_t v_sb, v_sh, v_ss;
  void* o;       int64_t o_sb, o_sh, o_ss;
  float* lse;
  const int32_t* kv_start;
  const int32_t* kv_end;
  const void* d_o; int64_t do_sb, do_sh, do_ss;
  void* dq; int64_t dq_sb, dq_sh, dq_ss;
  void* dk; int64_t dk_sb, dk_sh, dk_ss;
  void* dv; int64_t dv_sb, dv_sh, dv_ss;
  int32_t force_generic;
  const int32_t* q_limit;
  const uint8_t* key_valid;
  const void* drop_mask;
} dxa_attn_desc;
int dxa_attn_fwd(const dxa_attn_desc* d, dxa_stream_t stream);
size_t dxa_attn_fwd_workspace(const dxa_attn_desc* d);
int dxa_attn_fwd_ws(const dxa_attn_desc* d, void* workspace, size_t workspace_bytes, dxa_stream_t stream);
size_t dxa_attn_bwd_workspace(const dxa_attn_desc* d);
int dxa_attn_bwd(const dxa_attn_desc* d, void* workspace, size_t workspace_bytes, dxa_stream_t stream);

int dxa_swiglu_fwd(const void* gu, void* out, int64_t rows, int64_t F, int dtype, dxa_stream_t stream);
int dxa_swiglu_bwd(const void* gu, const void* dout, void* dgu, int64_t rows, int64_t F, int dtype,
                   dxa_stream_t stream);
int dxa_glu_fwd(const void* gu, void* out, int64_t rows, int64_t F, int act, int dtype, dxa_stream_t stream);
int dxa_glu_bwd(const void* gu, const void* dout, void* dgu, int64_t rows, int64_t F, int act, int dtype,
                dxa_stream_t stream);
int dxa_axpby(const void* a, const void* b, void* out, int64_t n, float alpha, float beta, int dtype, dxa_stream_t stream);
int dxa_mul(const void* a, const void* b, void* out, int64_t n, int dtype, dxa_stream_t stream);
int dxa_mul_rows(const void* x, const void* g, void* out, int64_t R, int64_t Nn, int64_t C, int dtype, dxa_stream_t stream);
int dxa_act_fwd(const void* x, void* y, int64_t n, int act, int dtype, dxa_stream_t stream);
int dxa_act_bwd(const void* x, const void* dy, void* dx, int64_t n, int act, int dtype, dxa_stream_t stream);
int dxa_add(const void* a, const void* b, void* out, int64_t n, int dtype, dxa_stream_t stream);
int dxa_cast(const void* src, void* dst, int64_t n, int src_dtype, int dst_dtype, dxa_stream_t stream);
int dxa_copy2d(const void* src, int64_t lds, void* dst, int64_t ldd, int64_t rows, int64_t cols,
               int64_t cols_padded, int src_dtype, int dst_dtype, dxa_stream_t stream);

int dxa_transpose(const void* src, int64_t ld_src, void* dst, int64_t ld_dst, int64_t R, int64_t C,
                  int64_t R_padded, int dtype, dxa_stream_t stream);
int dxa_permute_bshd(const void* src, void* dst, int B, int S, int H, int D, int to_head, int dtype,
                     dxa_stream_t stream);

int dxa_splice_fwd(const int64_t* plan, const void* embed, const void* img, void* out, int64_t n_rows,
                   int64_t d, int dtype, dxa_stream_t stream);
int dxa_splice_bwd(const int64_t* plan, const void* dout, float* d_embed, void* d_img, int64_t n_rows,
                   int64_t d, int dtype, dxa_stream_t stream);
int dxa_zero_rows(const int64_t* plan, float* g, int64_t n_rows, int64_t d, dxa_stream_t stream);
int dxa_gather_rows(const void* x, const int64_t* idx, void* out, int64_t n, int64_t d, int src_dtype,
                    int dst_dtype, dxa_stream_t stream);
int dxa_scatter_rows(const void* dout, const int64_t* idx, void* dx, int64_t n, int64_t R, int64_t d,
                     int src_dtype, int dst_dtype, dxa_stream_t stream);

int dxa_im2col(const void* images, void* rows, int N, int H, int W, int P, int64_t ld, int img_dtype,
               int dtype, dxa_stream_t stream);
int dxa_vit_embed_fwd(const void* patch, const void* cls, const void* pos, void* x, int N, int np, int C,
                      int dtype, int w_dtype, dxa_stream_t stream);
int dxa_vit_embed_bwd(const void* dx, void* dpatch, int N, int np, int C, int dtype, dxa_stream_t stream);

int dxa_qsample(const float* x0, const float* noise, const float* a, const float* s, float* xt,
                int64_t N, int64_t per, dxa_stream_t stream);
int dxa_timestep_embedding(const float* t, const float* freqs, float* out, int64_t N, int half,
                           dxa_stream_t stream);
int dxa_dit_assemble_fwd(const float* xe, const float* te, const float* ze, const float* pos, float* h,
                         int N, int T, int hd, dxa_stream_t stream);
int dxa_dit_assemble_bwd(const float* dh, float* dxe, float* dc, int N, int T, int hd, dxa_stream_t stream);
int dxa_token_drop(const float* z, const float* uncond, const uint8_t* drop, float* out, int64_t N,
                   int64_t d, dxa_stream_t stream);
int dxa_token_drop_bwd(const float* dout, const uint8_t* drop, float* dz, float* duncond, int64_t N,
                       int64_t d, int accumulate, dxa_stream_t stream);
int dxa_dropout_mask(void* out, int64_t n, float p, uint64_t seed, uint64_t offset, int dtype, dxa_stream_t stream);
int dxa_bank_consolidate(void* feat, float* ts, int len, int64_t N, int64_t D, int dtype, int fifo, float* sims,
                         dxa_stream_t stream);
int dxa_add_rows(const void* x, const void* g, void* out, int64_t R, int64_t Nn, int64_t C, float alpha, int dtype,
                 dxa_stream_t stream);
int dxa_token_sum(const void* x, void* out, int64_t R, int64_t Nn, int64_t C, float scale, int dtype, dxa_stream_t stream);
int dxa_mse_loss(const float* pred, const float* target, float* loss, float* dpred, int64_t n,
                 float gscale, dxa_stream_t stream);
int dxa_mse_loss_rows(const float* pred, const float* target, const float* row_w, float* loss, float* dpred,
                      int64_t rows, int64_t cols, float gscale, dxa_stream_t stream);
int dxa_ddim_step(float* x, const float* model_out, int64_t B, int64_t per, int use_cfg, float cfg_scale,
                  float c_recip, float c_recipm1, float ab_prev, dxa_stream_t stream);

typedef struct dxa_adamw_desc {
  float* p; const void* g; float* m; float* v;
  uint16_t* shadow;
  const int64_t* chunk_start; const int32_t* chunk_len; const int32_t* chunk_grp; int32_t n_chunks;
  float lr[8]; float wd[8];
  float beta1, beta2, eps;
  float bc1, bc2;
  const float* clip_coef;
  int32_t g_dtype;
  uint8_t* chunk_state;
  const int64_t* chunk_mv_start;
} dxa_adamw_desc;
int dxa_adamw(const dxa_adamw_desc* d, dxa_stream_t stream);
int dxa_sumsq(const void* x, int64_t n, int dtype, double* scratch, float* out, int accumulate, dxa_stream_t stream);
int dxa_sumsq_ranges(const void* base, int dtype, const int64_t* starts, const int64_t* lens, int n_ranges, double* scratch,
                     float* out, int accumulate, dxa_stream_t stream);
int dxa_sum_f32(const float* x, int64_t n, float* out, int accumulate, dxa_stream_t stream);
int dxa_clip_coef(const float* sumsq, float max_norm, float* norm_out, float* coef_out, dxa_stream_t stream);
int dxa_clip_coef_scaled(const float* sumsq, float max_norm, float grad_scale, float* norm_out, float* coef_out,
                         dxa_stream_t stream);
int dxa_scale(float* x, int64_t n, float s, dxa_stream_t stream);
int dxa_scale_dev(float* x, int64_t n, const float* s, dxa_stream_t stream);

int dxa_cross_entropy_fwd(const void* logits, int64_t ld, const int64_t* labels, float* row_loss, float* lse,
                          int64_t rows, int64_t V, int64_t ignore_index, int dtype, dxa_stream_t stream);
int dxa_cross_entropy_bwd(const void* logits, int64_t ld, const int64_t* labels, const float* lse,
                          const float* gscale, float scale, void* dlogits, int64_t ldd, int64_t rows, int64_t V,
                          int64_t ignore_index, int dtype, dxa_stream_t stream);
int dxa_argmax_rows(const void* x, int64_t ld, int64_t* out, int64_t rows, int64_t cols, int dtype,
                    dxa_stream_t stream);
int dxa_sample_rows(const void* logits, int64_t ld, int64_t rows, int64_t V, int dtype, float temperature, int64_t top_k,
                    float top_p, const float* u, int64_t* token, int32_t* kept, float* thresh, float* prob,
                    dxa_stream_t stream);
int dxa_soft_cross_entropy_fwd(const void* logits, int64_t ld, const int64_t* labels, float* row_loss, float* lse,
                               int64_t rows, int64_t V, int64_t ignore_index, const int64_t* soft_ids,
                               const int64_t* soft_ids_host, int K, float inv2s2, int dtype, dxa_stream_t stream);
int dxa_soft_cross_entropy_bwd(const void* logits, int64_t ld, const int64_t* labels, const float* lse,
                               const float* gscale, float scale, void* dlogits, int64_t ldd, int64_t rows, int64_t V,
                               int64_t ignore_index, const int64_t* soft_ids, const int64_t* soft_ids_host, int K,
                               float inv2s2, int dtype, dxa_stream_t stream);

#define DXA_FILTER_BICUBIC 3
typedef struct dxa_image_desc {
  const void* src;
  int n, h, w;
  int pad;
  unsigned char bg[4];
  int res_h, res_w;
  int crop_top, crop_left, out_h, out_w;
  int row0, rows;
  const int32_t *hb, *hk;
  int hks;
  const int32_t *vb, *vk;
  int vks;
  void* tmp;
  void* out;
  int out_dtype;
  void* out_u8;
  double rescale;
  float mean[3], std[3];
} dxa_image_desc;
int dxa_resample_ksize(int in_size, int out_size);
int dxa_resample_coeffs(int in_size, int out_size, int filter, int32_t* bounds, int32_t* kk);
int dxa_image_preprocess(const dxa_image_desc* d, dxa_stream_t stream);

size_t dxa_dit_blocks_workspace(int M, int H, int I);
int dxa_dit_blocks_fwd(float* h, const float* const* weights, int depth, int N, int T1, int H, int heads, int I, float eps,
                       void* workspace, size_t workspace_bytes, dxa_stream_t stream);
size_t dxa_dit_sample_workspace(int M, int H, int I);
int dxa_dit_sample_fwd(float* x, const float* z_emb, const float* t_emb, const float* pos, const float* x_w, const float* x_b,
                       const float* final_w, const float* final_b, const float* coef, int steps, int A, int nb, int use_cfg,
                       float cfg_scale, const float* const* weights, int depth, int N, int T1, int H, int heads, int I, float eps,
                       void* workspace, size_t workspace_bytes, dxa_stream_t stream);
int dxa_dit_blocks_status(dxa_stream_t stream, int* timed_out);

size_t dxa_dit_bf16_pack_bytes(int depth, int H, int I);
int dxa_dit_bf16_pack(const float* const* weights, int depth, int H, int I, void* packed, size_t packed_bytes, const void** table,
                      dxa_stream_t stream);
size_t dxa_dit_sample_bf16_workspace(int M, int H, int I);
int dxa_dit_sample_bf16_fwd(float* x, const float* z_emb, const float* t_emb, const float* pos, const float* x_w, const float* x_b,
                            const float* final_w, const float* final_b, const float* coef, int steps, int A, int nb, int use_cfg,
                            float cfg_scale, const void* const* packed_table, int depth, int N, int T1, int H, int heads, int I,
                            float eps, void* workspace, size_t workspace_bytes, dxa_stream_t stream);

size_t dxa_dit_bf16_pack_per_bytes(int depth, int H, int I);
int dxa_dit_bf16_pack_per(const float* const* weights, int depth, int H, int I, void* packed, size_t packed_bytes, const void** table,
                          dxa_stream_t stream);
int dxa_dit_sample_bf16_per_fwd(float* x, const float* z_emb, const float* t_emb, const float* pos, const float* x_w, const float* x_b,
                                const float* final_w, const float* final_b, const float* coef, int steps, int A, int nb, int use_cfg,
                                float cfg_scale, const void* const* packed_table, const float* per_kv, int P, int depth, int N, int T1,
                                int H, int heads, int I, float eps, void* workspace, size_t workspace_bytes, dxa_stream_t stream);

typedef struct dxa_decode_desc {
  const void* const* layers;
  const void* x_in; void* out; const void* final_norm_w;
  const float* cos_row; const float* sin_row;
  void* workspace; size_t workspace_bytes;
  int32_t n_layers, d, Hq, Hkv, D, F, slot, kv_lo, max_len;
  float eps;
} dxa_decode_desc;
size_t dxa_decode_step_workspace(int d, int Hq, int Hkv, int D, int F);
int dxa_decode_step(const dxa_decode_desc* desc, dxa_stream_t stream);
int dxa_decode_status(dxa_stream_t stream, int* timed_out);

#ifdef __cplusplus
}
#endif
#endif
```

Baseline: 70.59 episodes/s.

## Make ping-pong GEMM persistent with next-tile prefetch and vectorized epilogue

Turns the ping-pong bf16 GEMM into a persistent kernel: the grid is capped at the CU count and each workgroup loops over tiles. In the lean and SwiGLU paths it issues the next tile's first DMA before running the current tile's epilogue, so loads overlap the stores. It also adds a fast vectorized 16-byte row epilogue in tile_finish for aligned bf16 outputs, batching residual, grad and accumulate loads. The cost is higher register pressure, extra loop control and barriers, and a new descriptor field that changes the ABI.

```diff
diff --git a/dexbotic_amd/_lib.py b/dexbotic_amd/_lib.py
--- a/dexbotic_amd/_lib.py
+++ b/dexbotic_amd/_lib.py
@@ -33,6 +33,7 @@
         ("epi_f32", _i32), ("mirror", _vp), ("sumsq", _vp),
         ("A2", _vp), ("B2", _vp), ("K2", _i64),
         ("fuse", _i32), ("ld_aux", _i64),
+        ("max_workgroups", _i32),
     ]
 
 
diff --git a/dexbotic_amd/csrc/gemm.hip b/dexbotic_amd/csrc/gemm.hip
--- a/dexbotic_amd/csrc/gemm.hip
+++ b/dexbotic_amd/csrc/gemm.hip
@@ -841,23 +841,11 @@
   const int tid = threadIdx.x, lane = tid & 63;
   const int wave = __builtin_amdgcn_readfirstlane(tid >> 6);
   const int wm = wave >> 2, wn = wave & 3;
-  const int l32 = lane & 31, lh = lane >> 5;
-
-  int bid = blockIdx.x;
-  int split_j = 0, split_s = 1, tail_i = 0;
-  if (bid < p.full) {
-    const int q = p.full >> 3, r = p.full & 7, xcd = bid & 7;
-    bid = (xcd < r ? xcd * (q + 1) : r * (q + 1) + (xcd - r) * q) + (bid >> 3);
-  } else {
-    const int idx = bid - p.full;
-    tail_i = idx % p.tail_r;
-    split_j = idx / p.tail_r;
-    split_s = p.split_s;
-    bid = p.full + tail_i;
-  }
-  int m0i, n0i;
-  sk_tile_origin(p, bid, m0i, n0i);
-  const int64_t m0 = m0i, n0 = n0i;
+  [[maybe_unused]] const int l32 = lane & 31, lh = lane >> 5;
+
+  int bid, split_j, split_s, tail_i, m0i, n0i;
+  int k_lo, nk;
+  uint32_t voA[2][2], voB[2][2];
 
   const uint32_t bytesA = (uint32_t)((A_KS ? (p.K - 1) * p.lda + p.M : (p.M - 1) * p.lda + p.K) * 2);
   const uint32_t bytesB = (uint32_t)((B_KS ? (p.K - 1) * p.ldb + p.N : (p.N - 1) * p.ldb + p.K) * 2);
@@ -865,16 +853,31 @@
   const __amdgpu_buffer_rsrc_t rB = __builtin_amdgcn_make_buffer_rsrc(const_cast<char*>(p.B), 0, bytesB, 0x00020000);
 #define PP_A_ROW0(h, j) ((((wave * 2 + (j)) & 7) * 8) + (((wave * 2 + (j)) >> 3) * 128) + 64 * (h))
 #define PP_B_ROW0(h, j) ((((wave * 2 + (j)) >> 2) * 64) + (((wave * 2 + (j)) & 3) * 8) + 32 * (h))
-  uint32_t voA[2][2], voB[2][2];
-  {
-    const int lrow = lane >> 3, lslot = lane & 7;
+  const int nk1 = (int)((p.K + 63) >> 6);
+  const int nk_tot = nk1 + ((A_KS && B_KS) ? (int)((p.K2 + 63) >> 6) : 0);
+  auto set_tile = [&](const GemmP& p, int v, int ln) {
+    bid = v; split_j = 0; split_s = 1; tail_i = 0;
+    if (bid < p.full) {
+      const int q = p.full >> 3, r = p.full & 7, xcd = bid & 7;
+      bid = (xcd < r ? xcd * (q + 1) : r * (q + 1) + (xcd - r) * q) + (bid >> 3);
+    } else {
+      const int idx = bid - p.full;
+      tail_i = idx % p.tail_r;
+      split_j = idx / p.tail_r;
+      split_s = p.split_s;
+      bid = p.full + tail_i;
+    }
+    sk_tile_origin(p, bid, m0i, n0i);
+    k_lo = split_j * nk_tot / split_s;
+    nk = (split_j + 1) * nk_tot / split_s - k_lo;
+    const int lrow = ln >> 3, lslot = ln & 7;
     const uint32_t lda2 = (uint32_t)p.lda * 2u, ldb2 = (uint32_t)p.ldb * 2u;
 #pragma unroll
     for (int h = 0; h < 2; ++h)
 #pragma unroll
       for (int j = 0; j < 2; ++j) {
-        const int krow = (wave * 2 + j) * 4 + (lane >> 4);
-        const int sig = (lane & 15) ^ ((krow & 3) << 2) ^ (((krow >> 3) & 1) << 1);
+        const int krow = (wave * 2 + j) * 4 + (ln >> 4);
+        const int sig = (ln & 15) ^ ((krow & 3) << 2) ^ (((krow >> 3) & 1) << 1);
         if constexpr (A_KS) {
           const int ga = m0i + (sig >> 3) * 128 + 64 * h + 8 * (sig & 7);
           voA[h][j] = ga < (int)p.M ? (uint32_t)krow * lda2 + (uint32_t)ga * 2u : 0x80000000u;
@@ -894,16 +897,12 @@
           voB[h][j] = gb < (int)p.N ? (uint32_t)gb * ldb2 + (uint32_t)((lslot ^ ((rb >> 1) & 7)) << 4) : 0x80000000u;
         }
       }
-  }
-  const int nk1 = (int)((p.K + 63) >> 6);
-  const int nk_tot = nk1 + ((A_KS && B_KS) ? (int)((p.K2 + 63) >> 6) : 0);
+  };
   const bool seg2 = (A_KS && B_KS) && p.K2 > 0;
   const __amdgpu_buffer_rsrc_t rA2 = __builtin_amdgcn_make_buffer_rsrc(
       const_cast<char*>(seg2 ? p.A2 : p.A), 0, seg2 ? (uint32_t)(((p.K2 - 1) * p.lda + p.M) * 2) : 0u, 0x00020000);
   const __amdgpu_buffer_rsrc_t rB2 = __builtin_amdgcn_make_buffer_rsrc(
       const_cast<char*>(seg2 ? p.B2 : p.B), 0, seg2 ? (uint32_t)(((p.K2 - 1) * p.ldb + p.N) * 2) : 0u, 0x00020000);
-  const int k_lo = split_j * nk_tot / split_s;
-  const int nk = (split_j + 1) * nk_tot / split_s - k_lo;
   const uint32_t ktileA = A_KS ? 64u * (uint32_t)p.lda * 2u : 0u, ktileB = B_KS ? 64u * (uint32_t)p.ldb * 2u : 0u;
 #define PP_DMA(rsrc, vo, ldsoff, buf, soff)                                                                             \
   __builtin_amdgcn_raw_ptr_buffer_load_lds(rsrc, (lds_void_t*)(smem + (buf) * BUF + (ldsoff)), 16, vo, soff, 0, 0)
@@ -937,10 +936,6 @@
 #define PP_DMA_B(h, buf, tile) do { PP_DMA_B1(h, 0, buf, tile); PP_DMA_B1(h, 1, buf, tile); } while (0)
 
   f32x4_t acc[8][4];
-#pragma unroll
-  for (int i = 0; i < 8; ++i)
-#pragma unroll
-    for (int j = 0; j < 4; ++j) acc[i][j] = (f32x4_t){0.f, 0.f, 0.f, 0.f};
 
   const uint32_t lds0 = (uint32_t)(uintptr_t)(__attribute__((address_space(3))) char*)smem;
   const int i16 = lane & 15, g = lane >> 4, sw = (i16 >> 1) & 7, tq = (i16 >> 2) & 3;
@@ -1030,24 +1025,75 @@
     PP_STAMPS_FOLD();                                                                                       \
   } while (0)
 
-  PP_DMA_A(0, 0, 0); PP_DMA_B(0, 0, 0); PP_DMA_B(1, 0, 0); PP_DMA_A(1, 0, 0);
-  if (nk > 1) { PP_DMA_A(0, 1, 1); PP_DMA_B(0, 1, 1); PP_DMA_B(1, 1, 1); }
-  PP_SB();
-  if (nk > 1) { PP_VMCNT(8); } else { PP_VMCNT(2); }
-  PP_BAR();
-  PP_RDF_A(0, 0, 0, 0); PP_RDF_A(0, 0, 1, 0); PP_RDF_A(0, 0, 2, 0); PP_RDF_A(0, 0, 3, 0);
-  PP_RDF_A(0, 0, 0, 1); PP_RDF_A(0, 0, 1, 1); PP_RDF_A(0, 0, 2, 1); PP_RDF_A(0, 0, 3, 1);
-  PP_RDF_B(0, 0, 0, 0); PP_RDF_B(0, 0, 1, 0); PP_RDF_B(0, 0, 0, 1); PP_RDF_B(0, 0, 1, 1);
-  PP_SB();
-  if (wm == 1) PP_BAR();
-  for (int t = 0; t < nk; t += 2) {
-    PP_TILE(0, t);
-    if (t + 1 < nk) PP_TILE(1, t + 1);
-  }
-  if (wm == 0) PP_BAR();
+  constexpr bool PREFETCH = LEAN;
+#define PP_DMA_TILE0() do { PP_DMA_A(0, 0, 0); PP_DMA_B(0, 0, 0); PP_DMA_B(1, 0, 0); PP_DMA_A(1, 0, 0); } while (0)
+  const int v0 = blockIdx.x, vstep = gridDim.x, nv = p.nv;
+#define PP_OPAQUE_LANE(x)                                                                  \
+  uint32_t x##z_ = 0u;                                                                     \
+  asm volatile("" : "+s"(x##z_));                                                          \
+  const int x = (int)__builtin_amdgcn_mbcnt_hi(~0u, __builtin_amdgcn_mbcnt_lo(~0u, x##z_))
+#define PP_OPAQUE_ARGS(x)                                                                                                    \
+  const __attribute__((address_space(4))) GemmP* x##k_ = (const __attribute__((address_space(4))) GemmP*)__builtin_amdgcn_kernarg_segment_ptr(); \
+  asm volatile("" : "+s"(x##k_));                                                                                            \
+  const GemmP& x = *(const GemmP*)x##k_
+  {
+    PP_OPAQUE_LANE(ln);
+    set_tile(p, v0, ln);
+  }
+  PP_DMA_TILE0();
+  for (int v = v0;;) {
+#pragma unroll
+    for (int i = 0; i < 8; ++i)
+#pragma unroll
+      for (int j = 0; j < 4; ++j) acc[i][j] = (f32x4_t){0.f, 0.f, 0.f, 0.f};
+    if (PREFETCH && v != v0) { PP_SB(); PP_VMCNT(0); PP_BAR(); }
+    if (nk > 1) { PP_DMA_A(0, 1, 1); PP_DMA_B(0, 1, 1); PP_DMA_B(1, 1, 1); }
+    PP_SB();
+    if (nk > 1) { PP_VMCNT(8); } else { PP_VMCNT(2); }
+    PP_BAR();
+    PP_RDF_A(0, 0, 0, 0); PP_RDF_A(0, 0, 1, 0); PP_RDF_A(0, 0, 2, 0); PP_RDF_A(0, 0, 3, 0);
+    PP_RDF_A(0, 0, 0, 1); PP_RDF_A(0, 0, 1, 1); PP_RDF_A(0, 0, 2, 1); PP_RDF_A(0, 0, 3, 1);
+    PP_RDF_B(0, 0, 0, 0); PP_RDF_B(0, 0, 1, 0); PP_RDF_B(0, 0, 0, 1); PP_RDF_B(0, 0, 1, 1);
+    PP_SB();
+    if (wm == 1) PP_BAR();
+    for (int t = 0; t < nk; t += 2) {
+      PP_TILE(0, t);
+      if (t + 1 < nk) PP_TILE(1, t + 1);
+    }
+    if (wm == 0) PP_BAR();
 #if defined(DXA_PP_STAMPS)
-  const uint32_t iv0_ = iv_[0], iv1_ = iv_[1], iv2_ = iv_[2], iv3_ = iv_[3], iv4_ = iv_[4], iv5_ = iv_[5], iv6_ = iv_[6], iv7_ = iv_[7];
+    const uint32_t iv0_ = iv_[0], iv1_ = iv_[1], iv2_ = iv_[2], iv3_ = iv_[3], iv4_ = iv_[4], iv5_ = iv_[5], iv6_ = iv_[6], iv7_ = iv_[7];
 #endif
+    const int e_bid = bid, e_split_j = split_j, e_split_s = split_s, e_tail_i = tail_i, e_m0i = m0i, e_n0i = n0i;
+    [[maybe_unused]] const int e_nk = nk;
+    const int vn = v + vstep;
+    const bool more = LEAN && vn < nv;
+    PP_OPAQUE_LANE(ln);
+    const int tid_e = wave * 64 + ln;
+    PP_OPAQUE_ARGS(pe);
+    if (PREFETCH && more) { set_tile(pe, vn, ln); PP_SB(); PP_DMA_TILE0(); PP_SB(); }
+    if constexpr (LEAN) {
+      if (tile_split_exchange<4, 16>(pe, acc, tid_e, e_split_j, e_split_s, e_tail_i)) {
+        __builtin_amdgcn_sched_barrier(0);
+        char* slab = smem + BUF + wave * 4096;
+        if constexpr (FUSE == 1) sk_epilogue_swiglu<4, 16>(pe, acc, slab, ln, wm, wn, e_m0i, e_n0i);
+        else sk_epilogue<TO, TE, 4, 16>(pe, acc, slab, ln, wm, wn, e_m0i, e_n0i, reinterpret_cast<float*>(smem + 2 * BUF), e_bid);
+#if defined(DXA_PP_STAMPS)
+        __syncthreads();
+        if (e_m0i == 0 && e_n0i == 0 && lane == 0) {
+          uint32_t* o_ = reinterpret_cast<uint32_t*>(p.C) + wave * 16;
+          o_[0] = iv0_; o_[1] = iv1_; o_[2] = iv2_; o_[3] = iv3_; o_[4] = iv4_; o_[5] = iv5_; o_[6] = iv6_; o_[7] = iv7_;
+          o_[8] = (uint32_t)e_nk;
+        }
+#endif
+      }
+    } else {
+      tile_finish<TO, 4, TE, false, 16>(pe, acc, smem, tid_e, ln, wave, wm, wn, ln & 31, ln >> 5, (int64_t)e_m0i, (int64_t)e_n0i, e_split_j, e_split_s, e_tail_i);
+    }
+    if (!more) break;
+    if (!PREFETCH) { PP_SB(); PP_VMCNT(0); PP_BAR(); set_tile(pe, vn, ln); PP_DMA_TILE0(); }
+    v = vn;
+  }
 #undef PP_A_ROW0
 #undef PP_B_ROW0
 #undef PP_DMA
@@ -1073,23 +1119,9 @@
 #undef PP_R_B1
 #undef PP_R_A1
 #undef PP_R_NEXT
-
-  if constexpr (LEAN) {
-    if (!tile_split_exchange<4, 16>(p, acc, tid, split_j, split_s, tail_i)) return;
-    __builtin_amdgcn_sched_barrier(0);
-    if constexpr (FUSE == 1) sk_epilogue_swiglu<4, 16>(p, acc, smem + wave * 4096, lane, wm, wn, m0i, n0i);
-    else sk_epilogue<TO, TE, 4, 16>(p, acc, smem + wave * 4096, lane, wm, wn, m0i, n0i, reinterpret_cast<float*>(smem + 8 * 4096), bid);
-#if defined(DXA_PP_STAMPS)
-    __syncthreads();
-    if (m0i == 0 && n0i == 0 && lane == 0) {
-      uint32_t* o_ = reinterpret_cast<uint32_t*>(p.C) + wave * 16;
-      o_[0] = iv0_; o_[1] = iv1_; o_[2] = iv2_; o_[3] = iv3_; o_[4] = iv4_; o_[5] = iv5_; o_[6] = iv6_; o_[7] = iv7_;
-      o_[8] = (uint32_t)nk;
-    }
-#endif
-  } else {
-    tile_finish<TO, 4, TE, false, 16>(p, acc, smem, tid, lane, wave, wm, wn, l32, lh, m0, n0, split_j, split_s, tail_i);
-  }
+#undef PP_DMA_TILE0
+#undef PP_OPAQUE_LANE
+#undef PP_OPAQUE_ARGS
 #endif
 }
 
@@ -1472,7 +1504,10 @@
     else if (pp) k = &KERNELS.pp_nt[!lean][ty];
     else if (ai == 3 && d->K % 64 == 0) k = &KERNELS.pp3[!lean_ok][ty];
     else k = &KERNELS.ring[ai == 3][ty];
-    plan_add(plan, s, *k, s.full + s.tail_r * s.split_s);
+    int64_t grid = s.full + s.tail_r * s.split_s;
+    const bool loops = pp && (lean || d->fuse == DXA_FUSE_SWIGLU);
+    if (loops && d->max_workgroups > 0 && (d->max_workgroups <= NUM_CU || s.split_s == 1)) grid = std::min<int64_t>(grid, d->max_workgroups);
+    plan_add(plan, s, *k, grid);
     return DXA_OK;
   }
   DXA_CHECK_ARG(d->fuse == DXA_FUSE_NONE, "dxa_gemm: fuse is only implemented on the bf16 NT MFMA fast path (K %% 32 == 0, M, N >= 64, 16-byte aligned rows, no batching)");
@@ -1516,6 +1551,7 @@
   DXA_CHECK_ARG(d->out_dtype == d->in_dtype || d->out_dtype == DXA_F32,
                 "dxa_gemm: out_dtype must equal in_dtype or be fp32");
   DXA_CHECK_ARG(d->nb[0] >= 1 && d->nb[1] >= 1 && d->nb[2] >= 1, "dxa_gemm: batch extents must be >= 1");
+  DXA_CHECK_ARG(d->max_workgroups >= 0, "dxa_gemm: negative max_workgroups %d", d->max_workgroups);
   if (d->M == 0 || d->N == 0) return DXA_OK;
   DXA_CHECK_ARG(d->A && d->B && d->C, "dxa_gemm: null operand");
   const int64_t nbatch = (int64_t)d->nb[0] * d->nb[1] * d->nb[2];
@@ -1576,6 +1612,7 @@
   p.tm = s.tm; p.tn = s.tn;
   p.vecA = s.vecA; p.vecB = s.vecB; p.vecC = s.vecC; p.vecR = s.vecR; p.vecG = s.vecG; p.vecBias = s.vecBias;
   p.full = s.full; p.tail_r = s.tail_r; p.split_s = s.split_s; p.group_m = s.group_m;
+  p.nv = s.full + s.tail_r * s.split_s;
   if (s.mirror) p.mirror = (char*)d->mirror;
   if (s.sumsq) p.sumsq = d->sumsq;
   if (s.K2 > 0) { p.A2 = (const char*)d->A2; p.B2 = (const char*)d->B2; p.K2 = s.K2; }
diff --git a/dexbotic_amd/csrc/gemm_common.h b/dexbotic_amd/csrc/gemm_common.h
--- a/dexbotic_amd/csrc/gemm_common.h
+++ b/dexbotic_amd/csrc/gemm_common.h
@@ -1,5 +1,6 @@
 #pragma once
 #include "common.h"
+#include <type_traits>
 
 namespace dxa_gemm_detail {
 typedef float f32x16_t __attribute__((ext_vector_type(16)));
@@ -26,6 +27,7 @@
   int* flags;
   const char* A2; const char* B2; int64_t K2;
   int fuse; int64_t ldaux;
+  int nv;
 };
 }
 
@@ -110,6 +112,39 @@
     for (int r = 0; r < 4; ++r) v[r] += c0[r];
   }
   store4<TO>(cp, v, p.vecC, n_ok);
+}
+
+template <int NW> __device__ __forceinline__ void ld_words(uint32_t (&o)[NW], const void* p) {
+  static_assert(NW == 2 || NW == 4 || NW == 8, "8, 16 or 32 bytes");
+  if constexpr (NW == 2) {
+    const uint2 v = *reinterpret_cast<const uint2*>(p);
+    o[0] = v.x; o[1] = v.y;
+  } else {
+#pragma unroll
+    for (int h = 0; h < NW / 4; ++h) {
+      const uint4 v = reinterpret_cast<const uint4*>(p)[h];
+      o[4 * h] = v.x; o[4 * h + 1] = v.y; o[4 * h + 2] = v.z; o[4 * h + 3] = v.w;
+    }
+  }
+}
+template <typename T, int CPL> __device__ __forceinline__ void words_to_f32(float (&o)[CPL], const uint32_t (&w)[CPL * (int)sizeof(T) / 4]) {
+  if constexpr (sizeof(T) == 4) {
+#pragma unroll
+    for (int e = 0; e < CPL; ++e) o[e] = __uint_as_float(w[e]);
+  } else {
+#pragma unroll
+    for (int e = 0; e < CPL / 2; ++e) { o[2 * e] = __uint_as_float(w[e] << 16); o[2 * e + 1] = __uint_as_float(w[e] & 0xffff0000u); }
+  }
+}
+template <typename T, int CPL> __device__ __forceinline__ void st_row16(T* p, const float (&v)[CPL]) {
+  static_assert(CPL * sizeof(T) == 16, "one 16-byte store");
+  if constexpr (sizeof(T) == 4) {
+    *reinterpret_cast<float4*>(p) = make_float4(v[0], v[1], v[2], v[3]);
+  } else {
+    uint4 o;
+    o.x = pack_bf16x2(v[0], v[1]); o.y = pack_bf16x2(v[2], v[3]); o.z = pack_bf16x2(v[4], v[5]); o.w = pack_bf16x2(v[6], v[7]);
+    *reinterpret_cast<uint4*>(p) = o;
+  }
 }
 
 constexpr int NUM_CU_D = 256;
@@ -232,8 +267,31 @@
   if constexpr (!SMALL) {
     constexpr int ROWP = 64 * 4 + 16;
     char* slab = smem + wave * (64 * ROWP);
-#pragma unroll
-    for (int pass = 0; pass < 2; ++pass) {
+    constexpr int CPL = 16 / (int)sizeof(TO), LPR = 64 / CPL, RPI = 64 / LPR;
+    constexpr int EB = CPL * (int)sizeof(TE), NWE = EB / 4, NWO = 4;
+    constexpr int NB = 8;
+    const auto al = [](const void* q, int a) { return (reinterpret_cast<uintptr_t>(q) & (uintptr_t)(a - 1)) == 0; };
+    const int64_t mw = m0 + wm * (BMR / 2), nw = n0 + wn * 64;
+    const bool fast = sizeof(TO) == 2 && p.vecC && al(C, 16) && (p.ldc * (int64_t)sizeof(TO)) % 16 == 0 && (!AUX || al(AUX, 16)) &&
+                      (!R || (p.vecR && al(R, EB) && (p.ldr * (int64_t)sizeof(TE)) % EB == 0)) &&
+                      (!G || (p.vecG && al(G, EB) && (p.ldg * (int64_t)sizeof(TE)) % EB == 0)) &&
+                      mw + BMR / 2 <= p.M && nw + 64 <= p.N;
+    const int fr = lane / LPR, fc = (lane % LPR) * CPL;
+    const int64_t nf = nw + fc;
+    float bvf[CPL];
+#pragma unroll
+    for (int e = 0; e < CPL; ++e) bvf[e] = 0.f;
+    if (fast && bias) {
+#pragma unroll
+      for (int u = 0; u < CPL / 4; ++u) {
+        float b4[4];
+        load4<TE>(b4, bias + nf + 4 * u, p.vecBias, 4);
+#pragma unroll
+        for (int e = 0; e < 4; ++e) bvf[4 * u + e] = b4[e];
+      }
+    }
+    const auto do_pass = [&](auto pass_c) {
+      constexpr int pass = decltype(pass_c)::value;
       if constexpr (MF == 32) {
 #pragma unroll
         for (int ii = 0; ii < 2; ++ii)
@@ -251,19 +309,75 @@
       }
       __builtin_amdgcn_fence(__ATOMIC_RELEASE, "wavefront");
       __builtin_amdgcn_wave_barrier();
+      if (sizeof(TO) == 2 && fast) {
+        constexpr int nit = (AI == 3 && pass == 1) ? 32 / RPI : 64 / RPI;
+#pragma unroll
+        for (int b0 = 0; b0 < nit; b0 += NB) {
+          uint32_t gw[NB][NWE], rw[NB][NWE], cw[NB][NWO];
+#pragma unroll
+          for (int k = 0; k < NB; ++k) {
+            if (b0 + k >= nit) continue;
+            const int64_t m = mw + pass * 64 + fr + RPI * (b0 + k);
+            if (G) ld_words<NWE>(gw[k], G + m * p.ldg + nf);
+            if (R) ld_words<NWE>(rw[k], R + m * p.ldr + nf);
+            if (p.accumulate) ld_words<NWO>(cw[k], C + m * p.ldc + nf);
+          }
+#pragma unroll
+          for (int k = 0; k < NB; ++k) {
+            if (b0 + k >= nit) continue;
+            const int row = fr + RPI * (b0 + k);
+            const int64_t m = mw + pass * 64 + row;
+            float v[CPL];
+#pragma unroll
+            for (int u = 0; u < CPL / 4; ++u) {
+              const float4 t = *reinterpret_cast<const float4*>(slab + row * ROWP + (fc + 4 * u) * 4);
+              v[4 * u] = t.x; v[4 * u + 1] = t.y; v[4 * u + 2] = t.z; v[4 * u + 3] = t.w;
+            }
+#pragma unroll
+            for (int e = 0; e < CPL; ++e) v[e] = v[e] * p.alpha + bvf[e];
+            if (AUX) st_row16<TO, CPL>(AUX + m * p.ldc + nf, v);
+            if (G) {
+              float g[CPL];
+              words_to_f32<TE, CPL>(g, gw[k]);
+#pragma unroll
+              for (int e = 0; e < CPL; ++e) v[e] *= act_grad(p.act, g[e]);
+            } else if (p.act != DXA_ACT_NONE) {
+#pragma unroll
+              for (int e = 0; e < CPL; ++e) v[e] = act_fwd(p.act, v[e]);
+            }
+            if (R) {
+              float r[CPL];
+              words_to_f32<TE, CPL>(r, rw[k]);
+#pragma unroll
+              for (int e = 0; e < CPL; ++e) v[e] += r[e];
+            }
+            if (p.accumulate) {
+              float c0[CPL];
+              words_to_f32<TO, CPL>(c0, cw[k]);
+#pragma unroll
+              for (int e = 0; e < CPL; ++e) v[e] += c0[e];
+            }
+            st_row16<TO, CPL>(C + m * p.ldc + nf, v);
+          }
+          __builtin_amdgcn_sched_barrier(0);
+        }
+      } else {
 #pragma unroll 4
-      for (int it = 0; it < (AI == 3 && pass == 1 ? 8 : 16); ++it) {
-        const int row = cr + 4 * it;
-        const int64_t m = m0 + wm * (BMR / 2) + pass * 64 + row;
-        const float4 v = *reinterpret_cast<const float4*>(slab + row * ROWP + cc * 4);
-        if (m < p.M && n_ok > 0) {
-          const float a4[4] = {v.x, v.y, v.z, v.w};
-          epilogue4<TE, TO>(p, C, AUX, R, G, bv, m, n, n_ok, a4);
+        for (int it = 0; it < (AI == 3 && pass == 1 ? 8 : 16); ++it) {
+          const int row = cr + 4 * it;
+          const int64_t m = m0 + wm * (BMR / 2) + pass * 64 + row;
+          const float4 v = *reinterpret_cast<const float4*>(slab + row * ROWP + cc * 4);
+          if (m < p.M && n_ok > 0) {
+            const float a4[4] = {v.x, v.y, v.z, v.w};
+            epilogue4<TE, TO>(p, C, AUX, R, G, bv, m, n, n_ok, a4);
+          }
         }
       }
       __builtin_amdgcn_fence(__ATOMIC_RELEASE, "wavefront");
       __builtin_amdgcn_wave_barrier();
-    }
+    };
+    do_pass(std::integral_constant<int, 0>{});
+    do_pass(std::integral_constant<int, 1>{});
   } else {
     char* slab = smem + 131072 + wave * 4096;
     [[maybe_unused]] const int r16 = l32 & 15;
diff --git a/dexbotic_amd/kernels.py b/dexbotic_amd/kernels.py
--- a/dexbotic_amd/kernels.py
+++ b/dexbotic_amd/kernels.py
@@ -139,6 +139,16 @@
 
 _NB1 = (1, 1, 1)
 
+_CU_COUNT: dict = {}
+
+
+def _cu_count() -> int:
+    dev = _cur_device() if _cur_device is not None else torch.cuda.current_device()
+    n = _CU_COUNT.get(dev)
+    if n is None:
+        n = _CU_COUNT[dev] = int(torch.cuda.get_device_properties(dev).multi_processor_count)
+    return n
+
 
 def gemm(layout: int, a: torch.Tensor, b: torch.Tensor, M: int, N: int, K: int, lda: int, ldb: int,
          out: torch.Tensor, ldc: int, *, bias: Optional[torch.Tensor] = None,
@@ -148,12 +158,13 @@
          sA: Sequence[int] = (0, 0, 0), sB: Sequence[int] = (0, 0, 0), sC: Sequence[int] = (0, 0, 0),
          sR: Sequence[int] = (0, 0, 0), sG: Sequence[int] = (0, 0, 0), epi_f32: bool = False,
          mirror: Optional[torch.Tensor] = None, sumsq: Optional[torch.Tensor] = None,
-         a2: Optional[torch.Tensor] = None, b2: Optional[torch.Tensor] = None) -> torch.Tensor:
+         a2: Optional[torch.Tensor] = None, b2: Optional[torch.Tensor] = None,
+         max_workgroups: Optional[int] = None) -> torch.Tensor:
     if not epi_f32 and a2 is None and _x3_eligible(layout, a, b, out, M, N, K, lda, ldb, nb):
         a3, b3 = split3_pair(a, False, b, False, a_dims=(M, K, lda), b_dims=(N, K, ldb))
         return gemm(L.NT, a3, b3, M, N, 3 * K, 3 * K, 3 * K, out, ldc, bias=bias, residual=residual, ldr=ldr, act=act,
                     aux_out=aux_out, mulgrad=mulgrad, ldg=ldg, alpha=alpha, accumulate=accumulate, epi_f32=True,
-                    mirror=mirror, sumsq=sumsq)
+                    mirror=mirror, sumsq=sumsq, max_workgroups=max_workgroups)
     d = L.GemmDesc()
     d.layout, d.in_dtype, d.out_dtype, d.act = layout, dt(a), dt(out), act
     d.epi_f32 = int(epi_f32)
@@ -169,6 +180,7 @@
     d.bias, d.residual, d.ldr = _ptr(bias), _ptr(residual), ldr
     d.aux_out, d.mulgrad, d.ldg = _ptr(aux_out), _ptr(mulgrad), ldg
     d.alpha, d.accumulate = alpha, int(accumulate)
+    d.max_workgroups = _cu_count() if max_workgroups is None else max_workgroups
     if mirror is not None:
         if mirror.dtype != torch.bfloat16 or out.dtype != torch.float32 or tuple(nb) != (1, 1, 1) or \
                 _row_major(mirror, "mirror") != ldc:
@@ -283,7 +295,7 @@
             M * 2 * F_ * 2 < (1 << 31) and w.numel() * 2 < (1 << 31))
 
 
-def mm_nt_swiglu(x: torch.Tensor, w: torch.Tensor, keep_pre: bool = True):
+def mm_nt_swiglu(x: torch.Tensor, w: torch.Tensor, keep_pre: bool = True, max_workgroups: Optional[int] = None):
     M, K_ = x.shape
     N = w.shape[0]
     F_ = N // 2
@@ -295,6 +307,7 @@
     d.A, d.lda, d.B, d.ldb, d.C, d.ldc = _ptr(x), K_, _ptr(w), K_, _ptr(out), F_
     d.aux_out, d.ld_aux = _ptr(pre), N
     d.alpha, d.fuse = 1.0, L.FUSE_SWIGLU
+    d.max_workgroups = _cu_count() if max_workgroups is None else max_workgroups
     for i in range(3):
         d.nb[i] = 1
     prof = GEMM_PROFILE
diff --git a/include/dexbotic_amd.h b/include/dexbotic_amd.h
--- a/include/dexbotic_amd.h
+++ b/include/dexbotic_amd.h
@@ -61,6 +61,7 @@
   int64_t K2;
   int32_t fuse;
   int64_t ld_aux;
+  int32_t max_workgroups;
 } dxa_gemm_desc;
 int dxa_gemm(const dxa_gemm_desc* d, dxa_stream_t stream);
 int64_t dxa_gemm_sumsq_slots(int64_t M, int64_t N);
```

Result: slower. 69.86 episodes/s (-1.0%).
